# aantoine890/navierstokes

Measured on AMD Instinct MI355X. Metric: fp64 CSR SpMV GFLOP/s & % HBM roofline @ nnz; 1/2/4/8 GPU, higher is better.
Workload: dtype f64

## Files before the change

include/mi355_spmv.h:

```cpp
#ifndef MI355_SPMV_H
#define MI355_SPMV_H

#ifdef __cplusplus
extern "C" {
#endif

#define MI355_SPMV_VERSION 501

enum {
    MI_OK = 0,
    MI_ERR_ARG = 1,
    MI_ERR_NODEVICE = 2,
    MI_ERR_HIP = 3,
    MI_ERR_ALLOC = 4,
    MI_ERR_UNSUPPORTED = 5,
    MI_ERR_STATE = 6
};

#define MI_MAX_POWERS 16

typedef struct mi_csr_s* mi_csr_t;
typedef struct mi_bcsr4_s* mi_bcsr4_t;
typedef struct mi_part_s* mi_part_t;
typedef void* mi_stream_t;

enum {
    MI_KERNEL_AUTO = 0,
    MI_KERNEL_STREAM = 1,
    MI_KERNEL_RING = 2,
    MI_KERNEL_ROWPAR = 3,
    MI_KERNEL_BCSR4 = 4,
    MI_KERNEL_MRING = 6,
    MI_KERNEL_SSTREAM = 7,
    MI_KERNEL_TILE = 5
};

int mi_version(void);
const char* mi_strerror(int status);
const char* mi_last_error(void);
int mi_device_count(int* count);
int mi_set_device(int device);
int mi_device_synchronize(void);
int mi_flush_cache(void);
int mi_flush_cache_async(mi_stream_t s);

int mi_csr_create(int n, int ncols, const int* ptrow, const int* indcol, const double* coef, mi_csr_t* out);
int mi_csr_create_mapped(int n, int ncols, const int* ptrow, const int* indcol, const double* coef,
                         const int* rowmap, mi_csr_t* out);
int mi_csr_destroy(mi_csr_t A);
int mi_csr_update_values(mi_csr_t A, const double* coef);
int mi_csr_update_values_dev(mi_csr_t A, const double* d_coef, mi_stream_t s);
int mi_csr_dims(mi_csr_t A, int* n, int* ncols, long long* nnz);
int mi_csr_reorder_info(mi_csr_t A, int* reordered, int* block, double* spread_before, double* spread_after,
                        double* us_natural, double* us_reordered);
int mi_csr_perm(mi_csr_t A, int* reordered, int* perm );
int mi_vec_to_internal_dev(mi_csr_t A, const double* d_x, double* d_x_int, mi_stream_t s);
int mi_vec_from_internal_dev(mi_csr_t A, const double* d_x_int, double* d_x, mi_stream_t s);
int mi_spmv_internal_dev(mi_csr_t A, const double* d_x_int, double* d_y_int, mi_stream_t s);
int mi_spmk_internal_dev(mi_csr_t A, int k, const double* d_x_int, double* const* d_y_int_out, mi_stream_t s);
int mi_reorder_probe(int n, const int* ptrow, const int* indcol, int* block, int* perm, double* spread_before,
                     double* spread_after);
int mi_csr_set_kernel(mi_csr_t A, int kernel_id);
int mi_csr_ring_info(mi_csr_t A, int* config_id, int* runs, int* runs_not_ringable, double* nnz_fraction_ringable);
int mi_csr_ring_shape_info(mi_csr_t A, int* blocks, int* lean, int* depth, double* us_aligned, double* us_unaligned);
int mi_csr_tune_info(mi_csr_t A, double* us_ring, double* us_stream);
int mi_csr_tune_detail(mi_csr_t A, double us[5], int* ring_nt, int* stream_nt);
int mi_ring_plan_probe(int n, const int* ptrow, const int* indcol, int config_id, int* nblk, int* runs,
                       int* runs_not_ringable, double* nnz_fraction_ringable, int* max_slot);
int mi_csr_tile_info(mi_csr_t A, int* built, int* nblk, double* unique_per_nnz, double us[2], int* nt);
int mi_tile_plan_probe(int n, const int* ptrow, const int* indcol, int threads, int* nblk, long long* distinct_total,
                       int* max_distinct, long long* nnz_listed);
int mi_csr_placement_info(mi_csr_t A, int* n_values, int* n_total, double* us, int cap);
int mi_vec_alloc_placed(mi_csr_t A, int nvec, int draws, double** d_vecs, double* us, int cap, int* n_us);
int mi_vec_free_placed(double* d_vec);
int mi_csr_sstream_info(mi_csr_t A, int* built, int* rounds, long long* steps, double* padding, double us[4], int* form);
int mi_sstream_plan_probe(int n, int ncols, const int* ptrow, const int* indcol, int* eligible, int* rounds, long long* steps, double* padding);
int mi_sstream_plan_probe_ex(int n, int ncols, const int* ptrow, const int* indcol, int shift, int ghost_lo, int ghost_hi, int* eligible, int* rounds,
                             long long* steps, double* padding, int* ghost_workgroups, int* rounds_min_max);
int mi_sstream_mw_plan_probe(int n, int ncols, const int* ptrow, const int* indcol, int shift, int* eligible, int* rounds, long long* steps, double* padding);
int mi_csr_mring_info(mi_csr_t A, int* built, int* runs, int* runs_not_served, double* nnz_fraction_served, double us[2], int* nt);
int mi_mring_plan_probe(int n, const int* ptrow, const int* indcol, int* nblk, int* runs, int* runs_not_served,
                        double* nnz_fraction_served, long long* window_restarts);
int mi_mring_plan_deal_probe(int n, const int* ptrow, const int* indcol, int* table_len, int* run_blocks, int cap);
int mi_ring_plan_lean(int n, const int* ptrow, const int* indcol, int config_id, int* lean);
int mi_csr_block4_structure(int n, const int* ptrow, const int* indcol, int* is_blocked, long long* nblocks);
int mi_csr_set_nontemporal(mi_csr_t A, int ring_nt, int stream_nt);
int mi_stream_read_probe(long long bytes, int launches, double* us_per_launch);
int mi_csr_get_kernel(mi_csr_t A, int* kernel_id);
const char* mi_csr_kernel_name(mi_csr_t A);

int mi_spmv(mi_csr_t A, const double* x, double* y);
int mi_spmv_dev(mi_csr_t A, const double* d_x, double* d_y, mi_stream_t s);

int mi_spmk(mi_csr_t A, int k, const double* x, double* const* y_out);
int mi_spmk_dev(mi_csr_t A, int k, const double* d_x, double* const* d_y_out, mi_stream_t s);

int mi_csr_spmk_info(mi_csr_t A, int k, int* eligible, int* one_launch, double* us_k_launches, double* us_one_launch);

int mi_spmk_plan_probe(int n, const int* ptrow, const int* indcol, int* eligible, int* runs, int* max_deps);

int mi_dot(int n, const double* x, const double* y, double* out);
int mi_dot_dev(int n, const double* d_x, const double* d_y, double* d_out, mi_stream_t s);
int mi_axpy(int n, double a, const double* x, double* y);
int mi_axpy_dev(int n, double a, const double* d_x, double* d_y, mi_stream_t s);
int mi_orthogonalize(int n, const double* b, const double* x1, double* x3, double alpha, double* beta_out);
int mi_orthogonalize_dev(int n, const double* d_b, const double* d_x1, double* d_x3, double alpha,
                         double* d_beta_out, mi_stream_t s);
int mi_spmv_dot_dev(mi_csr_t A, const double* d_x, double* d_y, const double* d_b, double* d_beta_out, mi_stream_t s);
int mi_csr_dot_epilogue_info(mi_csr_t A, int* in_epilogue);
int mi_csr_dot_epilogue_layout(mi_csr_t A, int* threads, int* wgs, int* nblk, int* run_first_block, int* block_row0,
                               int* block_rows, int cap_runs, int cap_blocks);
int mi_spmv_orthogonalize_dev(mi_csr_t A, const double* d_x, double* d_x1, const double* d_b, double* d_x3, double alpha,
                              double* d_beta_out, mi_stream_t s);
int mi_orthonormalize_against_basis(int n, int m, const double* const* basis, double* y, double* dots_out );
int mi_orthonormalize_against_basis_dev(int n, int m, const double* const* d_basis, double* d_y, double* d_dots ,
                                        mi_stream_t s);
int mi_mdot(int n, int m, const double* const* basis, const double* y, double* dots );
int mi_mdot_dev(int n, int m, const double* const* d_basis , const double* d_y,
                double* d_dots , mi_stream_t s);
int mi_maxpy(int n, int m, const double* coef , int negate, const double* const* basis, double* y);
int mi_maxpy_dev(int n, int m, const double* d_coef , int negate, const double* const* d_basis, double* d_y,
                 double* d_norm_out, mi_stream_t s);
int mi_cgs_dev(int n, int m, const double* const* d_basis, double* d_y, int passes, double* d_h ,
               double* d_norm , mi_stream_t s);
int mi_norm2(int n, const double* x, double* out);
int mi_norm2_dev(int n, const double* d_x, double* d_out, mi_stream_t s);
int mi_rel_error(int n, const double* ref, const double* test, double* out);
int mi_rel_error_dev(int n, const double* d_ref, const double* d_test, double* d_out, mi_stream_t s);
int mi_gather_dev(int m, const int* d_idx, const double* d_src, double* d_dst, mi_stream_t s);

int mi_bcsr4_create(int nbrows, int nbcols, const int* ptrow, const int* indcol, const double* coef,
                    mi_bcsr4_t* out);
int mi_bcsr4_destroy(mi_bcsr4_t A);
enum { MI_BLOCK_ROWMAJOR = 0, MI_BLOCK_COLMAJOR = 1 };
int mi_bcsr4_create_layout(int nbrows, int nbcols, const int* ptrow, const int* indcol, const double* coef, int layout, mi_bcsr4_t* out);
int mi_bcsr4_update_values_layout(mi_bcsr4_t A, const double* coef, int layout);
int mi_bcsr4_update_values_layout_dev(mi_bcsr4_t A, const double* d_coef, int layout, mi_stream_t s);
int mi_bcsr4_tile_info(mi_bcsr4_t A, int* built, int* in_use, double* us_plain, double* us_tile);
int mi_bcsr4_sell_info(mi_bcsr4_t A, int* built, int* form_in_use, long long* steps, double* padding, double us[4]);
int mi_bcsr4_sell_plan_probe(int nbrows, const int* ptrow, const int* indcol, int nwaves_max, int* nslices, long long* nsteps, int* nwaves,
                             int* sptr, int* wrng, unsigned* col);
int mi_bcsr4_update_values(mi_bcsr4_t A, const double* coef);
int mi_bcsr4_update_values_dev(mi_bcsr4_t A, const double* d_coef, mi_stream_t s);
int mi_bcsr4_spmv(mi_bcsr4_t A, const double* x, double* y);
int mi_bcsr4_spmv_dev(mi_bcsr4_t A, const double* d_x, double* d_y, mi_stream_t s);
int mi_bcsr4_spmk(mi_bcsr4_t A, int k, const double* x, double* const* y_out);
int mi_bcsr4_spmk_dev(mi_bcsr4_t A, int k, const double* d_x, double* const* d_y_out, mi_stream_t s);

enum { MI_ARITH_CHAIN = 0, MI_ARITH_BLOCKACC = 1 };
int mi_bcsr4_spmm(mi_bcsr4_t A, int s, const double* X, long long ldx, double* Y, long long ldy, int arith);
int mi_bcsr4_spmm_dev(mi_bcsr4_t A, int s, const double* d_X, long long ldx, double* d_Y, long long ldy, int arith,
                      mi_stream_t st);
int mi_bcsr4_spmm_info(mi_bcsr4_t A, int s, int* tile_built, int* form_in_use, int* longest_list, double us[5]);
int mi_spmm_dev(mi_csr_t A, int s, const double* d_X, long long ldx, double* d_Y, long long ldy, mi_stream_t st);
int mi_krylov_basis_dev(mi_csr_t A, int s, const double* d_v0, double* d_V, long long ldv, int orth, double* d_coef,
                        mi_stream_t st);
int mi_krylov_basis_cgs_dev(mi_csr_t A, int s, const double* d_v0, double* d_V, long long ldv, int passes, double* d_coef,
                            mi_stream_t st);

typedef struct mi_bilu4_s* mi_bilu4_t;
int mi_bilu4_create(int nbrows, const int* ptrow, const int* indcol, const double* coef, int layout , int fill,
                    mi_bilu4_t* out);
int mi_bilu4_create_host(int nbrows, const int* ptrow, const int* indcol, const double* coef, int layout, int fill, mi_bilu4_t* out);
int mi_bilu4_destroy(mi_bilu4_t F);
int mi_bilu4_refactor(mi_bilu4_t F, const double* coef, int layout);
int mi_bilu4_solve_dev(mi_bilu4_t F, const double* d_b, double* d_x, mi_stream_t s);
int mi_bilu4_solve(mi_bilu4_t F, const double* b, double* x);
int mi_bilu4_info(mi_bilu4_t F, int* nbrows, long long* nblocks, int* fwd_levels, int* bwd_levels, int* launches, int* form,
                  double us[2], double* factor_seconds, long long* factor_bytes);
int mi_bilu4_factor_host(mi_bilu4_t F, int* ptr, int* col, int* diag, double* val, long long cap_blocks);
int mi_bilu4_plan_probe(int nbrows, const int* ptrow, const int* indcol, int fill, long long* nblocks, int* fwd_levels,
                        int* bwd_levels, int* fwd_launches, int* bwd_launches, int* fwd_sizes, int* bwd_sizes, int cap_levels);

int mi_bilu4dev_plan_probe(int nbrows, const int* ptrow, const int* indcol, int fill, long long* update_pairs, int* launches,
                           long long* plan_bytes);
int mi_bilu4dev_prepare(mi_bilu4_t F);
int mi_bilu4dev_refactor(mi_bilu4_t F, const double* d_coef, int layout, mi_stream_t s);
int mi_bilu4dev_status(mi_bilu4_t F, int* bad_row);
int mi_bilu4dev_fetch(mi_bilu4_t F);
int mi_bilu4dev_info(mi_bilu4_t F, int* prepared, int* launches, long long* plan_bytes);

enum { MI_BILU_FORM_LEVELS = 0, MI_BILU_FORM_ONE = 1, MI_BILU_FORM_AUTO = -1 };
int mi_bilu4one_plan_probe(int nbrows, const int* ptrow, const int* indcol, int fill, int workgroups, int* eligible, int nchunks[2],
                           int max_deps[2], long long* plan_bytes, int* const chunk_pos[2], int* const chunk_lev[2],
                           int* const dep_ptr[2], int* const dep[2]);
int mi_bilu4one_prepare(mi_bilu4_t F);
int (mi_bilu4_set_solve_form)(mi_bilu4_t F, int form);
int mi_bilu4one_status(mi_bilu4_t F);
int mi_bilu4one_info(mi_bilu4_t F, int* prepared, int* eligible, int* workgroups, int nchunks[2], int max_deps[2], long long* plan_bytes);

int mi_bilu4sw_prepare(mi_bilu4_t F);
int mi_bilu4sw_solve_dev(mi_bilu4_t F, const double* d_b, double* d_x, int sweeps_fwd, int sweeps_bwd, mi_stream_t s);
// ... 74 lines not shown
```

navierstokes_amd/csrc/capi_bcsr.hip:

```cpp
#include "capi_internal.hpp"
#include "spmv_bcsr_sell.hpp"

static int sell_fill(mi_bcsr4_t A, hipStream_t s);

template <class Select>
static bool bcsr4_race(mi_bcsr4_t A, int ncand, Select select, double* us)
{
    LaunchTimer tm;
    ScratchPair sp;
    if (sp.alloc(4 * (size_t)std::max(A->nbcols, 1), 4 * (size_t)std::max(A->nbrows, 1)) != MI_OK || tm.init() != MI_OK) return false;
    std::vector<char> failed((size_t)ncand, 0);
    for (int round = 0; round < 2; round++)
        for (int c = 0; c < ncand; c++) {
            if (failed[c]) continue;
            select(c);
            double t = 0.0;
            if (tm.time(3, 8, [&] { return launch_bcsr4(A, sp.x, sp.y, nullptr, false); }, &t) == MI_OK) us[c] = min_measured(us[c], t);
            else failed[c] = 1;
        }
    for (int c = 0; c < ncand; c++)
        if (failed[c]) us[c] = 0.0;
    return true;
}

// ... 42 lines not shown

static int build_bcsr4_sell(mi_bcsr4_t A, const int* ptrow, const int* indcol)
{
    SellPlanHost P, P2;
    build_sell_plan(A->nbrows, ptrow, indcol, 1024, P);
    build_sell_wave_ranges(P, 2048, P2.wrng, P2.nwaves);
    const size_t vbytes = sizeof(double) * (size_t)(P.nsteps + kSellPadSteps) * kSellStepDoubles;
    hipError_t e;
    if ((e = hipMalloc(&A->d_sell_val, vbytes)) != hipSuccess || (e = hipMalloc(&A->d_sell_col, sizeof(unsigned) * P.col.size())) != hipSuccess ||
        (e = hipMalloc(&A->d_sell_sptr, sizeof(int) * P.sptr.size())) != hipSuccess || (e = hipMalloc(&A->d_sell_wrng, sizeof(int) * P.wrng.size())) != hipSuccess ||
        (e = hipMalloc(&A->d_sell_wrng2, sizeof(int) * P2.wrng.size())) != hipSuccess ||
        (e = hipMemcpy(A->d_sell_wrng2, P2.wrng.data(), sizeof(int) * P2.wrng.size(), hipMemcpyHostToDevice)) != hipSuccess ||
        (e = hipMemset(A->d_sell_val + (size_t)P.nsteps * kSellStepDoubles, 0, sizeof(double) * (size_t)kSellPadSteps * kSellStepDoubles)) != hipSuccess ||
        (e = hipMemcpy(A->d_sell_col, P.col.data(), sizeof(unsigned) * P.col.size(), hipMemcpyHostToDevice)) != hipSuccess ||
        (e = hipMemcpy(A->d_sell_sptr, P.sptr.data(), sizeof(int) * P.sptr.size(), hipMemcpyHostToDevice)) != hipSuccess ||
        (e = hipMemcpy(A->d_sell_wrng, P.wrng.data(), sizeof(int) * P.wrng.size(), hipMemcpyHostToDevice)) != hipSuccess) {
        (void)hipGetLastError();
        dfree(A->d_sell_val); dfree(A->d_sell_col); dfree(A->d_sell_sptr); dfree(A->d_sell_wrng); dfree(A->d_sell_wrng2);
        A->d_sell_val = nullptr;
        A->d_sell_col = nullptr;
        A->d_sell_sptr = A->d_sell_wrng = A->d_sell_wrng2 = nullptr;
        return e == hipErrorOutOfMemory ? MI_OK : fail(MI_ERR_HIP, std::string("bcsr4 sliced copy: ") + hipGetErrorString(e));
    }
    A->sell_nslices = P.nslices;
    A->sell_nwaves = P.nwaves;
    A->sell_nwaves2 = P2.nwaves;
    A->sell_nsteps = P.nsteps;
    return sell_fill(A, nullptr);
}

static void choose_bcsr4_sell_form(mi_bcsr4_t A, bool forced)
{
    if (const char* fe = getenv("MI355_BCSR_SELL_FORM")) A->sell_form = std::max(0, std::min(3, atoi(fe)));
    else if (forced) A->sell_form = 0;
    else if (env_is("MI355_SPMV_AUTOTUNE", "0")) A->sell_form = 0;
    else {
        double us[5] = {0, 0, 0, 0, 0};
        if (!bcsr4_race(A, 5, [&](int c) { A->sell_form = c - 1; }, us)) return;
        int best = 0;
        for (int c = 1; c < 5; c++) {
            A->tune_us_sell[c - 1] = us[c];
            if (better(us[c], us[best])) best = c;
        }
        if (A->tune_us_plain <= 0 && A->tune_us_tile <= 0) A->tune_us_plain = us[0];
        A->sell_form = best - 1;
    }
}

extern "C" int mi_bcsr4_create(int nbrows, int nbcols, const int* ptrow, const int* indcol, const double* coef,
                               mi_bcsr4_t* out)
{
    CHECK_ARG(out, "out is null");
    *out = nullptr;
    CHECK_ARG(nbrows >= 0 && nbcols >= 0 && ptrow && ptrow[0] == 0, "bad argument");
    for (int i = 0; i < nbrows; i++) CHECK_ARG(ptrow[i] <= ptrow[i + 1], "ptrow must be non-decreasing");
    const long long nb = ptrow[nbrows];
    CHECK_ARG(nb == 0 || (indcol && coef), "indcol/coef is null");
    for (long long k = 0; k < nb; k++) CHECK_ARG(indcol[k] >= 0 && indcol[k] < nbcols, "block column outside [0, nbcols)");
    int rc = need_device();
    if (rc) return rc;
    std::unique_ptr<mi_bcsr4_s, int (*)(mi_bcsr4_t)> owner(new (std::nothrow) mi_bcsr4_s(), mi_bcsr4_destroy);
    mi_bcsr4_t A = owner.get();
    if (!A) return fail(MI_ERR_ALLOC, "host allocation failed");
    A->nbrows = nbrows;
    A->nbcols = nbcols;
    A->nblocks = nb;
    hipError_t e;
    if ((e = hipGetDevice(&A->device)) != hipSuccess ||
        (e = hipMalloc(&A->d_ptrow, sizeof(int) * ((size_t)nbrows + 1))) != hipSuccess ||
        (e = hipMalloc(&A->d_indcol, sizeof(int) * ((size_t)nb + 1))) != hipSuccess ||
        (e = hipMalloc(&A->d_coef, sizeof(double) * 16 * ((size_t)nb + 1))) != hipSuccess ||
        (e = hipMemcpy(A->d_ptrow, ptrow, sizeof(int) * ((size_t)nbrows + 1), hipMemcpyHostToDevice)) != hipSuccess ||
        (nb && (e = hipMemcpy(A->d_indcol, indcol, sizeof(int) * (size_t)nb, hipMemcpyHostToDevice)) != hipSuccess) ||
        (nb && (e = hipMemcpy(A->d_coef, coef, sizeof(double) * 16 * (size_t)nb, hipMemcpyHostToDevice)) != hipSuccess))
        return fail(e == hipErrorOutOfMemory ? MI_ERR_ALLOC : MI_ERR_HIP, std::string("bcsr4 upload: ") + hipGetErrorString(e));
    for (int s0 = 0; s0 < nbrows; s0 += kSellRows)
        A->max_slice_vals = std::max(A->max_slice_vals, 16 * (ptrow[std::min(nbrows, s0 + kSellRows)] - ptrow[s0]));
    if ((rc = build_bcsr4_tile(A, ptrow, indcol))) return rc;
    const bool forced = env_is("MI355_BCSR_SELL", "1");
    if (!env_is("MI355_BCSR_SELL", "0") && (forced || nb >= 100000) && nbcols > 0 && nbcols < (1 << 30)) {
        if ((rc = build_bcsr4_sell(A, ptrow, indcol))) return rc;
        if (A->d_sell_val) choose_bcsr4_sell_form(A, forced);
    }
    if ((e = hipStreamSynchronize(nullptr)) != hipSuccess) return fail(MI_ERR_HIP, std::string("mi_bcsr4_create: ") + hipGetErrorString(e));
    *out = owner.release();
    return MI_OK;
}

static int sell_fill(mi_bcsr4_t A, hipStream_t s)
{
    const int grid = std::max(1, std::min(A->sell_nslices, 8192));
    hipLaunchKernelGGL(bcsr4_to_sell_kernel, dim3((unsigned)grid), dim3(64), 0, s, A->sell_nslices, A->nbrows, A->d_ptrow, A->d_coef, A->d_sell_sptr, A->d_sell_val);
    HIP_TRY(hipGetLastError());
    return MI_OK;
}

int bcsr4_refresh_from_csr(mi_bcsr4_s* A, const int* d_csr_ptrow, const double* d_src, double* d_csr_out, hipStream_t s)
{
    if (!A || A->nbrows == 0) return MI_OK;
    const int nslices = (A->nbrows + kSellRows - 1) / kSellRows;
    const int grid = std::max(1, std::min(nslices, 2048));
    const int* sptr = A->d_sell_val ? A->d_sell_sptr : nullptr;
    double* sv = A->d_sell_val;
    if (A->max_slice_vals <= 4096)
        hipLaunchKernelGGL((bcsr4_refresh_kernel<4096>), dim3((unsigned)grid), dim3(256), 0, s, nslices, A->nbrows, d_csr_ptrow, d_src, d_csr_out, A->d_ptrow, A->d_coef, sptr, sv);
    else if (A->max_slice_vals <= 16384)
        hipLaunchKernelGGL((bcsr4_refresh_kernel<16384>), dim3((unsigned)std::min(grid, 256)), dim3(256), 0, s, nslices, A->nbrows, d_csr_ptrow, d_src, d_csr_out, A->d_ptrow, A->d_coef, sptr, sv);
    else
        hipLaunchKernelGGL((bcsr4_refresh_kernel<0>), dim3((unsigned)grid), dim3(256), 0, s, nslices, A->nbrows, d_csr_ptrow, d_src, d_csr_out, A->d_ptrow, A->d_coef, sptr, sv);
    HIP_TRY(hipGetLastError());
    return MI_OK;
}

static int bcsr4_refresh_from_blocks(mi_bcsr4_s* A, const double* d_src, bool colmajor, hipStream_t s)
{
    if (!A || A->nbrows == 0 || A->nblocks == 0) return MI_OK;
    const int nslices = (A->nbrows + kSellRows - 1) / kSellRows;
    const int grid = std::max(1, std::min(nslices, 2048));
    const int* sptr = A->d_sell_val ? A->d_sell_sptr : nullptr;
    double* out = d_src == A->d_coef ? nullptr : A->d_coef;
    if (colmajor && !out) return fail(MI_ERR_ARG, "column-major blocks cannot be transposed in place");
    if (!out && !A->d_sell_val) return MI_OK;
#define BR_LAUNCH(CAP_, CM_, G_) hipLaunchKernelGGL((bcsr4_blocks_refresh_kernel<CAP_, CM_>), dim3((unsigned)(G_)), dim3(256), 0, s, nslices, A->nbrows, A->d_ptrow, d_src, out, sptr, A->d_sell_val)
    if (A->max_slice_vals <= 4096) { if (colmajor) BR_LAUNCH(4096, true, grid); else BR_LAUNCH(4096, false, grid); }
    else if (A->max_slice_vals <= 16384) { if (colmajor) BR_LAUNCH(16384, true, std::min(grid, 256)); else BR_LAUNCH(16384, false, std::min(grid, 256)); }
    else { if (colmajor) BR_LAUNCH(0, true, grid); else BR_LAUNCH(0, false, grid); }
#undef BR_LAUNCH
    HIP_TRY(hipGetLastError());
    return MI_OK;
}

int bcsr4_values_changed(mi_bcsr4_s* A, hipStream_t s)
{
    if (A && A->d_sell_val && A->nblocks > 0) return sell_fill(A, s);
    return MI_OK;
}

extern "C" int mi_bcsr4_sell_info(mi_bcsr4_t A, int* built, int* form_in_use, long long* steps, double* padding, double us[4])
{
    CHECK_ARG(A, "null handle");
    if (built) *built = A->d_sell_val != nullptr;
    if (form_in_use) *form_in_use = A->d_sell_val ? A->sell_form : -1;
    if (steps) *steps = A->sell_nsteps;
    if (padding) *padding = A->nblocks > 0 && A->d_sell_val ? (double)A->sell_nsteps * kSellRows / (double)A->nblocks - 1.0 : 0.0;
    if (us)
        for (int i = 0; i < 4; i++) us[i] = A->tune_us_sell[i];
    return MI_OK;
}

extern "C" int mi_bcsr4_sell_plan_probe(int nbrows, const int* ptrow, const int* indcol, int nwaves_max, int* nslices, long long* nsteps,
                                        int* nwaves, int* sptr, int* wrng, unsigned* col)
{
    CHECK_ARG(nbrows >= 0 && ptrow && ptrow[0] == 0 && nwaves_max >= 1, "bad argument");
    for (int i = 0; i < nbrows; i++) CHECK_ARG(ptrow[i] <= ptrow[i + 1], "ptrow must be non-decreasing");
    const long long nb = ptrow[nbrows];
    CHECK_ARG(nb == 0 || indcol, "indcol is null");
    for (long long k = 0; k < nb; k++) CHECK_ARG(indcol[k] >= 0 && indcol[k] < (1 << 30), "block column outside [0, 2^30)");
    SellPlanHost P;
    build_sell_plan(nbrows, ptrow, indcol, nwaves_max, P);
    if (nslices) *nslices = P.nslices;
    if (nsteps) *nsteps = P.nsteps;
    if (nwaves) *nwaves = P.nwaves;
    if (sptr) std::copy(P.sptr.begin(), P.sptr.end(), sptr);
    if (wrng) std::copy(P.wrng.begin(), P.wrng.end(), wrng);
    if (col) std::copy(P.col.begin(), P.col.end(), col);
    return MI_OK;
}

static void transpose_blocks_host(long long nb, const double* src, double* dst)
{
    for (long long k = 0; k < nb; k++)
        for (int r = 0; r < 4; r++)
            for (int c = 0; c < 4; c++) dst[16 * k + 4 * r + c] = src[16 * k + 4 * c + r];
}

extern "C" int mi_bcsr4_create_layout(int nbrows, int nbcols, const int* ptrow, const int* indcol, const double* coef, int layout,
                                      mi_bcsr4_t* out)
{
    CHECK_ARG(layout == MI_BLOCK_ROWMAJOR || layout == MI_BLOCK_COLMAJOR, "unknown block layout");
    if (layout == MI_BLOCK_ROWMAJOR) return mi_bcsr4_create(nbrows, nbcols, ptrow, indcol, coef, out);
    CHECK_ARG(out, "out is null");
    *out = nullptr;
    CHECK_ARG(nbrows >= 0 && ptrow && ptrow[0] == 0 && ptrow[nbrows] >= 0, "bad argument");
    const long long nb = ptrow[nbrows];
    CHECK_ARG(nb == 0 || coef, "coef is null");
    std::vector<double> t((size_t)nb * 16);
    transpose_blocks_host(nb, coef, t.data());
    return mi_bcsr4_create(nbrows, nbcols, ptrow, indcol, t.data(), out);
}

extern "C" int mi_bcsr4_update_values_layout(mi_bcsr4_t A, const double* coef, int layout)
{
    CHECK_ARG(A, "null handle");
    CHECK_ARG(layout == MI_BLOCK_ROWMAJOR || layout == MI_BLOCK_COLMAJOR, "unknown block layout");
    if (layout == MI_BLOCK_ROWMAJOR || A->nblocks == 0) return mi_bcsr4_update_values(A, coef);
    CHECK_ARG(coef, "null coef");
    std::vector<double> t((size_t)A->nblocks * 16);
    transpose_blocks_host(A->nblocks, coef, t.data());
    return mi_bcsr4_update_values(A, t.data());
}

extern "C" int mi_bcsr4_update_values_layout_dev(mi_bcsr4_t A, const double* d_coef, int layout, mi_stream_t s)
{
    CHECK_ARG(A, "null handle");
    CHECK_ARG(layout == MI_BLOCK_ROWMAJOR || layout == MI_BLOCK_COLMAJOR, "unknown block layout");
    if (layout == MI_BLOCK_ROWMAJOR || A->nblocks == 0) return mi_bcsr4_update_values_dev(A, d_coef, s);
    CHECK_ARG(d_coef && d_coef != A->d_coef, "null coef, or the handle's own array");
    return bcsr4_refresh_from_blocks(A, d_coef, true, (hipStream_t)s);
}

extern "C" int mi_bcsr4_tile_info(mi_bcsr4_t A, int* built, int* in_use, double* us_plain, double* us_tile)
{
    CHECK_ARG(A, "null handle");
    if (built) *built = A->d_tl_ptr != nullptr;
    if (in_use) *in_use = A->use_tile && A->d_tl_ptr;
    if (us_plain) *us_plain = A->tune_us_plain;
    if (us_tile) *us_tile = A->tune_us_tile;
    return MI_OK;
}

extern "C" int mi_bcsr4_update_values(mi_bcsr4_t A, const double* coef)
{
    CHECK_ARG(A, "null handle");
    if (A->nblocks == 0) return MI_OK;
    CHECK_ARG(coef, "null coef");
    HIP_TRY(hipMemcpy(A->d_coef, coef, sizeof(double) * 16 * (size_t)A->nblocks, hipMemcpyHostToDevice));
    int rc = bcsr4_values_changed(A, nullptr);
    if (rc) return rc;
    HIP_TRY(hipStreamSynchronize(nullptr));
    return MI_OK;
}

extern "C" int mi_bcsr4_update_values_dev(mi_bcsr4_t A, const double* d_coef, mi_stream_t s)
{
    CHECK_ARG(A, "null handle");
    if (A->nblocks == 0) return MI_OK;
    CHECK_ARG(d_coef, "null coef");
    return bcsr4_refresh_from_blocks(A, d_coef, false, (hipStream_t)s);
}

extern "C" int mi_bcsr4_destroy(mi_bcsr4_t A)
{
    if (!A) return MI_OK;
    dfree(A->d_ptrow);
    dfree(A->d_indcol);
    dfree(A->d_coef);
    dfree(A->d_browmap);
    dfree(A->d_tl_ptr);
    dfree(A->d_tl_nodes);
    dfree(A->d_tl_slots);
    dfree(A->d_sell_val);
    dfree(A->d_sell_col);
    dfree(A->d_sell_sptr);
    dfree(A->d_sell_wrng);
    dfree(A->d_sell_wrng2);
    dfree(A->st.d_ptr);
    dfree(A->st.d_nodes);
    dfree(A->st.d_slots);
    dfree(A->st.d_rows);
    dfree(A->st64.d_ptr);
    dfree(A->st64.d_nodes);
    dfree(A->st64.d_slots);
    dfree(A->st64.d_rows);
    dfree(A->d_x);
    dfree(A->d_y);
    for (double* p : A->d_pow) dfree(p);
    delete A;
    return MI_OK;
}

int launch_bcsr4(mi_bcsr4_t A, const double* d_x, double* d_y, mi_stream_t s, bool use_map)
{
    CHECK_ARG(A, "null handle");
    if (A->nbrows == 0) return MI_OK;
    CHECK_ARG(d_x && d_y, "null vector");
    CHECK_ARG((((uintptr_t)d_x) & 15) == 0, "x must be 16-byte aligned");
    Bcsr4View V{A->nbrows, A->nbcols, A->d_ptrow, A->d_indcol, A->d_coef, use_map ? A->d_browmap : nullptr};
    const long long threads = 4LL * A->nbrows;
    const int nwg = (int)((threads + kWG - 1) / kWG);
    static const int chunk = getenv("MI355_BCSR_XCD_CHUNK") ? atoi(getenv("MI355_BCSR_XCD_CHUNK")) : 0;
    const int grid = nwg;
    if (A->sell_form >= 0 && A->d_sell_val) {
        const bool two = A->sell_form == 2;
        SellView S{A->d_sell_val, A->d_sell_col, A->d_sell_sptr, two ? A->d_sell_wrng2 : A->d_sell_wrng, A->sell_nslices, A->nbrows, V.browmap};
        const int swg = two ? A->sell_nwaves2 / 8 : A->sell_nwaves / 4;
        switch (A->sell_form) {
        case 0: hipLaunchKernelGGL((spmv_bcsr4_sell<8, true, 0, 2, 4>), dim3((unsigned)swg), dim3(256), 0, (hipStream_t)s, S, d_x, d_y, swg); break;
        case 1: hipLaunchKernelGGL((spmv_bcsr4_sell<8, false, 0, 2, 4>), dim3((unsigned)swg), dim3(256), 0, (hipStream_t)s, S, d_x, d_y, swg); break;
        case 2: hipLaunchKernelGGL((spmv_bcsr4_sell<4, true, 0, 2, 8>), dim3((unsigned)swg), dim3(512), 0, (hipStream_t)s, S, d_x, d_y, swg); break;
        default: hipLaunchKernelGGL((spmv_bcsr4_sell<12, true, 0, 2, 4>), dim3((unsigned)swg), dim3(256), 0, (hipStream_t)s, S, d_x, d_y, swg); break;
        }
        HIP_TRY(hipGetLastError());
        return MI_OK;
    }
    if (A->use_tile && A->d_tl_ptr) {
        Bcsr4Tile Tl{A->d_tl_ptr, A->d_tl_nodes, A->d_tl_slots};
        hipLaunchKernelGGL(spmv_bcsr4_tile<kBcsrDepth>, dim3((unsigned)grid), dim3(kWG), 0, (hipStream_t)s, V, Tl, d_x, d_y, nwg);
        HIP_TRY(hipGetLastError());
        return MI_OK;
    }
    hipLaunchKernelGGL(spmv_bcsr4<kBcsrDepth>, dim3((unsigned)grid), dim3(kWG), 0, (hipStream_t)s, V, d_x, d_y, chunk, nwg);
    HIP_TRY(hipGetLastError());
    return MI_OK;
}

void bcsr4_drop_sliced(mi_bcsr4_s* A)
{
    if (!A || !A->d_sell_val) return;
    (void)hipDeviceSynchronize();
    dfree(A->d_sell_val);
    dfree(A->d_sell_col);
    dfree(A->d_sell_sptr);
    dfree(A->d_sell_wrng);
    dfree(A->d_sell_wrng2);
    A->d_sell_val = nullptr;
    A->d_sell_col = nullptr;
    A->d_sell_sptr = A->d_sell_wrng = A->d_sell_wrng2 = nullptr;
    A->sell_form = -1;
}

extern "C" int mi_bcsr4_spmv_dev(mi_bcsr4_t A, const double* d_x, double* d_y, mi_stream_t s)
{
    return launch_bcsr4(A, d_x, d_y, s, true);
}

extern "C" int mi_bcsr4_spmv(mi_bcsr4_t A, const double* x, double* y)
{
    CHECK_ARG(A, "null handle");
    if (A->nbrows == 0) return MI_OK;
    CHECK_ARG(x && y, "null vector");
    if (!A->d_x) HIP_TRY(hipMalloc(&A->d_x, sizeof(double) * 4 * (size_t)(A->nbcols > 0 ? A->nbcols : 1)));
    if (!A->d_y) HIP_TRY(hipMalloc(&A->d_y, sizeof(double) * 4 * (size_t)A->nbrows));
    HIP_TRY(hipMemcpy(A->d_x, x, sizeof(double) * 4 * (size_t)A->nbcols, hipMemcpyHostToDevice));
    int rc = mi_bcsr4_spmv_dev(A, A->d_x, A->d_y, nullptr);
    if (rc) return rc;
    HIP_TRY(hipMemcpy(y, A->d_y, sizeof(double) * 4 * (size_t)A->nbrows, hipMemcpyDeviceToHost));
    return MI_OK;
}

extern "C" int mi_bcsr4_spmk_dev(mi_bcsr4_t A, int k, const double* d_x, double* const* d_y_out, mi_stream_t s)
{
    CHECK_ARG(A, "null handle");
    if (k < 1 || k > MI_MAX_POWERS) return fail(MI_ERR_UNSUPPORTED, "k must be in 1..MI_MAX_POWERS");
    CHECK_ARG(A->nbrows == A->nbcols, "matrix powers need a square matrix");
    CHECK_ARG(d_y_out, "null output array");
    const double* src = d_x;
    for (int p = 0; p < k; p++) {
        CHECK_ARG(A->nbrows == 0 || d_y_out[p], "null output vector");
        int rc = mi_bcsr4_spmv_dev(A, src, d_y_out[p], s);
        if (rc) return rc;
        src = d_y_out[p];
    }
    return MI_OK;
}

extern "C" int mi_bcsr4_spmk(mi_bcsr4_t A, int k, const double* x, double* const* y_out)
{
    CHECK_ARG(A, "null handle");
    if (k < 1 || k > MI_MAX_POWERS) return fail(MI_ERR_UNSUPPORTED, "k must be in 1..MI_MAX_POWERS");
    CHECK_ARG(A->nbrows == A->nbcols, "matrix powers need a square matrix");
    if (A->nbrows == 0) return MI_OK;
// ... 156 lines not shown
    if (A->st_state) return A->st_state;
    A->st_state = -1;
    if (env_is("MI355_SPMM_TILE", "0") || A->nblocks < 4096) return -1;
    std::vector<int> ptrow((size_t)A->nbrows + 1), indcol((size_t)A->nblocks);
    if (hipMemcpy(ptrow.data(), A->d_ptrow, sizeof(int) * ptrow.size(), hipMemcpyDeviceToHost) != hipSuccess ||
        hipMemcpy(indcol.data(), A->d_indcol, sizeof(int) * indcol.size(), hipMemcpyDeviceToHost) != hipSuccess) {
        (void)hipGetLastError();
        return -1;
    }
    int cap128 = 368, cap64 = 256;
    if (const char* ce = getenv("MI355_SPMM_TILE_UCAP")) (void)sscanf(ce, "%d,%d", &cap128, &cap64);
    A->st_state = build_spmm_tile_plan(A, 128, cap128, ptrow, indcol, A->st);
    (void)build_spmm_tile_plan(A, 64, cap64, ptrow, indcol, A->st64);
    return A->st_state;
}

static const SpmmTilePlan* spmm_plan_of(const mi_bcsr4_s* A, int s)
{
    if (s < 1 || s > 4) return nullptr;
    const SpmmTilePlan* Pl = A->st.d_ptr ? &A->st : nullptr;
    if (!Pl || spmm_tile_lds(Pl, s) > kLdsBytesPerCU) return nullptr;
    return Pl;
}

enum { kSpmmGather = 0, kSpmmTile = 1, kSpmmOct = 2, kSpmmOctNt = 3, kSpmmSell = 4, kSpmmForms = 5 };

static int sell_fill(mi_bcsr4_t A, hipStream_t s);

static bool spmm_form_possible(const mi_bcsr4_s* A, int s, int form, bool mapped = false)
{
    if (form == kSpmmGather) return true;
    if (form == kSpmmSell) return (s == 4 || s == 8) && A->d_sell_val;
    if (form == kSpmmTile) return spmm_plan_of(A, s) != nullptr;
    return s % 2 == 0 && A->st64.d_ptr && spmm_tile_lds(&A->st64, s) <= kLdsBytesPerCU;
}

static void launch_spmm_gather(const Bcsr4View& V, int m, int arith, const double* Xj, long long ldx, double* Yj, long long ldy, hipStream_t st)
{
    switch (m) {
    case 1: launch_spmm_s<1>(V, arith, Xj, ldx, Yj, ldy, st); break;
    case 2: launch_spmm_s<2>(V, arith, Xj, ldx, Yj, ldy, st); break;
    case 3: launch_spmm_s<3>(V, arith, Xj, ldx, Yj, ldy, st); break;
    case 4: launch_spmm_s<4>(V, arith, Xj, ldx, Yj, ldy, st); break;
    case 5: launch_spmm_s<5>(V, arith, Xj, ldx, Yj, ldy, st); break;
    case 6: launch_spmm_s<6>(V, arith, Xj, ldx, Yj, ldy, st); break;
    case 7: launch_spmm_s<7>(V, arith, Xj, ldx, Yj, ldy, st); break;
    default: launch_spmm_s<8>(V, arith, Xj, ldx, Yj, ldy, st); break;
    }
}

static int launch_spmm(mi_bcsr4_t A, int s, int arith, const double* X, long long ldx, double* Y, long long ldy, hipStream_t st,
                       bool use_map)
{
    Bcsr4View V{A->nbrows, A->nbcols, A->d_ptrow, A->d_indcol, A->d_coef, use_map ? A->d_browmap : nullptr};
    for (int j0 = 0; j0 < s; j0 += 8) {
        const int m = std::min(8, s - j0);
        const double* Xj = X + (size_t)j0 * ldx;
        double* Yj = Y + (size_t)j0 * ldy;
        const bool mapped = V.browmap != nullptr;
        auto run = [&](int form) -> hipError_t {
            if (form == kSpmmSell) {
                SellView Sv{A->d_sell_val, A->d_sell_col, A->d_sell_sptr, A->d_sell_wrng, A->sell_nslices, A->nbrows, V.browmap};
                const int swg = A->sell_nwaves / 4;
                if (m == 4) {
                    if (arith == MI_ARITH_CHAIN) hipLaunchKernelGGL((spmm_bcsr4_sell<4, 0, 6, true>), dim3((unsigned)swg), dim3(256), 0, st, Sv, Xj, ldx, Yj, ldy, swg);
                    else hipLaunchKernelGGL((spmm_bcsr4_sell<4, 1, 6, true>), dim3((unsigned)swg), dim3(256), 0, st, Sv, Xj, ldx, Yj, ldy, swg);
                } else {
                    if (arith == MI_ARITH_CHAIN) hipLaunchKernelGGL((spmm_bcsr4_sell<8, 0, 6, true>), dim3((unsigned)swg), dim3(256), 0, st, Sv, Xj, ldx, Yj, ldy, swg);
                    else hipLaunchKernelGGL((spmm_bcsr4_sell<8, 1, 6, true>), dim3((unsigned)swg), dim3(256), 0, st, Sv, Xj, ldx, Yj, ldy, swg);
                }
                return hipGetLastError();
            }
            if (form == kSpmmTile) return spmm_tile_launch(A, spmm_plan_of(A, m), V, m, arith, Xj, ldx, Yj, ldy, st);
            if (form == kSpmmOct || form == kSpmmOctNt) return spmm_otile_launch(A, &A->st64, V, m, arith, form == kSpmmOctNt, Xj, ldx, Yj, ldy, st);
            launch_spmm_gather(V, m, arith, Xj, ldx, Yj, ldy, st);
            return hipGetLastError();
        };
        int form = kSpmmGather;
        const bool capturing = stream_is_capturing(st);
        if (capturing && A->spmm_choice[m] > 0 && (A->st_state == 1 || A->spmm_choice[m] - 1 == kSpmmSell) &&
            !(A->spmm_choice[m] - 1 == kSpmmSell && mapped))
            form = A->spmm_choice[m] - 1;
        const bool tiles = !capturing && build_spmm_tile(A) == 1;
        if (!capturing && (tiles || spmm_form_possible(A, m, kSpmmSell, mapped))) {
            const char* e = getenv("MI355_SPMM_TILE");
            const int forced = e ? atoi(e) : -1;
            auto possible = [&](int f) { return (f == kSpmmGather || f == kSpmmSell || tiles) && spmm_form_possible(A, m, f, mapped); };
            if (forced >= 0 && forced < kSpmmForms) form = possible(forced) ? forced : kSpmmGather;
            else {
                if (A->spmm_choice[m] == 0) {
                    int best = kSpmmGather;
                    LaunchTimer tm(st);
                    if (tm.init() == MI_OK) {
                        double us[kSpmmForms] = {0, 0, 0, 0, 0};
                        bool ok = true;
                        for (int round = 0; round < 2 && ok; round++)
                            for (int f = 0; f < kSpmmForms && ok; f++) {
                                if (!possible(f)) continue;
                                double t = 0.0;
                                ok = tm.time(2, 5, [&] { return run(f) == hipSuccess ? MI_OK : MI_ERR_HIP; }, &t) == MI_OK;
                                if (ok) us[f] = min_measured(us[f], t);
                            }
                        for (int f = 0; f < kSpmmForms; f++) {
                            A->spmm_us[m][f] = us[f];
                            if (ok && us[f] > 0 && us[f] < us[best]) best = f;
                        }
                        if (!ok) { (void)hipGetLastError(); best = kSpmmGather; }
                    }
                    A->spmm_choice[m] = 1 + best;
                }
                form = A->spmm_choice[m] - 1;
                if (!possible(form)) form = kSpmmGather;
            }
        }
        hipError_t er = run(form);
        if (er != hipSuccess) return fail(MI_ERR_HIP, std::string("multi-vector product: ") + hipGetErrorString(er));
    }
    HIP_TRY(hipGetLastError());
    return MI_OK;
}

extern "C" int mi_bcsr4_spmm_info(mi_bcsr4_t A, int s, int* tile_built, int* form_in_use, int* longest_list, double us[5])
{
    CHECK_ARG(A && s >= 1 && s <= 8, "bad argument");
    if (tile_built) *tile_built = A->st_state == 1;
// ... 155 lines not shown
```

navierstokes_amd/csrc/capi_csr.hip:

```cpp
#include "capi_internal.hpp"
#include "reorder.hpp"
#include "mring_plan.hpp"
#include "tile_plan.hpp"

int get_table(mi_csr_t A, int nnzb, BlockTable** out)
{
    BlockTable& T = A->tables[nnzb];
    if (!T.d_blk) {
        std::vector<int> rows, ptrs;
        int row_align = A->nnz < 20000000 ? 64 : 1;
        if (const char* e = getenv("MI355_STREAM_ROW_ALIGN")) row_align = std::max(1, atoi(e));
        build_row_blocks(A->n, A->h_ptrow.data(), nnzb, 4 * kWG, rows, ptrs, row_align, 7);
        T.nnzb = nnzb;
        T.nblk = (int)rows.size() - 1;
        std::vector<int2> h(rows.size());
        for (size_t i = 0; i < rows.size(); i++) h[i] = make_int2(rows[i], ptrs[i]);
        HIP_TRY(hipMalloc(&T.d_blk, sizeof(int2) * h.size()));
        HIP_TRY(hipMemcpy(T.d_blk, h.data(), sizeof(int2) * h.size(), hipMemcpyHostToDevice));
    }
    *out = &T;
    return MI_OK;
}

static void free_tile(mi_csr_t A)
{
    dfree(A->tile.d_desc);
    dfree(A->tile.d_ulist);
    dfree(A->tile.d_slots);
    A->tile = TileTable();
}

static void free_mring(mi_csr_t A)
{
    dfree(A->mring.d_plan);
    dfree(A->mring.d_first);
    dfree(A->mring.d_ok);
    dfree(A->mring.d_rng);
    dfree(A->mring.d_slots);
    A->mring = MringTable();
}

static void free_sstream(mi_csr_t A)
{
    ss_free(A->ss.dev);
    A->ss = SstreamTable();
}

static inline bool beyond_infinity_cache(double bytes_per_nnz, long long nnz, int n) { return bytes_per_nnz * (double)nnz + 16.0 * (double)n > 0.75 * 256e6; }

constexpr double kSsMaxPadding = 0.12;
static double ss_max_padding()
{
    if (const char* e = getenv("MI355_SSTREAM_MAX_PADDING")) return std::max(0.0, atof(e));
    return kSsMaxPadding;
}

static int build_sstream(mi_csr_t A, const int* ptrow, const int* indcol, int ghost_lo = 0, int ghost_hi = 0)
{
    if (A->ss.dev.val) return MI_OK;
    SsPlanHost P;
    SsMwPlanHost M;
    const int shift = (A->y_offset & 1) && !A->d_rowmap ? 1 : 0;
    build_sstream_plan(A->n, A->ncols, ptrow, indcol, ss_max_padding(), P, true, shift, ghost_lo, ghost_hi);
    SstreamTable& T = A->ss;
    hipError_t e;
    if (!P.eligible) {
        if (ghost_lo < ghost_hi || env_is("MI355_SSTREAM_MW", "0")) return MI_OK;
        build_sstream_mw_plan(A->n, A->ncols, ptrow, indcol, ss_max_padding(), M, shift);
        if (!M.eligible) return MI_OK;
        e = ss_mw_upload(M, T.dev);
        T.mw = e == hipSuccess;
    } else e = ss_upload(P, T.dev, ghost_lo < ghost_hi);
    const SsPlanHost& Q = P.eligible ? P : M;
    if (e != hipSuccess) {
        free_sstream(A);
        if (e == hipErrorOutOfMemory) { (void)hipGetLastError(); return MI_OK; }
        return fail(MI_ERR_HIP, std::string("sliced copy: ") + hipGetErrorString(e));
    }
    T.nwg = Q.nwg;
    T.rounds = Q.rounds;
    T.shift = Q.shift;
    T.steps = Q.steps;
    T.padding = (double)Q.pad_places / (double)A->nnz;
    T.max_slice_nnz = Q.max_slice_nnz;
    if (ghost_lo < ghost_hi) {
        T.h_wg_halo = P.wg_halo;
        T.h_wg = P.wg;
        T.fusable = P.fusable;
    }
    sstream_fill_values(T.rounds, A->n, T.shift, A->d_ptrow, A->d_coef, nullptr, T.dev.slice_step, T.dev.slice_len, T.dev.val, T.max_slice_nnz, nullptr, T.mw ? 1 : 0);
    if ((e = hipGetLastError()) != hipSuccess) {
        free_sstream(A);
        return fail(MI_ERR_HIP, std::string("sliced copy fill: ") + hipGetErrorString(e));
    }
    T.nt = beyond_infinity_cache(10.0, A->nnz, A->n);
    T.deep = T.nt;
    if (const char* fe = getenv("MI355_SSTREAM_FORM")) {
        const int f = atoi(fe);
        T.nt = (f & 1) == 0;
        T.deep = f >= 2;
    }
    return MI_OK;
}

int launch_sstream(mi_csr_t A, const double* d_x, double* d_y, const int* rowmap, hipStream_t s, const RingComm* comm)
{
    SstreamTable& T = A->ss;
    SsView S{T.dev.val, T.dev.slot, T.dev.wg, T.dev.win, T.nwg, A->n + T.shift, A->ncols, rowmap, T.shift};
    double* yy = rowmap ? d_y : d_y - T.shift;
    if (T.mw) {
        if (comm) return fail(MI_ERR_STATE, "the cut-ring sliced stream has no fused multi-GPU form");
        SsMwView V{S, T.dev.winK};
        if (T.deep) {
            if (T.nt) hipLaunchKernelGGL((spmv_sstream_mw<12, true>), dim3((unsigned)T.nwg), dim3(256), 0, s, V, d_x, yy);
            else hipLaunchKernelGGL((spmv_sstream_mw<12, false>), dim3((unsigned)T.nwg), dim3(256), 0, s, V, d_x, yy);
        } else {
            if (T.nt) hipLaunchKernelGGL((spmv_sstream_mw<8, true>), dim3((unsigned)T.nwg), dim3(256), 0, s, V, d_x, yy);
            else hipLaunchKernelGGL((spmv_sstream_mw<8, false>), dim3((unsigned)T.nwg), dim3(256), 0, s, V, d_x, yy);
        }
        HIP_TRY(hipGetLastError());
        return MI_OK;
    }
    if (comm) {
        const unsigned grid = (unsigned)(T.nwg + comm->push_wgs);
        if (T.deep) {
            if (T.nt) hipLaunchKernelGGL((spmv_sstream_fused<12, true>), dim3(grid), dim3(256), 0, s, S, d_x, yy, *comm);
            else hipLaunchKernelGGL((spmv_sstream_fused<12, false>), dim3(grid), dim3(256), 0, s, S, d_x, yy, *comm);
        } else {
            if (T.nt) hipLaunchKernelGGL((spmv_sstream_fused<8, true>), dim3(grid), dim3(256), 0, s, S, d_x, yy, *comm);
            else hipLaunchKernelGGL((spmv_sstream_fused<8, false>), dim3(grid), dim3(256), 0, s, S, d_x, yy, *comm);
        }
    } else if (T.deep) {
        if (T.nt) hipLaunchKernelGGL((spmv_sstream<12, true>), dim3((unsigned)T.nwg), dim3(256), 0, s, S, d_x, yy);
        else hipLaunchKernelGGL((spmv_sstream<12, false>), dim3((unsigned)T.nwg), dim3(256), 0, s, S, d_x, yy);
    } else {
        if (T.nt) hipLaunchKernelGGL((spmv_sstream<8, true>), dim3((unsigned)T.nwg), dim3(256), 0, s, S, d_x, yy);
        else hipLaunchKernelGGL((spmv_sstream<8, false>), dim3((unsigned)T.nwg), dim3(256), 0, s, S, d_x, yy);
    }
    HIP_TRY(hipGetLastError());
    return MI_OK;
}

static bool ring_wants_skew(int n, const int* ptrow)
// ... 504 lines not shown
            T2.nt = A->ring.nt;
            A->kernel = MI_KERNEL_RING;
            int rct = time_now(&us1);
            std::swap(A->ring, T2);
            if (rct == MI_OK) rct = time_now(&us64);
            A->kernel = MI_KERNEL_AUTO;
            A->tune_us_ring_aligned = us64;
            A->tune_us_ring_unaligned = us1;
            if (rct != MI_OK || !(us64 < 0.98 * us1)) std::swap(A->ring, T2);
            free_ring_table(T2);
        }
    } else if (A->auto_kernel == MI_KERNEL_MRING) {
        MringTable keep = A->mring;
        A->mring = MringTable();
        if (build_mring(A, in.indcol, 64) == MI_OK && A->mring.d_plan && A->mring.ok_fraction >= 0.90) {
            A->mring.nt = keep.nt;
            A->kernel = MI_KERNEL_MRING;
            int rct = time_now(&us64);
            std::swap(A->mring, keep);
            if (rct == MI_OK) rct = time_now(&us1);
            A->kernel = MI_KERNEL_AUTO;
            A->tune_us_ring_aligned = us64;
            A->tune_us_ring_unaligned = us1;
            if (rct == MI_OK && us64 < 0.98 * us1) std::swap(A->mring, keep);
        } else {
            std::swap(A->mring, keep);
        }
        std::swap(A->mring, keep);
        free_mring(A);
        A->mring = keep;
    }
}

static int measure_at_create(mi_csr_t A, const CsrInput& in, bool defer_placement)
{
    const size_t scratch_len = placed_vector_len(in.n, in.ncols);
    LaunchTimer tm;
    ScratchPair sp;
    int rc = sp.alloc(std::max(scratch_len, (size_t)(in.ncols > 0 ? in.ncols : 1)), std::max(scratch_len, (size_t)(A->n_out > 0 ? A->n_out : 1)));
    if (rc || (rc = tm.init())) return rc;
    tune(A, tm, sp);
    compare_ring_shapes(A, in, tm, sp);
    if (!defer_placement && placement_draws(A, sp.x, sp.y, !in.rowmap && in.n == in.ncols && in.n == A->n_out && !in.ghosts()) == MI_OK &&
        A->kept_x == sp.x)
        sp.hand_over();
    return MI_OK;
}

int csr_create_impl(int n, int ncols, const int* ptrow, const int* indcol, const double* coef,
                    const int* rowmap, mi_csr_t* out, int ghost_lo, int ghost_hi, bool defer_placement)
{
    CHECK_ARG(out, "out is null");
    *out = nullptr;
    CsrInput in{n, ncols, ptrow, indcol, coef, rowmap, ghost_lo, ghost_hi};
    int rc = check_input(in);
    if (rc || (rc = need_device())) return rc;
    std::unique_ptr<mi_csr_s, int (*)(mi_csr_t)> owner(new (std::nothrow) mi_csr_s(), mi_csr_destroy);
    mi_csr_t A = owner.get();
    if (!A) return fail(MI_ERR_ALLOC, "host allocation failed");
    A->n = n;
    A->ncols = ncols;
    A->nnz = in.nnz;
    A->ghost_lo = ghost_lo;
    A->ghost_hi = ghost_hi;
    A->h_ptrow.assign(ptrow, ptrow + n + 1);
    if ((rc = upload(A, in)) || (rc = plan_ring(A, in)) || (rc = plan_optional(A, in)) || (rc = attach_blocked(A, in))) return rc;
    load_defaults(A, in);
    const bool forced_kernel = apply_forced_kernel(A);
    if (!forced_kernel && in.nnz < kMeasureNnz && A->auto_kernel == MI_KERNEL_RING && !in.ghosts()) A->auto_kernel = MI_KERNEL_STREAM;
    if (!forced_kernel && !env_is("MI355_SPMV_AUTOTUNE", "0") && in.nnz >= kMeasureNnz && (rc = measure_at_create(A, in, defer_placement))) return rc;
    HIP_TRY(hipStreamSynchronize(nullptr));
    *out = owner.release();
    return MI_OK;
}

static int time_handle(mi_csr_t A, int warm, int timed, double* us)
{
    LaunchTimer tm;
    ScratchPair sp;
    int rc = sp.alloc((size_t)(A->ncols > 0 ? A->ncols : 1), (size_t)(A->n_out > 0 ? A->n_out : 1));
    if (rc || (rc = tm.init())) return rc;
    return time_on(tm, A, sp.x, sp.y, warm, timed, us);
}

static void release_natural_arrays(mi_csr_t A)
{
    dfree(A->d_ptrow);
    dfree(A->d_indcol);
    dfree(A->d_coef);
    A->d_ptrow = A->d_indcol = nullptr;
    A->d_coef = nullptr;
    for (auto& kv : A->tables) dfree(kv.second.d_blk);
    A->tables.clear();
    free_ring_table(A->ring);
    free_tile(A);
    free_mring(A);
    free_sstream(A);
    mi_bcsr4_destroy(A->blocked);
    A->blocked = nullptr;
}

static int maybe_reorder(mi_csr_t A, const int* ptrow, const int* indcol, const double* coef)
{
    const bool force = env_is("MI355_REORDER", "1");
    if (env_is("MI355_REORDER", "0")) return MI_OK;
    const int n = A->n;
// ... 1 lines not shown
    if (!force && (n < 100000 || resolve_kernel(A) == MI_KERNEL_RING || resolve_kernel(A) == MI_KERNEL_SSTREAM)) return MI_OK;
    const int block = csr_has_block4_pattern(n, ptrow, indcol) ? 4 : 1;
    const double nn = (double)n / block;
    const double spread = mean_column_distance(n, ptrow, indcol, block);
    A->spread_before = spread;
    if (!force && spread < 2.0 * std::pow(nn, 2.0 / 3.0)) return MI_OK;
    Reorder R;
    rcm_reorder(n, ptrow, indcol, block, R);
    A->reorder_block = block;
    A->spread_after = R.spread_after;
    if (!force && R.spread_after > 0.5 * spread) return MI_OK;
    std::vector<int> p2, c2, src_start;
    std::vector<double> v2;
    permute_csr(n, ptrow, indcol, coef, R, p2, c2, v2, src_start);
    mi_csr_t inner = nullptr;
    int rc = csr_create_impl(n, n, p2.data(), c2.data(), v2.data(), R.iperm.data(), &inner);
    if (rc) return rc;
    A->inner = inner;
    hipError_t e;
    if ((e = hipMalloc(&A->d_iperm, sizeof(int) * (size_t)n)) != hipSuccess ||
        (e = hipMalloc(&A->d_src_start, sizeof(int) * (size_t)n)) != hipSuccess ||
        (e = hipMalloc(&A->d_xp, sizeof(double) * (size_t)n)) != hipSuccess ||
        (e = hipMemcpy(A->d_iperm, R.iperm.data(), sizeof(int) * (size_t)n, hipMemcpyHostToDevice)) != hipSuccess ||
        (e = hipMemcpy(A->d_src_start, src_start.data(), sizeof(int) * (size_t)n, hipMemcpyHostToDevice)) != hipSuccess)
        return fail(e == hipErrorOutOfMemory ? MI_ERR_ALLOC : MI_ERR_HIP, std::string("reorder upload: ") + hipGetErrorString(e));
    bool keep = true;
    if (!force && !env_is("MI355_SPMV_AUTOTUNE", "0")) {
        const int timed = A->nnz < 40000000 ? 12 : 6;
        A->inner = nullptr;
        rc = time_handle(A, 3, timed, &A->us_natural);
        A->inner = inner;
        if (rc) return rc;
        if ((rc = time_handle(A, 3, timed, &A->us_reordered))) return rc;
        keep = A->us_reordered < 0.97 * A->us_natural;
    }
    if (!keep) {
        mi_csr_destroy(A->inner);
        A->inner = nullptr;
        dfree(A->d_iperm);
        dfree(A->d_src_start);
        dfree(A->d_xp);
        A->d_iperm = A->d_src_start = nullptr;
        A->d_xp = nullptr;
        return MI_OK;
    }
    A->h_iperm = R.iperm;
    A->xp_claimed = false;
    release_natural_arrays(A);
    return MI_OK;
}

extern "C" int mi_csr_create(int n, int ncols, const int* ptrow, const int* indcol, const double* coef, mi_csr_t* out)
{
    int rc = csr_create_impl(n, ncols, ptrow, indcol, coef, nullptr, out, 0, 0, true);
    if (rc) return rc;
    if ((rc = maybe_reorder(*out, ptrow, indcol, coef)) || (!(*out)->inner && (rc = placement_draws(*out, nullptr, nullptr, n == ncols))) ||
        (hipStreamSynchronize(nullptr) != hipSuccess && (rc = fail(MI_ERR_HIP, "mi_csr_create: synchronize")))) {
        mi_csr_destroy(*out);
        *out = nullptr;
    }
    return rc;
}

extern "C" int mi_reorder_probe(int n, const int* ptrow, const int* indcol, int* block, int* perm, double* spread_before,
                                double* spread_after)
{
    CHECK_ARG(n >= 0 && ptrow && (ptrow[n] == 0 || indcol), "bad argument");
    for (int i = 0; i < n; i++) {
        CHECK_ARG(ptrow[i] <= ptrow[i + 1], "ptrow must be non-decreasing");
        for (int k = ptrow[i]; k < ptrow[i + 1]; k++) CHECK_ARG(indcol[k] >= 0 && indcol[k] < n, "column index outside [0, n)");
    }
    const int b = csr_has_block4_pattern(n, ptrow, indcol) ? 4 : 1;
    Reorder R;
    rcm_reorder(n, ptrow, indcol, b, R);
    if (block) *block = b;
    if (perm)
        for (int i = 0; i < n; i++) perm[i] = R.perm[i];
    if (spread_before) *spread_before = R.spread_before;
    if (spread_after) *spread_after = R.spread_after;
    return MI_OK;
}

extern "C" int mi_csr_reorder_info(mi_csr_t A, int* reordered, int* block, double* spread_before, double* spread_after,
                                   double* us_natural, double* us_reordered)
{
    CHECK_ARG(A, "null handle");
    if (reordered) *reordered = A->inner ? 1 : 0;
    if (block) *block = A->reorder_block;
    if (spread_before) *spread_before = A->spread_before;
    if (spread_after) *spread_after = A->spread_after;
    if (us_natural) *us_natural = A->us_natural;
    if (us_reordered) *us_reordered = A->us_reordered;
    return MI_OK;
}

extern "C" int mi_csr_perm(mi_csr_t A, int* reordered, int* perm)
{
    CHECK_ARG(A, "null handle");
    if (reordered) *reordered = A->inner ? 1 : 0;
    if (perm) {
        if (A->inner) {
            CHECK_ARG((int)A->h_iperm.size() == A->n, "permutation not kept on this handle");
            for (int r = 0; r < A->n; r++) perm[A->h_iperm[r]] = r;
        } else {
            for (int i = 0; i < A->n; i++) perm[i] = i;
        }
// ... 30 lines not shown
    return launch_spmv(A, d_x_int, d_y_int, (hipStream_t)s);
}

extern "C" int mi_spmk_internal_dev(mi_csr_t A, int k, const double* d_x_int, double* const* d_y_int_out, mi_stream_t s)
{
    CHECK_ARG(A, "null handle");
    if (k < 1 || k > MI_MAX_POWERS) return fail(MI_ERR_UNSUPPORTED, "k must be in 1..MI_MAX_POWERS");
    CHECK_ARG(d_y_int_out, "null output array");
    CHECK_ARG(A->n == A->ncols && !A->mapped, "the internal numbering is defined for square, unmapped matrices");
    if (A->n == 0) return MI_OK;
    CHECK_ARG(d_x_int, "null vector");
    for (int p = 0; p < k; p++) CHECK_ARG(d_y_int_out[p], "null output vector");
    return spmk_unmapped(A->inner ? A->inner : A, k, d_x_int, d_y_int_out, (hipStream_t)s);
}

extern "C" int mi_csr_create_mapped(int n, int ncols, const int* ptrow, const int* indcol, const double* coef,
                                    const int* rowmap, mi_csr_t* out)
{
    return csr_create_impl(n, ncols, ptrow, indcol, coef, rowmap, out);
}

extern "C" int mi_csr_destroy(mi_csr_t A)
{
    if (!A) return MI_OK;
    dfree(A->d_ptrow);
    dfree(A->d_indcol);
    dfree(A->d_coef);
    dfree(A->d_rowmap);
    dfree(A->d_x);
    dfree(A->d_y);
    dfree(A->kept_x);
    dfree(A->kept_y);
    for (double* p : A->d_pow) dfree(p);
    for (auto& kv : A->tables) {
        dfree(kv.second.d_blk);
    }
    free_ring_table(A->ring);
    free_tile(A);
    free_mring(A);
    free_sstream(A);
    mi_bcsr4_destroy(A->blocked);
    mi_csr_destroy(A->inner);
    dfree(A->d_iperm);
    dfree(A->d_src_start);
    dfree(A->d_xp);
    for (auto& kv : A->xp_more) dfree(kv.second);
    dfree(A->d_vtmp);
    for (double* p : A->d_pp) dfree(p);
    spmk_release(A);
    delete A;
    return MI_OK;
}

static int refresh_blocked_values(mi_csr_t A, hipStream_t s, bool sliced_done = false)
{
    if (A->ss.dev.val && !sliced_done) {
        SstreamTable& T = A->ss;
        sstream_fill_values(T.rounds, A->n, T.shift, A->d_ptrow, A->d_coef, nullptr, T.dev.slice_step, T.dev.slice_len, T.dev.val, T.max_slice_nnz, s, T.mw ? 1 : 0);
        HIP_TRY(hipGetLastError());
    }
    if (!A->blocked || A->blocked->nbrows == 0) return MI_OK;
    return bcsr4_refresh_from_csr(A->blocked, A->d_ptrow, A->d_coef, nullptr, s);
}

__global__ __launch_bounds__(256) void permute_values_kernel(int n, const int* __restrict__ new_ptrow, const int* __restrict__ src_start,
                                                             const double* __restrict__ src, double* __restrict__ dst)
{
    __shared__ int s_p[65], s_a[64];
    const int tid = threadIdx.x;
    for (int r0 = blockIdx.x * 64; r0 < n; r0 += gridDim.x * 64) {
        const int nr = min(64, n - r0);
        if (tid <= nr) s_p[tid] = new_ptrow[r0 + tid];
        if (tid < nr) s_a[tid] = src_start[r0 + tid];
        __syncthreads();
        const int b0 = s_p[0], seg = s_p[nr] - b0;
        for (int k = tid; k < seg; k += 256) {
            const int p = b0 + k;
            int lo = 0, hi = nr;
            while (hi - lo > 1) {
                const int mid = (lo + hi) >> 1;
                if (s_p[mid] <= p) lo = mid;
                else hi = mid;
            }
            dst[p] = src[s_a[lo] + (p - s_p[lo])];
        }
        __syncthreads();
    }
}

extern "C" int mi_csr_update_values_dev(mi_csr_t A, const double* d_coef, mi_stream_t s_)
{
    CHECK_ARG(A, "null handle");
    if (A->nnz == 0) return MI_OK;
    CHECK_ARG(d_coef, "null coef");
    hipStream_t s = (hipStream_t)s_;
    if (A->inner) {
        mi_csr_t I = A->inner;
        hipLaunchKernelGGL(permute_values_kernel, dim3((unsigned)std::max(1, std::min((A->n + 63) / 64, 4096))), dim3(256), 0, s, A->n, I->d_ptrow, A->d_src_start, d_coef, I->d_coef);
        HIP_TRY(hipGetLastError());
        return refresh_blocked_values(I, s);
    }
    if (A->ss.dev.val && d_coef != A->d_coef) {
        SstreamTable& T = A->ss;
        sstream_fill_values(T.rounds, A->n, T.shift, A->d_ptrow, d_coef, A->d_coef, T.dev.slice_step, T.dev.slice_len, T.dev.val, T.max_slice_nnz, s, T.mw ? 1 : 0);
        HIP_TRY(hipGetLastError());
        return refresh_blocked_values(A, s, true);
    }
    if (A->blocked && A->blocked->nbrows > 0 && d_coef != A->d_coef)
        return bcsr4_refresh_from_csr(A->blocked, A->d_ptrow, d_coef, A->d_coef, s);
    if (d_coef != A->d_coef) HIP_TRY(hipMemcpyAsync(A->d_coef, d_coef, sizeof(double) * (size_t)A->nnz, hipMemcpyDeviceToDevice, s));
    return refresh_blocked_values(A, s);
}

extern "C" int mi_csr_update_values(mi_csr_t A, const double* coef)
{
    CHECK_ARG(A, "null handle");
    if (A->nnz == 0) return MI_OK;
    CHECK_ARG(coef, "null coef");
    if (A->inner) {
        if (!A->d_vtmp) HIP_TRY(hipMalloc(&A->d_vtmp, sizeof(double) * (size_t)A->nnz));
        HIP_TRY(hipMemcpy(A->d_vtmp, coef, sizeof(double) * (size_t)A->nnz, hipMemcpyHostToDevice));
        int rc = mi_csr_update_values_dev(A, A->d_vtmp, nullptr);
        if (rc) return rc;
        HIP_TRY(hipStreamSynchronize(nullptr));
        return MI_OK;
    }
    HIP_TRY(hipMemcpy(A->d_coef, coef, sizeof(double) * (size_t)A->nnz, hipMemcpyHostToDevice));
    int rc = refresh_blocked_values(A, nullptr);
    if (rc) return rc;
    HIP_TRY(hipStreamSynchronize(nullptr));
    return MI_OK;
}

extern "C" int mi_csr_dims(mi_csr_t A, int* n, int* ncols, long long* nnz)
{
    CHECK_ARG(A, "null handle");
    if (n) *n = A->n;
    if (ncols) *ncols = A->ncols;
    if (nnz) *nnz = A->nnz;
    return MI_OK;
}

int resolve_kernel(const mi_csr_s* A)
{
    int k = A->kernel != MI_KERNEL_AUTO ? A->kernel : A->auto_kernel;
    if (k == MI_KERNEL_RING && !A->ring.d_plan) k = MI_KERNEL_STREAM;
    if (k == MI_KERNEL_BCSR4 && !A->blocked) k = MI_KERNEL_STREAM;
    if (k == MI_KERNEL_TILE && !A->tile.d_desc) k = MI_KERNEL_STREAM;
    if (k == MI_KERNEL_MRING && !A->mring.d_plan) k = MI_KERNEL_STREAM;
    if (k == MI_KERNEL_SSTREAM && !A->ss.dev.val) k = A->ring.d_plan && A->ring.ok_fraction >= 0.90 ? MI_KERNEL_RING : MI_KERNEL_STREAM;
    return k;
}

extern "C" int mi_csr_tune_info(mi_csr_t A, double* us_ring, double* us_stream)
{
    CHECK_ARG(A, "null handle");
    if (A->inner) A = A->inner;
    if (us_ring) *us_ring = A->tune_us[MI_KERNEL_RING][A->ring.nt];
    if (us_stream) *us_stream = A->tune_us[MI_KERNEL_STREAM][A->stream_nt];
    return MI_OK;
}

extern "C" int mi_csr_tune_detail(mi_csr_t A, double us[5], int* ring_nt, int* stream_nt)
{
    CHECK_ARG(A, "null handle");
    if (A->inner) A = A->inner;
    if (us) {
        us[0] = A->tune_us[MI_KERNEL_RING][0];
        us[1] = A->tune_us[MI_KERNEL_RING][1];
        us[2] = A->tune_us[MI_KERNEL_STREAM][0];
        us[3] = A->tune_us[MI_KERNEL_STREAM][1];
        us[4] = A->tune_us[MI_KERNEL_BCSR4][0];
    }
    if (ring_nt) *ring_nt = A->ring.nt ? 1 : 0;
    if (stream_nt) *stream_nt = A->stream_nt ? 1 : 0;
// ... 607 lines not shown
```

navierstokes_amd/csrc/capi_internal.hpp:

```cpp
#pragma once
#include "mi355_spmv.h"

#include <hip/hip_runtime.h>

#include <cstdio>
#include <cstdlib>
#include <cmath>
#include <chrono>
#include <cstring>
#include <map>
#include <memory>
#include <mutex>
#include <new>
#include <string>
#include <vector>

#include "partition.hpp"
#include "push_exchange.hpp"
#include "ring_plan.hpp"
#include "spmv_kernels.hpp"
#include "spmv_ring.hpp"
#include "spmv_sstream_mw.hpp"

using namespace mi355;
// ... 53 lines not shown
        HIP_TRY(hipEventCreate(&e1));
        return MI_OK;
    }
    template <class F>
    int time(int warm, int timed, F&& launch, double* us)
    {
        int rc;
        for (int w = 0; w < warm; w++)
            if ((rc = launch())) return rc;
        HIP_TRY(hipEventRecord(e0, s));
        for (int w = 0; w < timed; w++)
            if ((rc = launch())) return rc;
        HIP_TRY(hipEventRecord(e1, s));
        HIP_TRY(hipEventSynchronize(e1));
        float ms = 0.f;
        HIP_TRY(hipEventElapsedTime(&ms, e0, e1));
        *us = ms * 1e3 / timed;
        return MI_OK;
    }
};

struct ScratchPair {
    double *x = nullptr, *y = nullptr;
    ScratchPair() = default;
    ScratchPair(const ScratchPair&) = delete;
    ScratchPair& operator=(const ScratchPair&) = delete;
    ~ScratchPair()
    {
        dfree(x);
        dfree(y);
    }
    int alloc(size_t nx, size_t ny)
    {
        HIP_TRY(hipMalloc(&x, sizeof(double) * nx));
        HIP_TRY(hipMalloc(&y, sizeof(double) * ny));
        HIP_TRY(hipMemset(x, 0, sizeof(double) * nx));
        return MI_OK;
    }
    void hand_over() { x = y = nullptr; }
};

static inline double min_measured(double a, double b) { return a > 0 ? std::min(a, b) : b; }
static inline bool better(double a, double b) { return a > 0 && (b <= 0 || a < b); }

static inline bool stream_is_capturing(hipStream_t s)
{
    hipStreamCaptureStatus st = hipStreamCaptureStatusNone;
    if (hipStreamIsCapturing(s, &st) != hipSuccess) {
        (void)hipGetLastError();
        return false;
    }
    return st != hipStreamCaptureStatusNone;
}

struct BlockTable {
    int nnzb = 0;
    int nblk = 0;
    int2* d_blk = nullptr;
};

struct RingTable {
    RingConfig cfg{};
    int nblk = 0, wgs = 0, bpw = 0, bad_runs = 0;
    double ok_fraction = 0.0;
    int* d_plan = nullptr;
    int* d_ok = nullptr;
    int* d_rng = nullptr;
    int* d_run_halo = nullptr;
    std::vector<int> h_run_halo;
    bool uniform = true;
    bool lean = false;
    bool all_in_loop = false;
    std::vector<int> h_dep_ptr, h_dep_run;
    unsigned short* d_slots = nullptr;
    bool nt = false;
    bool skew = false;
};

struct MringTable {
    int nblk = 0, wgs = 0, nruns = 0, bpw = 0, bad_runs = 0, depth = 2;
    double ok_fraction = 0.0;
    long long restarts = 0;
    int* d_plan = nullptr;
    int* d_first = nullptr;
    int* d_ok = nullptr;
    int* d_rng = nullptr;
    unsigned short* d_slots = nullptr;
    bool nt = false, skew = false;
};

struct TileTable {
    int nblk = 0;
    int* d_desc = nullptr;
    unsigned* d_ulist = nullptr;
    unsigned short* d_slots = nullptr;
    double unique_per_nnz = 0.0;
    bool nt = false;
    bool skew = false;
};

struct SstreamTable {
    bool mw = false;
    SsDevice dev;
    int nwg = 0, rounds = 0;
    int shift = 0;
    long long steps = 0;
    double padding = 0.0;
    int max_slice_nnz = 0;
    bool nt = true;
    bool deep = true;
    bool fusable = false;
    bool asked = false;
    std::vector<int> h_wg_halo;
    std::vector<SsWg> h_wg;
    double tune_us[4] = {0, 0, 0, 0};
};

struct mi_csr_s {
    int device = 0;
    int n = 0, ncols = 0;
    long long nnz = 0;
    int* d_ptrow = nullptr;
    int* d_indcol = nullptr;
    double* d_coef = nullptr;
    int* d_rowmap = nullptr;
    bool mapped = false;
    int y_offset = 0;
    int ghost_lo = 0, ghost_hi = 0;
    std::vector<int> h_ptrow;
    std::map<int, BlockTable> tables;
    RingTable ring;
    TileTable tile;
    SstreamTable ss;
    MringTable mring;
    int kernel = MI_KERNEL_AUTO;
    int auto_kernel = MI_KERNEL_STREAM;
    std::vector<double> place_us;
    int place_draws_coef = 0;
    double *kept_x = nullptr, *kept_y = nullptr;
    double tune_us[MI_KERNEL_SSTREAM + 1][2] = {};
    double tune_us_ring_aligned = 0.0, tune_us_ring_unaligned = 0.0;
    bool stream_nt = false;
    mi_bcsr4_t blocked = nullptr;
    int n_out = 0;
    mi_csr_t inner = nullptr;
    int* d_iperm = nullptr;
    std::vector<int> h_iperm;
    int* d_src_start = nullptr;
    double* d_xp = nullptr;
    hipStream_t xp_stream = nullptr;
    bool xp_claimed = false;
    std::map<hipStream_t, double*> xp_more;
    std::vector<double*> d_pp;
    double* d_vtmp = nullptr;
    double spread_before = 0.0, spread_after = 0.0, us_natural = 0.0, us_reordered = 0.0;
    int reorder_block = 0;
    double* d_x = nullptr;
    double* d_y = nullptr;
    std::vector<double*> d_pow;
    unsigned* d_kflags = nullptr;
    int* d_kdep_ptr = nullptr;
    int* d_kdep_run = nullptr;
    unsigned kstep_epoch = 0;
    unsigned* h_ktimeouts = nullptr;
    unsigned* d_ktimeouts = nullptr;
    int kstep_setup = 0;
    int kstep_choice[9] = {0, 0, 0, 0, 0, 0, 0, 0, 0};
    double kstep_us[9][2] = {};
};

struct SpmmTilePlan {
    int rows = 0, umax = 0, ntiles = 0;
    double mean_list = 0.0;
    int* d_ptr = nullptr;
    unsigned* d_nodes = nullptr;
    unsigned short* d_slots = nullptr;
    int* d_rows = nullptr;
};

struct mi_bcsr4_s {
    int device = 0;
    int nbrows = 0, nbcols = 0;
    long long nblocks = 0;
    int* d_ptrow = nullptr;
    int* d_indcol = nullptr;
    double* d_coef = nullptr;
    int* d_browmap = nullptr;
    int* d_tl_ptr = nullptr;
    unsigned* d_tl_nodes = nullptr;
    unsigned short* d_tl_slots = nullptr;
    bool use_tile = false;
    double tune_us_plain = 0.0, tune_us_tile = 0.0;
    double* d_sell_val = nullptr;
    unsigned* d_sell_col = nullptr;
    int* d_sell_sptr = nullptr;
    int* d_sell_wrng = nullptr;
    int* d_sell_wrng2 = nullptr;
    int sell_nslices = 0, sell_nwaves = 0, sell_nwaves2 = 0;
    long long sell_nsteps = 0;
    int max_slice_vals = 0;
    int sell_form = -1;
    double tune_us_sell[4] = {0, 0, 0, 0};
    SpmmTilePlan st, st64;
    int st_state = 0;
    int spmm_choice[9] = {0, 0, 0, 0, 0, 0, 0, 0, 0};
    double spmm_us[9][5] = {};
    double* d_x = nullptr;
    double* d_y = nullptr;
    std::vector<double*> d_pow;
};

struct mi_part_s {
    PartPlan plan;
    mi_csr_t piece[2] = {nullptr, nullptr};
    int* d_send_idx = nullptr;
    bool finalized = false;
    int kernel = MI_KERNEL_AUTO;
    void* comm = nullptr;
    hipStream_t comm_stream = nullptr;
    hipEvent_t ev_pack = nullptr, ev_comm = nullptr;
    double* d_sendbuf = nullptr;
    unsigned* d_flags = nullptr;
    unsigned* h_timeouts = nullptr;
    unsigned* d_timeouts = nullptr;
    unsigned step_no = 0;
    bool flag_handoff = false;
    std::vector<int> ag_union;
    int ag_slice = 0;
    int* d_ag_idx = nullptr;
    int* d_ag_src = nullptr;
    double* d_ag_send = nullptr;
    double* d_ag_recv = nullptr;
    bool ag_ready = false, ag_use = false;
    void* win = nullptr;
    bool win_uncached = false, win_registered = false;
    std::string win_key;
    unsigned* win_flags = nullptr;
    double* win_data = nullptr;
    std::vector<void*> ipc_opened;
// ... 27 lines not shown
    int ext_debug = 0;
};

static inline size_t win_data_offset(int nranks) { return ((size_t)nranks * kWinFlagStride * sizeof(unsigned) + 255) / 256 * 256; }

extern std::mutex g_mu;
int get_ws(hipStream_t s, double** out);

struct Scratch {
    std::vector<double*> bufs;
    ~Scratch()
    {
        for (double* p : bufs) dfree(p);
    }
    int up(const double* h, size_t n, double** d)
    {
        *d = nullptr;
        HIP_TRY(hipMalloc(d, sizeof(double) * (n ? n : 1)));
        bufs.push_back(*d);
        if (h && n) HIP_TRY(hipMemcpy(*d, h, sizeof(double) * n, hipMemcpyHostToDevice));
        return MI_OK;
    }
};

int csr_create_impl(int n, int ncols, const int* ptrow, const int* indcol, const double* coef, const int* rowmap, mi_csr_t* out,
                    int ghost_lo = 0, int ghost_hi = 0, bool defer_placement = false);
int resolve_kernel(const mi_csr_s* A);
int get_table(mi_csr_t A, int nnzb, BlockTable** out);
int launch_spmv(mi_csr_t A, const double* d_x, double* d_y, hipStream_t s, bool use_map = true, const RingComm* comm = nullptr,
                const RingDot* dot = nullptr);
bool ring_dot_eligible(const mi_csr_s* A);
int reorder_scratch(mi_csr_t A, hipStream_t s, double** buf);
void launch_ring_cfg(const mi_csr_s* A, const CsrView& V, const double* d_x, double* d_y, hipStream_t s, const RingComm* comm, const RingDot* dot);
int spmk_unmapped(mi_csr_t H, int k, const double* d_x, double* const* d_y, hipStream_t s);
void spmk_release(mi_csr_t H);
int gather_perm(mi_csr_t A, const double* d_x, double* d_xp, hipStream_t s);
int ortho_update_from_parts(int n, int nparts, const double* parts, double alpha, const double* d_b, const double* d_x1, double* d_x3, double* d_beta_out,
                            hipStream_t s);
int scatter_perm(mi_csr_t A, const double* d_src, double* d_dst, hipStream_t s);
constexpr size_t kLdsBytesPerCU = 160 * 1024;
static inline size_t spmm_tile_lds(const SpmmTilePlan* T, int s) { return T ? (size_t)T->umax * (4 * s + 2) * sizeof(double) : (size_t)-1; }
hipError_t spmm_tile_launch(const mi_bcsr4_s* A, const SpmmTilePlan* Pl, const Bcsr4View& V, int s, int arith, const double* X, long long ldx,
                            double* Y, long long ldy, hipStream_t st);
hipError_t spmm_otile_launch(const mi_bcsr4_s* A, const SpmmTilePlan* Pl, const Bcsr4View& V, int s, int arith, bool nt, const double* X, long long ldx,
                             double* Y, long long ldy, hipStream_t st);
int part_push_window(mi_part_s* P);
void part_push_layout(const mi_part_s* P, long long* layout );
int part_push_connect_bases(mi_part_s* P, void* const* bases , const long long* layouts);
int part_ext_launch(mi_part_s* P, const double* d_x_ext, double* d_y_local, unsigned step, unsigned spin_max, hipStream_t s, unsigned long long* trace, int* grid_out);
int launch_sstream(mi_csr_t A, const double* d_x, double* d_y, const int* rowmap, hipStream_t s, const RingComm* comm = nullptr);
static inline bool sstream_y_ok(const mi_csr_s* A, const double* yy, const int* map) { return map || A->ss.mw || (((uintptr_t)(yy - A->ss.shift)) & 15) == 0; }
int bcsr4_values_changed(mi_bcsr4_s* A, hipStream_t s);
void bcsr4_drop_sliced(mi_bcsr4_s* A);
int bcsr4_refresh_from_csr(mi_bcsr4_s* A, const int* d_csr_ptrow, const double* d_src, double* d_csr_out, hipStream_t s);
int launch_bcsr4(mi_bcsr4_t A, const double* d_x, double* d_y, mi_stream_t s, bool use_map);
```

navierstokes_amd/csrc/capi_lib.hip:

```cpp
#include "capi_internal.hpp"

thread_local std::string g_err;
std::mutex g_mu;

int need_device()
{
    int cnt = 0;
    hipError_t e = hipGetDeviceCount(&cnt);
    if (e != hipSuccess || cnt <= 0)
        return fail(MI_ERR_NODEVICE, std::string("no HIP device: ") + (e != hipSuccess ? hipGetErrorString(e) : "count is 0") +
                                         " (libmi355spmv has no CPU fallback)");
    return MI_OK;
}

extern "C" int mi_version(void) { return MI355_SPMV_VERSION; }

extern "C" const char* mi_strerror(int status)
{
    switch (status) {
    case MI_OK: return "ok";
    case MI_ERR_ARG: return "invalid argument";
    case MI_ERR_NODEVICE: return "no HIP device (no CPU fallback)";
    case MI_ERR_HIP: return "HIP runtime error";
    case MI_ERR_ALLOC: return "allocation failed";
    case MI_ERR_UNSUPPORTED: return "unsupported";
    case MI_ERR_STATE: return "bad handle state";
    default: return "unknown status";
    }
}

extern "C" const char* mi_last_error(void) { return g_err.c_str(); }

extern "C" int mi_device_count(int* count)
{
    CHECK_ARG(count, "count is null");
    int c = 0;
    hipError_t e = hipGetDeviceCount(&c);
    *count = (e == hipSuccess) ? c : 0;
    return MI_OK;
}

extern "C" int mi_set_device(int device)
{
    int rc = need_device();
    if (rc) return rc;
    HIP_TRY(hipSetDevice(device));
    return MI_OK;
}

extern "C" int mi_device_synchronize(void)
{
    int rc = need_device();
    if (rc) return rc;
    HIP_TRY(hipDeviceSynchronize());
    return MI_OK;
// ... 81 lines not shown
```

navierstokes_amd/csrc/capi_part.hip:

```cpp
#include "capi_internal.hpp"
#include "handoff_kernels.hpp"
#include "push_kernels.hpp"
#include "spmv_bcsr4_ext.hpp"
#include "rccl_loader.hpp"

static std::map<std::string, void*> g_win_registry;
static void part_comm_release(mi_part_s* P);
static int part_need_timeouts(mi_part_s* P);

static Rccl& g_rccl = rccl_state();
static_assert(MI_COMM_ID_BYTES == kCommIdBytes, "id size");

#define NCCL_TRY(expr)                                                                                  \
    do {                                                                                                \
        int r_ = (expr);                                                                                \
        if (r_ != 0) return fail(MI_ERR_HIP, std::string(#expr) + ": " + g_rccl.GetErrorString(r_));    \
    } while (0)

static void part_comm_release(mi_part_s* P)
{
    if (P->comm && g_rccl.ok) g_rccl.CommDestroy(P->comm);
    P->comm = nullptr;
    if (P->comm_stream) (void)hipStreamDestroy(P->comm_stream);
    if (P->ev_pack) (void)hipEventDestroy(P->ev_pack);
// ... 789 lines not shown
    if (P->fused_ext && P->ext_csr) return P->ext_split ? "spmv_csr_fused_ext x2 (ranks share a device: two launches)" : "spmv_csr_fused_ext";
    if (P->fused_ext) return P->ext_split ? "spmv_bcsr4_fused_ext x2 (ranks share a device: two launches)" : "spmv_bcsr4_fused_ext";
    static thread_local char nm[160];
    const char* base = mi_csr_kernel_name(P->piece_all);
    if (resolve_kernel(P->piece_all) == MI_KERNEL_SSTREAM) snprintf(nm, sizeof nm, "spmv_sstream_fused<%d, %s>", P->piece_all->ss.deep ? 12 : 8, P->piece_all->ss.nt ? "true" : "false");
    else snprintf(nm, sizeof nm, "%s [FUSED]", base);
    return nm;
}

extern "C" int mi_part_push_info(mi_part_t P, int* ready, int* fused, int* neighbours)
{
    CHECK_ARG(P, "null handle");
    if (ready) *ready = P->push_ready ? 1 : 0;
    if (fused) *fused = P->fused ? 1 : 0;
    if (neighbours) *neighbours = P->n_nb;
    return MI_OK;
}
int part_ext_launch(mi_part_s* P, const double* d_x_ext, double* d_y_local, unsigned step, unsigned spin_max, hipStream_t s, unsigned long long* trace, int* grid_out)
{
    const PartPlan& pl = P->plan;
    if (!P->ext_csr && (((uintptr_t)d_x_ext) & 15) != 0) return fail(MI_ERR_ARG, "the fused blocked step needs a 16-byte aligned x");
    ExtComm C;
    C.links = P->d_links;
    C.work = P->d_push_work;
    C.link_chunks = P->d_link_chunks;
    C.tickets = P->d_tickets;
    C.send_idx = P->d_send_idx;
    C.flags = P->win_flags;
    C.nb = P->d_nb;
    C.halo = P->win_data + (size_t)(step & 1u) * (size_t)pl.n_halo;
    C.stage = P->d_stage;
    C.ready = P->d_ready;
    C.timeouts = P->d_timeouts;
    C.n_work = P->n_push_work;
    C.n_nb = P->n_nb;
    C.n_local = pl.n_local;
    C.n_halo = pl.n_halo;
    C.xwgs = P->n_push_work + P->ext_wgs;
    C.step = step;
    C.spin_max = spin_max;
    C.trace = trace;
    C.nowait = 0;
    if (P->ext_debug & 2) C.links = nullptr;
    if (P->ext_debug & 4) C.n_halo = 0;
    if (P->ext_debug & 8) C.n_nb = 0;
    const bool split = P->ext_split && !trace && P->n_ext_units > P->n_ext_plain;
    const dim3 grid((split ? P->n_ext_plain : P->n_ext_units) + C.xwgs);
    if (grid_out) *grid_out = (int)grid.x;
    if (P->ext_csr) {
        mi_csr_t A = P->piece_all;
        BlockTable* T = nullptr;
        int rc = get_table(A, 1024, &T);
        if (rc) return rc;
        CsrView V{A->n, A->ncols, A->d_ptrow, A->d_indcol, A->d_coef, nullptr, T->d_blk, nullptr, T->nblk};
        if (trace) hipLaunchKernelGGL((spmv_csr_fused_ext<1024, false, true>), grid, dim3(kWG), 0, s, V, d_x_ext, d_y_local, C, P->d_ext_order);
        else if (A->stream_nt) hipLaunchKernelGGL((spmv_csr_fused_ext<1024, true>), grid, dim3(kWG), 0, s, V, d_x_ext, d_y_local, C, P->d_ext_order);
        else hipLaunchKernelGGL((spmv_csr_fused_ext<1024, false>), grid, dim3(kWG), 0, s, V, d_x_ext, d_y_local, C, P->d_ext_order);
        if (split) {
            ExtComm C2 = C;
            C2.xwgs = C2.n_work = 0;
            C2.nowait = 1;
            const dim3 g2(P->n_ext_units - P->n_ext_plain);
            if (A->stream_nt) hipLaunchKernelGGL((spmv_csr_fused_ext<1024, true>), g2, dim3(kWG), 0, s, V, d_x_ext, d_y_local, C2, P->d_ext_order + P->n_ext_plain);
            else hipLaunchKernelGGL((spmv_csr_fused_ext<1024, false>), g2, dim3(kWG), 0, s, V, d_x_ext, d_y_local, C2, P->d_ext_order + P->n_ext_plain);
        }
        HIP_TRY(hipGetLastError());
        return MI_OK;
    }
    mi_bcsr4_t B = P->piece_all->blocked;
    Bcsr4View V{B->nbrows, B->nbcols, B->d_ptrow, B->d_indcol, B->d_coef, nullptr};
    if (trace) {
        hipLaunchKernelGGL((spmv_bcsr4_fused_ext<kBcsrDepth, 4, kWG, true>), grid, dim3(kWG), 0, s, V, d_x_ext, d_y_local, C, P->d_ext_units);
        HIP_TRY(hipGetLastError());
        return MI_OK;
    }
    static const int depth = getenv("MI355_PUSH_EXT_DEPTH") ? atoi(getenv("MI355_PUSH_EXT_DEPTH")) : 24;
#define EXT_LAUNCH(P_, U_) hipLaunchKernelGGL((spmv_bcsr4_fused_ext<P_, U_, kWG>), grid, dim3(kWG), 0, s, V, d_x_ext, d_y_local, C, P->d_ext_units)
    switch (depth) {
    case 22: EXT_LAUNCH(2, 2); break;
    case 23: EXT_LAUNCH(2, 3); break;
    case 27: EXT_LAUNCH(2, 7); break;
    default: EXT_LAUNCH(2, 4); break;
    }
#undef EXT_LAUNCH
    if (split) {
        ExtComm C2 = C;
        C2.xwgs = C2.n_work = 0;
        C2.nowait = 1;
        hipLaunchKernelGGL((spmv_bcsr4_fused_ext<kBcsrDepth, 4, kWG>), dim3(P->n_ext_units - P->n_ext_plain), dim3(kWG), 0, s, V, d_x_ext, d_y_local, C2,
                           P->d_ext_units + P->n_ext_plain);
    }
    HIP_TRY(hipGetLastError());
    return MI_OK;
}

extern "C" int mi_part_spmv_push_dev(mi_part_t P, double* d_x_ext, double* d_y_local, mi_stream_t s_)
{
    CHECK_ARG(P, "null handle");
    if (!P->finalized) return fail(MI_ERR_STATE, "partition not finalized");
    hipStream_t s = (hipStream_t)s_;
    const PartPlan& pl = P->plan;
    int rc;
    if (pl.nranks == 1) {
        if ((rc = mi_spmv_dev(P->piece[0], d_x_ext, d_y_local, s))) return rc;
        return mi_spmv_dev(P->piece[1], d_x_ext, d_y_local, s);
    }
    if (!P->push_ready) return fail(MI_ERR_STATE, "mi_part_push_connect was not called");
    if ((rc = part_handoff_status(P))) return rc;
    if (stream_is_capturing(s))
        return fail(MI_ERR_UNSUPPORTED, "the push step cannot be captured into a HIP graph: its step number is a kernel argument (a replay would "
                                        "present an old step and every wait would pass at once); capture mi_part_spmv_dev (RCCL, events) instead");
    const unsigned step = ++P->push_step;
    static const unsigned spin_max = 1u << (getenv("MI355_PUSH_SPIN_LOG2") ? std::max(8, std::min(30, atoi(getenv("MI355_PUSH_SPIN_LOG2")))) : kPushSpinLog2Default);
    if (P->fused_ext) return part_ext_launch(P, d_x_ext, d_y_local, step, spin_max, s, nullptr, nullptr);
    if (P->fused) {
        RingComm C;
        C.links = P->d_links;
        C.send_idx = P->d_send_idx;
        C.flags = P->win_flags;
        C.nb = P->d_nb;
        C.halo = P->win_data + (size_t)(step & 1u) * (size_t)(pl.n_halo > 0 ? pl.n_halo : 1);
        C.run_halo = P->d_run_halo;
        C.timeouts = P->d_timeouts;
// ... 85 lines not shown
```

navierstokes_amd/csrc/devtools.hip:

```cpp
#include "capi_internal.hpp"
#include "mi355_devtools.h"

__global__ __launch_bounds__(256) void xcc_probe_kernel(int* out)
{
    __shared__ double hog[9000];
    hog[threadIdx.x] = 0.0;
    if (threadIdx.x == 0) out[blockIdx.x] = __builtin_amdgcn_s_getreg((3 << 11) | 20) & 15;
    if (hog[threadIdx.x] != 0.0) out[blockIdx.x] = -1;
}

extern "C" int mi_debug_xcc_map(int wgs, int* host_out)
{
    CHECK_ARG(wgs > 0 && host_out, "bad argument");
    int rc = need_device();
    if (rc) return rc;
    int* d = nullptr;
    HIP_TRY(hipMalloc(&d, sizeof(int) * wgs));
    hipLaunchKernelGGL(xcc_probe_kernel, dim3(wgs), dim3(256), 0, nullptr, d);
    HIP_TRY(hipMemcpy(host_out, d, sizeof(int) * wgs, hipMemcpyDeviceToHost));
    dfree(d);
    return MI_OK;
}
__global__ __launch_bounds__(256) void touch_pages_kernel(const char* __restrict__ p, size_t bytes, size_t stride, int* __restrict__ sink)
{
    int acc = 0;
    const size_t step = (size_t)gridDim.x * blockDim.x;
    for (size_t i = (size_t)blockIdx.x * blockDim.x + threadIdx.x; i * stride < bytes; i += step)
        acc += *reinterpret_cast<const int*>(p + i * stride);
    if (acc == 0x7fffffff) sink[0] = acc;
}

extern "C" int mi_debug_touch_pages(mi_csr_t A, int stride_bytes, const void* d_extra0, long long bytes0, const void* d_extra1, long long bytes1)
{
    CHECK_ARG(A && stride_bytes >= 64 && stride_bytes % 4 == 0, "bad argument");
    if (A->inner) A = A->inner;
    int* sink = nullptr;
    HIP_TRY(hipMalloc(&sink, 64));
    auto touch = [&](const void* p, size_t bytes) {
        if (!p || bytes < 4) return;
        hipLaunchKernelGGL(touch_pages_kernel, dim3(256), dim3(256), 0, nullptr, (const char*)p, bytes - 3, (size_t)stride_bytes, sink);
    };
    const size_t nnz = (size_t)A->nnz, n = (size_t)A->n;
    touch(A->d_coef, 8 * nnz);
    touch(A->d_indcol, 4 * nnz);
    touch(A->d_ptrow, 4 * (n + 1));
    touch(A->d_rowmap, 4 * n);
    if (A->ring.d_plan) {
        touch(A->ring.d_plan, 32 * (size_t)A->ring.nblk);
        touch(A->ring.d_slots, 2 * (size_t)A->ring.nblk * A->ring.cfg.nnzb);
    }
    if (A->tile.d_desc) {
        touch(A->tile.d_desc, 16 * (size_t)A->tile.nblk);
        touch(A->tile.d_ulist, (size_t)(A->tile.unique_per_nnz * 4.0 * (double)nnz));
        touch(A->tile.d_slots, 2 * nnz);
    }
    if (A->blocked) {
        touch(A->blocked->d_coef, 128 * (size_t)A->blocked->nblocks);
        touch(A->blocked->d_indcol, 4 * (size_t)A->blocked->nblocks);
        touch(A->blocked->d_ptrow, 4 * ((size_t)A->blocked->nbrows + 1));
    }
    touch(d_extra0, (size_t)bytes0);
    touch(d_extra1, (size_t)bytes1);
    HIP_TRY(hipGetLastError());
    HIP_TRY(hipDeviceSynchronize());
    dfree(sink);
    return MI_OK;
}
extern "C" int mi_part_push_debug_preset(mi_part_t P, unsigned value)
{
    CHECK_ARG(P && P->win, "no window");
    std::vector<unsigned> f((size_t)P->plan.nranks * kWinFlagStride, value);
    HIP_TRY(hipMemcpy(P->win_flags, f.data(), sizeof(unsigned) * f.size(), hipMemcpyHostToDevice));
    return MI_OK;
}

#include "spmv_mring.hpp"
extern "C" int mi_debug_mring_trace(mi_csr_t A, const double* d_x, double* d_y, int max_wgs, long long* host_out, int* wgs_out)
{
    CHECK_ARG(A && d_x && d_y && host_out && wgs_out, "null argument");
    if (A->inner) A = A->inner;
    const MringTable& M = A->mring;
    if (!M.d_plan) return fail(MI_ERR_STATE, "no multi-window ring plan on this handle");
    CHECK_ARG(M.wgs <= max_wgs, "output array too small");
    CsrView V{};
    V.n = A->n;
    V.ncols = A->ncols;
    V.ptrow = A->d_ptrow;
    V.indcol = A->d_indcol;
    V.coef = A->d_coef;
    V.rowmap = nullptr;
    V.nblk = M.nblk;
    long long* d = nullptr;
    HIP_TRY(hipMalloc(&d, sizeof(long long) * 4 * (size_t)M.wgs));
    HIP_TRY(hipMemset(d, 0, sizeof(long long) * 4 * (size_t)M.wgs));
    hipLaunchKernelGGL((spmv_csr_mring<kMringThreads, kMringNnzb, 4, kMringMaxB, false, true, false, true>), dim3(M.wgs), dim3(kMringThreads), 0, nullptr,
                       V, reinterpret_cast<const int4*>(M.d_plan), reinterpret_cast<const int4*>(M.d_first), M.d_ok, M.d_slots, d_x, d_y,
                       reinterpret_cast<const int2*>(M.d_rng), M.wgs, d);
    HIP_TRY(hipDeviceSynchronize());
    HIP_TRY(hipMemcpy(host_out, d, sizeof(long long) * 4 * (size_t)M.wgs, hipMemcpyDeviceToHost));
    dfree(d);
    *wgs_out = M.wgs;
    return MI_OK;
}

extern "C" int mi_debug_move_array(mi_csr_t A, int which, int how, unsigned long long* old_ptr, unsigned long long* new_ptr)
{
    CHECK_ARG(A && which >= 0 && which <= 3 && (how == 0 || how == 2 || how == 3), "bad argument (how = 1, hipDeviceMallocContiguous, is refused: see the comment in devtools.hip)");
    if (A->inner) A = A->inner;
    void** slot = nullptr;
    size_t bytes = 0, pad_bytes = 0;
    if (which == 0) { slot = (void**)&A->d_coef; bytes = sizeof(double) * (size_t)A->nnz; pad_bytes = sizeof(double) * (size_t)kRingPadNnz; }
    if (which == 1) { slot = (void**)&A->ring.d_slots; bytes = sizeof(unsigned short) * (size_t)A->ring.nblk * A->ring.cfg.nnzb; }
    if (which == 2) { slot = (void**)&A->d_ptrow; bytes = sizeof(int) * ((size_t)A->n + 1); pad_bytes = sizeof(int) * (size_t)kRingPadRows; }
    if (which == 3) { slot = (void**)&A->ring.d_plan; bytes = sizeof(int) * 8 * (size_t)A->ring.nblk; }
    if (!*slot || bytes == 0) return fail(MI_ERR_STATE, "the handle has no such array");
    void* fresh = nullptr;
    if (how == 0) HIP_TRY(hipMalloc(&fresh, bytes + pad_bytes));
    else HIP_TRY(hipExtMallocWithFlags(&fresh, bytes + pad_bytes, how == 2 ? hipDeviceMallocUncached : hipDeviceMallocFinegrained));
    if (pad_bytes) HIP_TRY(hipMemset((char*)fresh + bytes, 0, pad_bytes));
    HIP_TRY(hipMemcpy(fresh, *slot, bytes, hipMemcpyDeviceToDevice));
    HIP_TRY(hipDeviceSynchronize());
    if (old_ptr) *old_ptr = (unsigned long long)(uintptr_t)*slot;
    if (new_ptr) *new_ptr = (unsigned long long)(uintptr_t)fresh;
    void* old = *slot;
    *slot = fresh;
    HIP_TRY(hipFree(old));
    return MI_OK;
}

#include "mring_plan.hpp"
extern "C" int mi_debug_mring_replan(mi_csr_t A, int skew_pct, int* table_len, int* longest_run)
{
    CHECK_ARG(A, "null handle");
    if (A->inner) A = A->inner;
    MringTable& M = A->mring;
    if (!M.d_plan || !A->d_indcol) return fail(MI_ERR_STATE, "no multi-window ring plan (or no column indices) on this handle");
    std::vector<int> ind((size_t)A->nnz);
    HIP_TRY(hipMemcpy(ind.data(), A->d_indcol, sizeof(int) * (size_t)A->nnz, hipMemcpyDeviceToHost));
    MringPlanHost P;
    build_mring_plan(A->n, A->h_ptrow.data(), ind.data(), P, 0, skew_pct);
    if (P.nblk != M.nblk) return fail(MI_ERR_STATE, "the new plan has other row blocks");
    if (const char* bad = check_mring_plan(P, A->n, A->h_ptrow.data(), ind.data())) return fail(MI_ERR_STATE, std::string("mring plan: ") + bad);
    HIP_TRY(hipDeviceSynchronize());
    HIP_TRY(hipMemcpy(M.d_plan, P.plan.data(), sizeof(int) * P.plan.size(), hipMemcpyHostToDevice));
    HIP_TRY(hipMemcpy(M.d_slots, P.slots.data(), sizeof(unsigned short) * P.slots.size(), hipMemcpyHostToDevice));
    dfree(M.d_first); dfree(M.d_ok); dfree(M.d_rng);
    M.d_first = M.d_ok = M.d_rng = nullptr;
    HIP_TRY(hipMalloc(&M.d_first, sizeof(int) * P.first.size()));
    HIP_TRY(hipMalloc(&M.d_ok, sizeof(int) * P.run_ok.size()));
    HIP_TRY(hipMalloc(&M.d_rng, sizeof(int) * P.run_rng.size()));
    HIP_TRY(hipMemcpy(M.d_first, P.first.data(), sizeof(int) * P.first.size(), hipMemcpyHostToDevice));
    HIP_TRY(hipMemcpy(M.d_ok, P.run_ok.data(), sizeof(int) * P.run_ok.size(), hipMemcpyHostToDevice));
    HIP_TRY(hipMemcpy(M.d_rng, P.run_rng.data(), sizeof(int) * P.run_rng.size(), hipMemcpyHostToDevice));
    M.wgs = P.wgs;
    M.nruns = P.nruns;
    M.bpw = P.bpw;
    M.bad_runs = P.bad_runs;
    if (table_len) *table_len = P.wgs;
    if (longest_run) {
        *longest_run = 0;
        for (int g = 0; g < P.wgs; g++) *longest_run = std::max(*longest_run, P.run_rng[2 * g + 1] - P.run_rng[2 * g]);
    }
    return MI_OK;
// ... 96 lines not shown
```

navierstokes_amd/csrc/launch_csr.hip:

```cpp
#include "capi_internal.hpp"
#include "spmv_rowpar.hpp"
#include "spmv_tile.hpp"
#include "spmv_mring.hpp"

int reorder_scratch(mi_csr_t A, hipStream_t s, double** buf)
{
    std::lock_guard<std::mutex> lock(g_mu);
    if (!A->xp_claimed || A->xp_stream == s) {
        A->xp_claimed = true;
        A->xp_stream = s;
        *buf = A->d_xp;
        return MI_OK;
    }
    double*& b = A->xp_more[s];
    if (!b) {
        if (stream_is_capturing(s)) return fail(MI_ERR_STATE, "first product of a relabelled handle on this stream: run one outside stream capture first (it allocates a gather buffer)");
        HIP_TRY(hipMalloc(&b, sizeof(double) * (size_t)A->n));
    }
    *buf = b;
    return MI_OK;
}

bool ring_dot_eligible(const mi_csr_s* A)
{
    if (A->inner || A->n == 0 || A->d_rowmap || A->y_offset) return false;
    if (resolve_kernel(A) != MI_KERNEL_RING) return false;
    const RingTable& R = A->ring;
    int depth = R.cfg.depth;
    if (const char* e = getenv("MI355_RING_DEPTH")) depth = atoi(e);
    return R.cfg.id == 4 && R.lean && depth != 3 && R.all_in_loop && R.wgs >= 1 && R.wgs <= 1024  &&
           !env_is("MI355_SPMV_DOT_EPILOGUE", "0");
}

int launch_spmv(mi_csr_t A, const double* d_x, double* d_y, hipStream_t s, bool use_map, const RingComm* comm, const RingDot* dot)
{
    if (dot && !ring_dot_eligible(A)) return fail(MI_ERR_STATE, "dot epilogue requested on a handle whose launch cannot carry it");
    if (A->n == 0) return MI_OK;
    const bool ss_fused = comm && resolve_kernel(A) == MI_KERNEL_SSTREAM && A->ss.fusable;
    if (comm && (A->inner || A->d_rowmap || (resolve_kernel(A) != MI_KERNEL_RING && !ss_fused)))
        return fail(MI_ERR_STATE, "fused multi-GPU step: the combined piece must be an unmapped, unreordered handle served by the ring or the sliced-stream kernel");
    if (A->inner) {
        double* xp = nullptr;
        int rc = reorder_scratch(A, s, &xp);
        if (rc) return rc;
        if ((rc = gather_perm(A, d_x, xp, s))) return rc;
        return launch_spmv(A->inner, xp, d_y, s, true);
    }
    int kid = resolve_kernel(A);
    if (kid == MI_KERNEL_SSTREAM && !dot && (!comm || ss_fused)) {
        const int* map = use_map ? A->d_rowmap : nullptr;
        double* yy = d_y + (use_map ? A->y_offset : 0);
        if (sstream_y_ok(A, yy, map)) return launch_sstream(A, d_x, yy, map, s, comm);
        if (comm) return fail(MI_ERR_ARG, "fused multi-GPU step: y must be 16-byte aligned");
        kid = A->ring.d_plan && A->ring.ok_fraction >= 0.90 ? MI_KERNEL_RING : MI_KERNEL_STREAM;
    } else if (kid == MI_KERNEL_SSTREAM) {
        kid = A->ring.d_plan && A->ring.ok_fraction >= 0.90 ? MI_KERNEL_RING : MI_KERNEL_STREAM;
    }
    if (use_map) d_y += A->y_offset;
    CsrView V{};
    V.n = A->n;
    V.ncols = A->ncols;
    V.ptrow = A->d_ptrow;
    V.indcol = A->d_indcol;
    V.coef = A->d_coef;
    V.rowmap = use_map ? A->d_rowmap : nullptr;
    V.blk = nullptr;
    V.blk_span = nullptr;
    V.nblk = 0;
    if (kid == MI_KERNEL_BCSR4 && (((uintptr_t)d_x) & 15) == 0) return launch_bcsr4(A->blocked, d_x, d_y, (mi_stream_t)s, use_map);
    if (kid == MI_KERNEL_BCSR4) {
        BlockTable* T = nullptr;
        int rc = get_table(A, 1024, &T);
        if (rc) return rc;
        V.blk = T->d_blk;
        V.nblk = T->nblk;
        const int grid = kNXCD * ((T->nblk + kNXCD - 1) / kNXCD);
        hipLaunchKernelGGL((spmv_csr_stream<1024, false>), dim3(grid), dim3(kWG), 0, s, V, d_x, d_y);
        HIP_TRY(hipGetLastError());
        return MI_OK;
    }
    if (kid == MI_KERNEL_MRING) {
        const MringTable& M = A->mring;
        V.nblk = M.nblk;
        const int4* plan = reinterpret_cast<const int4*>(M.d_plan);
        const int2* rng = reinterpret_cast<const int2*>(M.d_rng);
#define MRING_L(D_, MP_, NT_, SK_) hipLaunchKernelGGL((spmv_csr_mring<kMringThreads, kMringNnzb, D_, kMringMaxB, MP_, NT_, SK_>), dim3(M.wgs), dim3(kMringThreads), 0, s, V, plan, reinterpret_cast<const int4*>(M.d_first), M.d_ok, M.d_slots, d_x, d_y, rng, M.wgs)
#define MRING_L3(D_, MP_) do { if (M.nt) { if (M.skew) MRING_L(D_, MP_, true, true); else MRING_L(D_, MP_, true, false); } \
                               else { if (M.skew) MRING_L(D_, MP_, false, true); else MRING_L(D_, MP_, false, false); } } while (0)
#define MRING_L2(D_) do { if (V.rowmap) MRING_L3(D_, true); else MRING_L3(D_, false); } while (0)
        int depth = M.depth;
        if (const char* e = getenv("MI355_RING_DEPTH")) depth = atoi(e);
        if (depth == 4) MRING_L2(4);
        else MRING_L2(2);
#undef MRING_L2
#undef MRING_L3
#undef MRING_L
    } else if (kid == MI_KERNEL_TILE) {
        const TileTable& T = A->tile;
        const int grid = kNXCD * ((T.nblk + kNXCD - 1) / kNXCD);
        const int4* desc = reinterpret_cast<const int4*>(T.d_desc);
#define TILE_LAUNCH(NT_, SK_) hipLaunchKernelGGL((spmv_csr_tile<kTileNnzb, NT_, SK_>), dim3(grid), dim3(kTileThreads), 0, s, V, desc, T.nblk, T.d_ulist, T.d_slots, d_x, d_y)
        if (T.nt) { if (T.skew) TILE_LAUNCH(true, true); else TILE_LAUNCH(true, false); }
        else { if (T.skew) TILE_LAUNCH(false, true); else TILE_LAUNCH(false, false); }
#undef TILE_LAUNCH
    } else if (kid == MI_KERNEL_ROWPAR) {
        hipLaunchKernelGGL(spmv_csr_rowpar, dim3((A->n + kWG - 1) / kWG), dim3(kWG), 0, s, V, d_x, d_y);
    } else if (kid == MI_KERNEL_RING) {
        V.nblk = A->ring.nblk;
        launch_ring_cfg(A, V, d_x, d_y, s, comm, dot);
    } else {
        BlockTable* T = nullptr;
        int rc = get_table(A, 1024, &T);
        if (rc) return rc;
        V.blk = T->d_blk;
        V.nblk = T->nblk;
        const int grid = kNXCD * ((T->nblk + kNXCD - 1) / kNXCD);
        if (A->stream_nt) hipLaunchKernelGGL((spmv_csr_stream<1024, true>), dim3(grid), dim3(kWG), 0, s, V, d_x, d_y);
        else hipLaunchKernelGGL((spmv_csr_stream<1024, false>), dim3(grid), dim3(kWG), 0, s, V, d_x, d_y);
    }
    HIP_TRY(hipGetLastError());
    return MI_OK;
}
// ... 1 lines not shown
```

navierstokes_amd/csrc/launch_spmk.hip:

```cpp
#include "capi_internal.hpp"
#include "spmk_ring.hpp"

template <int D, bool NT, bool SKEW>
static hipError_t launch_fused_t(const mi_csr_s* H, const CsrView& V, const SpmkArgs& K, hipStream_t s, bool query, int* max_blocks)
{
    auto kern = spmk_csr_ring<256, 2048, 5120, D, kRingMaxB, NT, SKEW>;
    if (query) return hipOccupancyMaxActiveBlocksPerMultiprocessor(max_blocks, kern, 256, 0);
    hipLaunchKernelGGL(kern, dim3(H->ring.wgs), dim3(256), 0, s, V, reinterpret_cast<const int4*>(H->ring.d_plan), H->ring.d_slots,
                       reinterpret_cast<const int2*>(H->ring.d_rng), H->ring.uniform ? H->ring.bpw : 0, K);
    return hipGetLastError();
}

static hipError_t launch_fused(const mi_csr_s* H, const CsrView& V, const SpmkArgs& K, hipStream_t s, bool query = false, int* max_blocks = nullptr)
{
    const bool nt = H->ring.nt, sk = H->ring.skew;
    if (H->ring.cfg.depth == 4) {
        if (nt) return sk ? launch_fused_t<4, true, true>(H, V, K, s, query, max_blocks) : launch_fused_t<4, true, false>(H, V, K, s, query, max_blocks);
        return sk ? launch_fused_t<4, false, true>(H, V, K, s, query, max_blocks) : launch_fused_t<4, false, false>(H, V, K, s, query, max_blocks);
    }
    if (nt) return sk ? launch_fused_t<2, true, true>(H, V, K, s, query, max_blocks) : launch_fused_t<2, true, false>(H, V, K, s, query, max_blocks);
    return sk ? launch_fused_t<2, false, true>(H, V, K, s, query, max_blocks) : launch_fused_t<2, false, false>(H, V, K, s, query, max_blocks);
}

void spmk_release(mi_csr_t H)
{
    dfree(H->d_kflags);
    dfree(H->d_kdep_ptr);
    dfree(H->d_kdep_run);
    if (H->h_ktimeouts) (void)hipHostFree(H->h_ktimeouts);
    H->d_kflags = nullptr;
    H->d_kdep_ptr = H->d_kdep_run = nullptr;
    H->h_ktimeouts = H->d_ktimeouts = nullptr;
    H->kstep_setup = 0;
}

static CsrView unmapped_view(const mi_csr_s* H)
{
    CsrView V{};
    V.n = H->n;
    V.ncols = H->ncols;
    V.ptrow = H->d_ptrow;
    V.indcol = H->d_indcol;
    V.coef = H->d_coef;
    V.rowmap = nullptr;
    V.blk = nullptr;
    V.blk_span = nullptr;
    V.nblk = H->ring.nblk;
    return V;
}

static int spmk_setup(mi_csr_t H)
{
    if (H->kstep_setup) return H->kstep_setup;
    H->kstep_setup = -1;
    const RingTable& R = H->ring;
    const int kid = resolve_kernel(H);
    if (H->inner || H->n != H->ncols || (kid != MI_KERNEL_RING && kid != MI_KERNEL_SSTREAM) || !R.d_plan || R.ok_fraction < 0.90 || R.cfg.id != 4 || !R.lean || !R.all_in_loop ||
        R.cfg.depth == 3 || R.h_dep_ptr.empty() || R.wgs < kNXCD || R.wgs % kNXCD)
        return -1;
    int maxdep = 0;
    for (int g = 0; g < R.wgs; g++) maxdep = std::max(maxdep, R.h_dep_ptr[g + 1] - R.h_dep_ptr[g]);
    if (maxdep > 64) return -1;
    int per_cu = 0, dev = 0, cus = 0;
    SpmkArgs dummy{};
    if (launch_fused(H, unmapped_view(H), dummy, nullptr, true, &per_cu) != hipSuccess || hipGetDevice(&dev) != hipSuccess ||
        hipDeviceGetAttribute(&cus, hipDeviceAttributeMultiprocessorCount, dev) != hipSuccess) {
        (void)hipGetLastError();
        return -1;
    }
    if ((long long)per_cu * cus < R.wgs) return -1;
    hipError_t e;
    const size_t nflag = (size_t)R.wgs * kSpmkFlagStride;
    if ((e = hipMalloc(&H->d_kflags, sizeof(unsigned) * nflag)) != hipSuccess || (e = hipMemset(H->d_kflags, 0, sizeof(unsigned) * nflag)) != hipSuccess ||
        (e = hipStreamSynchronize(nullptr)) != hipSuccess ||
        (e = hipMalloc(&H->d_kdep_ptr, sizeof(int) * R.h_dep_ptr.size())) != hipSuccess ||
        (e = hipMalloc(&H->d_kdep_run, sizeof(int) * std::max<size_t>(1, R.h_dep_run.size()))) != hipSuccess ||
        (e = hipMemcpy(H->d_kdep_ptr, R.h_dep_ptr.data(), sizeof(int) * R.h_dep_ptr.size(), hipMemcpyHostToDevice)) != hipSuccess ||
        (R.h_dep_run.size() && (e = hipMemcpy(H->d_kdep_run, R.h_dep_run.data(), sizeof(int) * R.h_dep_run.size(), hipMemcpyHostToDevice)) != hipSuccess) ||
        (e = hipHostMalloc((void**)&H->h_ktimeouts, sizeof(unsigned), hipHostMallocMapped)) != hipSuccess) {
        (void)hipGetLastError();
        spmk_release(H);
        H->kstep_setup = -1;
        return -1;
    }
    *H->h_ktimeouts = 0;
    if (hipHostGetDevicePointer((void**)&H->d_ktimeouts, H->h_ktimeouts, 0) != hipSuccess) {
        spmk_release(H);
        H->kstep_setup = -1;
        return -1;
    }
    H->kstep_epoch = 0;
    H->kstep_setup = 1;
    return 1;
}

static int spmk_chain(mi_csr_t H, int k, const double* d_x, double* const* d_y, hipStream_t s)
{
    const double* src = d_x;
    for (int p = 0; p < k; p++) {
        int rc = launch_spmv(H, src, d_y[p], s, false);
        if (rc) return rc;
        src = d_y[p];
    }
    return MI_OK;
}

static int spmk_fused(mi_csr_t H, int k, const double* d_x, double* const* d_y, hipStream_t s)
{
    SpmkArgs K{};
    K.x = d_x;
    for (int p = 0; p < k; p++) K.y[p] = d_y[p];
    for (int p = k; p < kSpmkFusedMaxK; p++) K.y[p] = d_y[k - 1];
    K.k = k;
    K.epoch = H->kstep_epoch;
    H->kstep_epoch += (unsigned)k;
    K.flags = H->d_kflags;
    K.dep_ptr = H->d_kdep_ptr;
    K.dep_run = H->d_kdep_run;
    K.timeouts = H->d_ktimeouts;
    static const unsigned spin_max = 1u << (getenv("MI355_SPMK_SPIN_LOG2") ? std::max(8, std::min(30, atoi(getenv("MI355_SPMK_SPIN_LOG2")))) : 21);
    K.spin_max = spin_max;
    K.acquire = env_is("MI355_SPMK_ACQUIRE", "1") ? 1 : 0;
    hipError_t e = launch_fused(H, unmapped_view(H), K, s);
    if (e != hipSuccess) return fail(MI_ERR_HIP, std::string("one-launch powers step: ") + hipGetErrorString(e));
    return MI_OK;
}

int spmk_unmapped(mi_csr_t H, int k, const double* d_x, double* const* d_y, hipStream_t s)
{
    if (H->h_ktimeouts && __atomic_load_n(H->h_ktimeouts, __ATOMIC_ACQUIRE) != 0)
        return fail(MI_ERR_HIP, "mi_spmk: a hand-off wait of the one-launch powers step gave up (workgroups of the grid were not all resident); "
                                "results since then are invalid — set MI355_SPMK_FUSED=0 when other kernels share the GPU");
    if (k < 2 || k > kSpmkFusedMaxK || env_is("MI355_SPMK_FUSED", "0") || stream_is_capturing(s) || spmk_setup(H) != 1) return spmk_chain(H, k, d_x, d_y, s);
    if (env_is("MI355_SPMK_FUSED", "1")) return spmk_fused(H, k, d_x, d_y, s);
    if (H->kstep_choice[k] == 0) {
        LaunchTimer tm(s);
        if (tm.init() != MI_OK) {
            (void)hipGetLastError();
            return spmk_chain(H, k, d_x, d_y, s);
        }
        double us[2] = {0, 0};
        int rc = MI_OK;
        for (int round = 0; round < 2 && !rc; round++)
            for (int form = 0; form < 2 && !rc; form++) {
                double t = 0.0;
                rc = tm.time(2, 5, [&] { return form ? spmk_fused(H, k, d_x, d_y, s) : spmk_chain(H, k, d_x, d_y, s); }, &t);
                if (!rc) us[form] = min_measured(us[form], t);
                if (form == 1 && H->h_ktimeouts && __atomic_load_n(H->h_ktimeouts, __ATOMIC_ACQUIRE) != 0) round = 2;
            }
        if (rc) return rc;
        H->kstep_us[k][0] = us[0];
        H->kstep_us[k][1] = us[1];
        const bool gave_up = H->h_ktimeouts && __atomic_load_n(H->h_ktimeouts, __ATOMIC_ACQUIRE) != 0;
        if (gave_up) *H->h_ktimeouts = 0;
        H->kstep_choice[k] = (!gave_up && us[1] > 0 && us[1] < 0.98 * us[0]) ? 1 : -1;
    }
    return H->kstep_choice[k] == 1 ? spmk_fused(H, k, d_x, d_y, s) : spmk_chain(H, k, d_x, d_y, s);
}

extern "C" int mi_csr_spmk_info(mi_csr_t A, int k, int* eligible, int* one_launch, double* us_k_launches, double* us_one_launch)
{
    CHECK_ARG(A && k >= 1 && k <= MI_MAX_POWERS, "bad argument");
    mi_csr_t H = A->inner ? A->inner : A;
    const bool small = k <= kSpmkFusedMaxK;
    if (eligible) *eligible = small && k >= 2 && H->kstep_setup == 1;
    if (one_launch) *one_launch = small && (env_is("MI355_SPMK_FUSED", "1") ? H->kstep_setup == 1 : H->kstep_choice[k] == 1);
    if (us_k_launches) *us_k_launches = small ? H->kstep_us[k][0] : 0.0;
    if (us_one_launch) *us_one_launch = small ? H->kstep_us[k][1] : 0.0;
    return MI_OK;
}
```

navierstokes_amd/csrc/spmv_bcsr_sell.hpp:

```cpp
#pragma once
#include <hip/hip_runtime.h>

#include <algorithm>
#include <vector>

#include "spmv_kernels.hpp"

namespace mi355 {

constexpr int kSellRows = 16;
constexpr int kSellStepDoubles = 256;
constexpr int kSellPadSteps = 48;
constexpr unsigned kSellPadCol = 0x80000000u;
constexpr unsigned kSellFirstCol = 0x40000000u;
constexpr unsigned kSellColMask = 0x3fffffffu;

struct SellView {
    const double* val;
    const unsigned* col;
    const int* sptr;
    const int* wrng;
    int nslices, nbrows;
    const int* browmap = nullptr;
};
// ... 28 lines not shown
        for (int r = 0; r < kSellRows; r++) P.col[(size_t)P.sptr[s] * kSellRows + r] |= kSellFirstCol;
    for (int r = 0; r < kSellRows; r++) P.col[(size_t)t * kSellRows + r] |= kSellFirstCol;
    P.nsteps = t;
    P.sptr[P.nslices] = P.sptr[P.nslices + 1] = P.sptr[P.nslices + 2] = (int)t;
    build_sell_wave_ranges(P, nwaves_max, P.wrng, P.nwaves);
}

inline void build_sell_wave_ranges(const SellPlanHost& P, int nwaves_max, std::vector<int>& wrng, int& nwaves, int nslices_static)
{
    const int NS = nslices_static >= 0 ? std::min(nslices_static, P.nslices) : P.nslices;
    const int W = std::min(nwaves_max, std::max(32, (P.nslices / 2 + 31) / 32 * 32));
    nwaves = W;
    wrng.assign((size_t)W + 1, NS);
    wrng[0] = 0;
    const long long steps = P.sptr[NS];
    int s = 0;
    for (int w = 1; w < W; w++) {
        const long long target = steps * w / W;
        while (s < NS && P.sptr[s] < target) s++;
        wrng[w] = s;
    }
}

typedef double sell_v2d __attribute__((ext_vector_type(2)));

template <bool NT>
__device__ __forceinline__ sell_v2d sell_ld(const sell_v2d* p)
{
    return NT ? __builtin_nontemporal_load(p) : *p;
}

__global__ __launch_bounds__(64) void bcsr4_to_sell_kernel(int nslices, int nbrows, const int* __restrict__ ptrow, const double* __restrict__ coef,
                                                           const int* __restrict__ sptr, double* __restrict__ val)
{
    const int lane = threadIdx.x, r = lane >> 2, q = lane & 3;
    for (int s = blockIdx.x; s < nslices; s += gridDim.x) {
        const int bi = kSellRows * s + r;
        const int b0 = bi < nbrows ? ptrow[bi] : 0, n = bi < nbrows ? ptrow[bi + 1] - b0 : 0;
        const int t0 = sptr[s], L = sptr[s + 1] - t0;
        for (int j = 0; j < L; j++) {
            sell_v2d lo = {0.0, 0.0}, hi = {0.0, 0.0};
            if (j < n) {
                const sell_v2d* src = reinterpret_cast<const sell_v2d*>(coef + 16 * (size_t)(b0 + j) + 4 * q);
                lo = src[0];
                hi = src[1];
            }
            sell_v2d* dst = reinterpret_cast<sell_v2d*>(val + (size_t)(t0 + j) * kSellStepDoubles);
            dst[lane] = lo;
            dst[64 + lane] = hi;
        }
    }
}

template <int CAP>
__global__ __launch_bounds__(256) void bcsr4_refresh_kernel(int nslices, int nbrows, const int* __restrict__ csr_ptrow, const double* __restrict__ src,
                                                            double* __restrict__ csr_out, const int* __restrict__ bptr, double* __restrict__ bval,
                                                            const int* __restrict__ sptr, double* __restrict__ sell_val)
{
    __shared__ double buf[CAP > 0 ? CAP : 1];
    __shared__ int rp[4 * kSellRows + 1];
    __shared__ int bp[kSellRows + 1];
    const int tid = threadIdx.x;
    for (int s = blockIdx.x; s < nslices; s += gridDim.x) {
        if (tid <= 4 * kSellRows) rp[tid] = csr_ptrow[min(4 * kSellRows * s + tid, 4 * nbrows)];
        if (tid <= kSellRows) bp[tid] = bptr[min(kSellRows * s + tid, nbrows)];
        __syncthreads();
        const int base = rp[0], seg = rp[4 * kSellRows] - base;
        const bool staged = CAP > 0 && seg <= CAP;
        if (staged) {
            for (int k0 = tid; k0 < seg; k0 += 4 * 256) {
                double v[4];
#pragma unroll
                for (int u = 0; u < 4; u++) v[u] = src[base + min(k0 + 256 * u, seg - 1)];
#pragma unroll
                for (int u = 0; u < 4; u++)
                    if (k0 + 256 * u < seg) {
                        buf[k0 + 256 * u] = v[u];
                        if (csr_out) csr_out[base + k0 + 256 * u] = v[u];
                    }
            }
            __syncthreads();
        } else if (csr_out) {
            for (int k = tid; k < seg; k += 256) csr_out[base + k] = src[base + k];
        }
        auto at = [&](int row, int pos) -> double { return staged ? buf[rp[row] - base + pos] : src[rp[row] + pos]; };
        for (int r = 0; r < kSellRows; r++) {
            const int nb = bp[r + 1] - bp[r];
            for (int k = tid; k < 16 * nb; k += 256) bval[16 * (size_t)bp[r] + k] = at(4 * r + ((k >> 2) & 3), 4 * (k >> 4) + (k & 3));
        }
        if (sell_val) {
            const int t0 = sptr[s], L = sptr[s + 1] - t0;
            for (int k = tid; k < L * 128; k += 256) {
                const int j = k >> 7, h = (k >> 6) & 1, lane = k & 63, r = lane >> 2, q = lane & 3;
                sell_v2d v = {0.0, 0.0};
                if (j < bp[r + 1] - bp[r]) {
                    v.x = at(4 * r + q, 4 * j + 2 * h);
                    v.y = at(4 * r + q, 4 * j + 2 * h + 1);
                }
                reinterpret_cast<sell_v2d*>(sell_val + (size_t)(t0 + j) * kSellStepDoubles)[h * 64 + lane] = v;
            }
        }
        __syncthreads();
    }
}

template <int CAP, bool COLMAJOR>
__global__ __launch_bounds__(256) void bcsr4_blocks_refresh_kernel(int nslices, int nbrows, const int* __restrict__ bptr, const double* __restrict__ src,
                                                                   double* __restrict__ bval_out, const int* __restrict__ sptr, double* __restrict__ sell_val)
{
    __shared__ double buf[CAP > 0 ? CAP : 1];
    __shared__ int bp[kSellRows + 1];
    const int tid = threadIdx.x;
    for (int s = blockIdx.x; s < nslices; s += gridDim.x) {
        if (tid <= kSellRows) bp[tid] = bptr[min(kSellRows * s + tid, nbrows)];
        __syncthreads();
        const size_t base = 16 * (size_t)bp[0];
        const int seg = 16 * (bp[kSellRows] - bp[0]);
        const bool staged = CAP > 0 && seg <= CAP;
        const bool copy_in_stage = staged && !COLMAJOR && bval_out != nullptr;
        if (staged) {
            for (int k0 = tid; k0 < seg; k0 += 4 * 256) {
                double v[4];
#pragma unroll
                for (int u = 0; u < 4; u++) v[u] = src[base + min(k0 + 256 * u, seg - 1)];
#pragma unroll
                for (int u = 0; u < 4; u++)
                    if (k0 + 256 * u < seg) {
                        buf[k0 + 256 * u] = v[u];
                        if (copy_in_stage) bval_out[base + k0 + 256 * u] = v[u];
                    }
            }
            __syncthreads();
        }
        auto el = [&](int blk, int q, int c) -> double {
            const int o = 16 * blk + (COLMAJOR ? 4 * c + q : 4 * q + c);
            return staged ? buf[o] : src[base + o];
        };
        if (bval_out && !copy_in_stage)
            for (int k = tid; k < seg; k += 256) bval_out[base + k] = el(k >> 4, (k >> 2) & 3, k & 3);
        if (sell_val) {
            const int t0 = sptr[s], L = sptr[s + 1] - t0;
            for (int k = tid; k < L * 128; k += 256) {
// ... 250 lines not shown
```

navierstokes_amd/csrc/spmv_sstream.hpp:

```cpp
#pragma once
#include <hip/hip_runtime.h>

#include <algorithm>
#include <thread>
#include <vector>

#include "spmv_ring.hpp"

namespace mi355 {

typedef double ss_v2d __attribute__((ext_vector_type(2)));
constexpr int kSsRing = 8192;
constexpr int kSsSliceRows = 128;
constexpr int kSsRound = 512;
constexpr int kSsNewMax = 1024;
constexpr int kSsPark = 20;
#ifndef MI355_SS_TAIL
#define MI355_SS_TAIL 2
#endif
constexpr int kSsTail = MI355_SS_TAIL;
constexpr unsigned kSsPad = 0x8000u;
constexpr unsigned kSsFirst = 0x4000u;
constexpr int kSsPadSteps = 64;
constexpr int kSsMaxWgs = 256;
// ... 229 lines not shown
        if (W.r_begin < W.r_end) {
            const int2 w0 = P.win[W.r_begin], w1 = P.win[std::min(W.r_begin + 1, W.r_end - 1)];
            if (W.w0_lo != w0.x || W.w0_n != w0.y || W.w1_lo != w1.x || W.w1_n != w1.y) return "a workgroup record disagrees with the window table";
        }
        bool names_ghost = false;
        for (int r = P.rptr[g]; r < P.rptr[g + 1]; r++) {
            const int2 w = P.win[r];
            if (r == P.rptr[g]) { wlo = w.x; whi = w.x + w.y; }
            else {
                if (w.x != whi) return "a round's new columns do not continue the window";
                whi += w.y;
                if (w.y > kSsNewMax) return "too many new columns";
            }
            wlo = std::max(wlo, whi - kSsRing);
            for (int wv = 0; wv < 4; wv++) {
                const int row0 = r * kSsRound + wv * kSsSliceRows;
                const size_t base = (size_t)P.slice_step[(size_t)r * 4 + wv] * 64;
                int L = 1;
                for (int v = row0; v < std::min(nv, row0 + kSsSliceRows); v++) L = std::max(L, PT(v + 1) - PT(v));
                if (L != P.slice_len[(size_t)r * 4 + wv]) return "slice length disagrees with the rows";
                for (int j = 0; j < L; j++)
                    for (int l = 0; l < 64; l++) {
                        const unsigned s = P.slot[base + (size_t)j * 64 + l];
                        if (l == 0 && ((s & kSsFirst) != 0) != (j == 0)) return "slice-begin flag misplaced";
                        for (int h = 0; h < 2; h++) {
                            const int v = row0 + 2 * l + h;
                            const unsigned sh = (s >> (16 * h)) & 0xffffu;
                            const bool real = v < nv && j < PT(v + 1) - PT(v);
                            if (!real) {
                                if (!(sh & kSsPad)) return "a padding place is not flagged";
                                continue;
                            }
                            const int c = indcol[PT(v) + j];
                            if (sh & kSsPad) return "a nonzero is flagged as padding";
                            if ((sh & (kSsRing - 1)) != (unsigned)(c & (kSsRing - 1))) return "slot is not the column's ring slot";
                            if (c < wlo || c >= whi) return "a column lies outside the window when its round runs";
                            names_ghost = names_ghost || (ghost_lo < ghost_hi && (c < ghost_lo || c >= ghost_hi));
                        }
                    }
            }
        }
        if (names_ghost && !P.wg_halo[g]) return "a workgroup names a ghost column and is not marked";
        if (P.fusable && P.wg_halo[g])
            for (int r = P.rptr[g] + 1; r < P.rptr[g + 1]; r++)
                if (P.win[r].y != 0) return "a ghost-reading workgroup takes columns in after its first fill";
        if (W.halo != P.wg_halo[g]) return "a workgroup record's ghost mark disagrees with the plan's";
    }
    return nullptr;
}

template <int CAP>
__global__ __launch_bounds__(256) void sstream_fill_kernel(int nslices, int n, int shift, const int* __restrict__ ptrow, const double* __restrict__ src,
                                                           double* __restrict__ csr_out, const int* __restrict__ slice_step, const int* __restrict__ slice_len,
                                                           ss_v2d* __restrict__ val, int pair64)
{
    __shared__ double buf[CAP > 0 ? CAP : 1];
    __shared__ int rp[kSsSliceRows + 1];
    const int tid = threadIdx.x;
    for (int sidx = blockIdx.x; sidx < nslices; sidx += gridDim.x) {
        const int row0 = kSsSliceRows * sidx - shift;
        if (tid <= kSsSliceRows) rp[tid] = ptrow[max(0, min(row0 + tid, n))];
        __syncthreads();
        const int base = rp[0], seg = rp[kSsSliceRows] - base;
        const bool staged = CAP > 0 && seg <= CAP;
        if (staged) {
            for (int k = tid; k < seg; k += 256) {
                const double v = src[base + k];
                buf[k] = v;
                if (csr_out) csr_out[base + k] = v;
            }
            __syncthreads();
        } else if (csr_out) {
            for (int k = tid; k < seg; k += 256) csr_out[base + k] = src[base + k];
        }
        const int t0 = slice_step[sidx], L = slice_len[sidx];
        for (int q = tid; q < L * 64; q += 256) {
            const int j = q >> 6, lane = q & 63;
            const int ra = pair64 ? lane : 2 * lane, rb = pair64 ? lane + 64 : 2 * lane + 1;
            const int a0 = rp[ra], a1 = rp[ra + 1], b0 = rp[rb], b1 = rp[rb + 1];
            ss_v2d v = {0.0, 0.0};
            if (j < a1 - a0) v.x = staged ? buf[a0 - base + j] : src[a0 + j];
            if (j < b1 - b0) v.y = staged ? buf[b0 - base + j] : src[b0 + j];
            val[(size_t)(t0 + j) * 64 + lane] = v;
        }
        __syncthreads();
    }
}

inline void sstream_fill_values(int rounds, int n, int shift, const int* d_ptrow, const double* d_src, double* d_csr_out, const int* d_slice_step,
                                const int* d_slice_len, ss_v2d* d_val, int max_slice_nnz, hipStream_t s, int pair64 = 0)
{
    const int nslices = 4 * rounds;
    if (nslices <= 0) return;
    if (max_slice_nnz <= 2048)
        hipLaunchKernelGGL((sstream_fill_kernel<2048>), dim3((unsigned)std::min(nslices, 2048)), dim3(256), 0, s, nslices, n, shift, d_ptrow, d_src, d_csr_out, d_slice_step, d_slice_len, d_val, pair64);
    else if (max_slice_nnz <= 8192)
        hipLaunchKernelGGL((sstream_fill_kernel<8192>), dim3((unsigned)std::min(nslices, 1024)), dim3(256), 0, s, nslices, n, shift, d_ptrow, d_src, d_csr_out, d_slice_step, d_slice_len, d_val, pair64);
    else
        hipLaunchKernelGGL((sstream_fill_kernel<0>), dim3((unsigned)std::min(nslices, 2048)), dim3(256), 0, s, nslices, n, shift, d_ptrow, d_src, d_csr_out, d_slice_step, d_slice_len, d_val, pair64);
}

struct SsDevice {
    ss_v2d* val = nullptr;
    unsigned* slot = nullptr;
    SsWg* wg = nullptr;
    int2* win = nullptr;
    int* slice_step = nullptr;
    int* slice_len = nullptr;
    int* wg_halo = nullptr;
    int2* winK = nullptr;
};
inline void ss_free(SsDevice& Dv)
{
    (void)hipFree(Dv.winK);
    (void)hipFree(Dv.val); (void)hipFree(Dv.slot); (void)hipFree(Dv.wg); (void)hipFree(Dv.win); (void)hipFree(Dv.slice_step); (void)hipFree(Dv.slice_len); (void)hipFree(Dv.wg_halo);
    Dv = SsDevice();
}
inline hipError_t ss_upload(const SsPlanHost& P, SsDevice& Dv, bool ghosts)
{
    hipError_t e;
    const size_t vbytes = sizeof(ss_v2d) * (size_t)(P.steps + kSsPadSteps) * 64;
    if ((e = hipMalloc(&Dv.val, vbytes)) != hipSuccess || (e = hipMalloc(&Dv.slot, sizeof(unsigned) * P.slot.size())) != hipSuccess ||
        (e = hipMalloc(&Dv.wg, sizeof(SsWg) * P.wg.size())) != hipSuccess || (e = hipMalloc(&Dv.win, sizeof(int2) * P.win.size())) != hipSuccess ||
        (e = hipMalloc(&Dv.slice_step, sizeof(int) * P.slice_step.size())) != hipSuccess || (e = hipMalloc(&Dv.slice_len, sizeof(int) * P.slice_len.size())) != hipSuccess ||
        (ghosts && (e = hipMalloc(&Dv.wg_halo, sizeof(int) * P.wg_halo.size())) != hipSuccess) ||
        (e = hipMemset((char*)Dv.val + sizeof(ss_v2d) * (size_t)P.steps * 64, 0, sizeof(ss_v2d) * (size_t)kSsPadSteps * 64)) != hipSuccess ||
        (e = hipMemcpy(Dv.slot, P.slot.data(), sizeof(unsigned) * P.slot.size(), hipMemcpyHostToDevice)) != hipSuccess ||
        (e = hipMemcpy(Dv.wg, P.wg.data(), sizeof(SsWg) * P.wg.size(), hipMemcpyHostToDevice)) != hipSuccess ||
        (e = hipMemcpy(Dv.win, P.win.data(), sizeof(int2) * P.win.size(), hipMemcpyHostToDevice)) != hipSuccess ||
        (e = hipMemcpy(Dv.slice_step, P.slice_step.data(), sizeof(int) * P.slice_step.size(), hipMemcpyHostToDevice)) != hipSuccess ||
        (e = hipMemcpy(Dv.slice_len, P.slice_len.data(), sizeof(int) * P.slice_len.size(), hipMemcpyHostToDevice)) != hipSuccess ||
        (ghosts && (e = hipMemcpy(Dv.wg_halo, P.wg_halo.data(), sizeof(int) * P.wg_halo.size(), hipMemcpyHostToDevice)) != hipSuccess)) {
        ss_free(Dv);
        return e;
    }
    return hipSuccess;
}

template <int D, bool NT, int ABL, int MODE>
__device__ __forceinline__ void ss_body(const SsView& S, const SsWg& W, int g, const double* __restrict__ x_in, double* __restrict__ y, const RingComm& C,
                                        double* ring , ss_v2d* s_park )
{
    constexpr bool GHOSTS = MODE == 2;
    const int tid = threadIdx.x, lane = tid & 63;
    const int wv = __builtin_amdgcn_readfirstlane(tid >> 6);
    const double* __restrict__ x = MODE != 0 ? x_in - C.n_left : x_in;
    const int r_begin = W.r_begin, r_end = W.r_end;
    if ((ABL & 8) && tid == 0) S.trace[4 * g] = __builtin_amdgcn_s_memrealtime();
    if (GHOSTS && W.link >= 0 && C.npush_runs > 0)
        for (int l = W.link; l < C.n_links; l += C.npush_runs) ring_push_link<256>(C, x_in, l);
    ss_v2d* park = s_park + wv * kSsPark * 64 + lane;
    int parked = 0, park_first = 0;
// ... 151 lines not shown
```

navierstokes_amd/mpk.py:

```python
from __future__ import annotations

import ctypes
import os

import numpy as np

_HERE = os.path.dirname(os.path.abspath(__file__))
LIB_PATH = os.environ.get("MI355_SPMV_LIBRARY") or os.path.join(_HERE, "csrc", "libmi355spmv.so")

MI_OK = 0
KERNEL_AUTO, KERNEL_STREAM, KERNEL_RING, KERNEL_ROWPAR = 0, 1, 2, 3
KERNELS = {"auto": 0, "stream": 1, "ring": 2, "rowpar": 3, "bcsr4": 4, "tile": 5, "mring": 6, "sstream": 7}

_c = ctypes
_vp = ctypes.c_void_p
_LIB = None


class MiError(RuntimeError):
    def __init__(self, status, detail):
        super().__init__(f"libmi355spmv status {status}: {detail}")
        self.status = status


# ... 25 lines not shown
        "mi_device_synchronize": [],
        "mi_flush_cache": [],
        "mi_flush_cache_async": [_vp],
        "mi_csr_create": [i, i, _vp, _vp, _vp, P(_vp)],
        "mi_csr_create_mapped": [i, i, _vp, _vp, _vp, _vp, P(_vp)],
        "mi_csr_destroy": [_vp],
        "mi_csr_update_values": [_vp, _vp],
        "mi_csr_update_values_dev": [_vp, _vp, _vp],
        "mi_bcsr4_update_values": [_vp, _vp],
        "mi_bcsr4_update_values_dev": [_vp, _vp, _vp],
        "mi_orthonormalize_against_basis": [i, i, _vp, _vp, _vp],
        "mi_orthonormalize_against_basis_dev": [i, i, _vp, _vp, _vp, _vp],
        "mi_mdot": [i, i, _vp, _vp, _vp],
        "mi_mdot_dev": [i, i, _vp, _vp, _vp, _vp],
        "mi_maxpy": [i, i, _vp, i, _vp, _vp],
        "mi_maxpy_dev": [i, i, _vp, i, _vp, _vp, _vp, _vp],
        "mi_cgs_dev": [i, i, _vp, _vp, i, _vp, _vp, _vp],
        "mi_part_status": [_vp],
        "mi_part_push_export": [_vp, _vp, _vp],
        "mi_part_push_connect": [_vp, _vp, _vp],
        "mi_part_spmv_push_dev": [_vp, _vp, _vp, _vp],
        "mi_part_push_info": [_vp, P(i), P(i), P(i)],
        "mi_part_sends_contiguous": [_vp, P(i)],
        "mi_part_combined_info": [_vp, P(i)],
        "mi_part_push_disable": [_vp],
        "mi_part_push_unfuse": [_vp],
        "mi_bcsr4_spmm": [_vp, i, _vp, ll, _vp, ll, i],
        "mi_bcsr4_spmm_info": [_vp, i, P(i), P(i), P(i), P(d)],
        "mi_bcsr4_spmm_dev": [_vp, i, _vp, ll, _vp, ll, i, _vp],
        "mi_spmm_dev": [_vp, i, _vp, ll, _vp, ll, _vp],
        "mi_krylov_basis_dev": [_vp, i, _vp, _vp, ll, i, _vp, _vp],
        "mi_krylov_basis_cgs_dev": [_vp, i, _vp, _vp, ll, i, _vp, _vp],
        "mi_csr_reorder_info": [_vp, P(i), P(i), P(d), P(d), P(d), P(d)],
        "mi_reorder_probe": [i, _vp, _vp, P(i), _vp, P(d), P(d)],
        "mi_csr_perm": [_vp, P(i), _vp],
        "mi_vec_to_internal_dev": [_vp, _vp, _vp, _vp],
        "mi_vec_from_internal_dev": [_vp, _vp, _vp, _vp],
        "mi_spmv_internal_dev": [_vp, _vp, _vp, _vp],
        "mi_spmk_internal_dev": [_vp, i, _vp, _vp, _vp],
        "mi_csr_dims": [_vp, P(i), P(i), P(ll)],
        "mi_csr_set_kernel": [_vp, i],
        "mi_csr_get_kernel": [_vp, P(i)],
        "mi_csr_ring_info": [_vp, P(i), P(i), P(i), P(d)],
        "mi_csr_ring_shape_info": [_vp, P(i), P(i), P(i), P(d), P(d)],
        "mi_csr_tune_info": [_vp, P(d), P(d)],
        "mi_csr_tune_detail": [_vp, P(d), P(_c.c_int), P(_c.c_int)],
        "mi_csr_set_nontemporal": [_vp, i, i],
        "mi_csr_block4_structure": [i, _vp, _vp, P(i), P(_c.c_longlong)],
        "mi_ring_plan_probe": [i, _vp, _vp, i, P(i), P(i), P(i), P(d), P(i)],
        "mi_ring_plan_lean": [i, _vp, _vp, i, P(i)],
        "mi_csr_tile_info": [_vp, P(i), P(i), P(d), P(d), P(i)],
        "mi_bcsr4_tile_info": [_vp, P(i), P(i), P(d), P(d)],
        "mi_bcsr4_sell_info": [_vp, P(i), P(i), P(ll), P(d), P(d)],
        "mi_bcsr4_sell_plan_probe": [i, _vp, _vp, i, P(i), P(ll), P(i), _vp, _vp, _vp],
        "mi_csr_mring_info": [_vp, P(i), P(i), P(i), P(d), P(d), P(i)],
        "mi_csr_sstream_info": [_vp, P(i), P(i), P(ll), P(d), P(d), P(i)],
        "mi_sstream_plan_probe": [i, i, _vp, _vp, P(i), P(i), P(ll), P(d)],
        "mi_sstream_plan_probe_ex": [i, i, _vp, _vp, i, i, i, P(i), P(i), P(ll), P(d), P(i), P(i)],
        "mi_sstream_mw_plan_probe": [i, i, _vp, _vp, i, P(i), P(i), P(ll), P(d)],
        "mi_csr_placement_info": [_vp, P(i), P(i), P(d), i],
        "mi_vec_alloc_placed": [_vp, i, i, P(_vp), P(d), i, P(i)],
        "mi_vec_free_placed": [_vp],
        "mi_mring_plan_deal_probe": [i, _vp, _vp, P(i), _vp, i],
        "mi_mring_plan_probe": [i, _vp, _vp, P(i), P(i), P(i), P(d), P(ll)],
        "mi_tile_plan_probe": [i, _vp, _vp, i, P(i), P(ll), P(i), P(ll)],
        "mi_stream_read_probe": [ll, i, P(d)],
        "mi_spmv": [_vp, _vp, _vp],
        "mi_spmv_dev": [_vp, _vp, _vp, _vp],
        "mi_spmk": [_vp, i, _vp, _vp],
        "mi_spmk_dev": [_vp, i, _vp, _vp, _vp],
        "mi_csr_spmk_info": [_vp, i, P(i), P(i), P(d), P(d)],
        "mi_spmk_plan_probe": [i, _vp, _vp, P(i), P(i), P(i)],
        "mi_dot": [i, _vp, _vp, P(d)],
        "mi_dot_dev": [i, _vp, _vp, _vp, _vp],
        "mi_axpy": [i, d, _vp, _vp],
        "mi_axpy_dev": [i, d, _vp, _vp, _vp],
        "mi_orthogonalize": [i, _vp, _vp, _vp, d, P(d)],
        "mi_orthogonalize_dev": [i, _vp, _vp, _vp, d, _vp, _vp],
        "mi_spmv_dot_dev": [_vp, _vp, _vp, _vp, _vp, _vp],
        "mi_csr_dot_epilogue_info": [_vp, P(i)],
        "mi_csr_dot_epilogue_layout": [_vp, P(i), P(i), P(i), _vp, _vp, _vp, i, i],
        "mi_spmv_orthogonalize_dev": [_vp, _vp, _vp, _vp, _vp, d, _vp, _vp],
        "mi_norm2": [i, _vp, P(d)],
        "mi_norm2_dev": [i, _vp, _vp, _vp],
        "mi_rel_error": [i, _vp, _vp, P(d)],
        "mi_rel_error_dev": [i, _vp, _vp, _vp, _vp],
        "mi_gather_dev": [i, _vp, _vp, _vp, _vp],
        "mi_bcsr4_create": [i, i, _vp, _vp, _vp, P(_vp)],
        "mi_bcsr4_destroy": [_vp],
        "mi_bcsr4_create_layout": [i, i, _vp, _vp, _vp, i, P(_vp)],
        "mi_bcsr4_update_values_layout": [_vp, _vp, i],
        "mi_bcsr4_update_values_layout_dev": [_vp, _vp, i, _vp],
        "mi_bcsr4_spmv": [_vp, _vp, _vp],
        "mi_bcsr4_spmv_dev": [_vp, _vp, _vp, _vp],
        "mi_bcsr4_spmk": [_vp, i, _vp, _vp],
        "mi_bcsr4_spmk_dev": [_vp, i, _vp, _vp, _vp],
        "mi_bilu4_create": [i, _vp, _vp, _vp, i, i, P(_vp)],
        "mi_bilu4_create_host": [i, _vp, _vp, _vp, i, i, P(_vp)],
        "mi_bilu4_destroy": [_vp],
        "mi_bilu4_refactor": [_vp, _vp, i],
        "mi_bilu4_solve_dev": [_vp, _vp, _vp, _vp],
        "mi_bilu4_solve": [_vp, _vp, _vp],
        "mi_bilu4_info": [_vp, P(i), P(ll), P(i), P(i), P(i), P(i), P(d), P(d), P(ll)],
        "mi_bilu4_factor_host": [_vp, _vp, _vp, _vp, _vp, ll],
        "mi_bilu4_plan_probe": [i, _vp, _vp, i, P(ll), P(i), P(i), P(i), P(i), _vp, _vp, i],
        "mi_bilu4dev_plan_probe": [i, _vp, _vp, i, P(ll), P(i), P(ll)],
# ... 228 lines not shown
    def tile_info(self):
        b, nb, nt = _c.c_int(), _c.c_int(), _c.c_int()
        u = _c.c_double()
        us = (_c.c_double * 2)()
        check(lib().mi_csr_tile_info(self.handle, _c.byref(b), _c.byref(nb), _c.byref(u), us, _c.byref(nt)))
        return dict(built=bool(b.value), nblk=nb.value, unique_per_nnz=u.value, us=us[0], us_nt=us[1], nt=bool(nt.value))

    def reorder_info(self):
        r, b = _c.c_int(), _c.c_int()
        v = [_c.c_double() for _ in range(4)]
        check(lib().mi_csr_reorder_info(self.handle, _c.byref(r), _c.byref(b), *[_c.byref(t) for t in v]))
        return dict(reordered=bool(r.value), block=b.value, spread_before=v[0].value, spread_after=v[1].value,
                    us_natural=v[2].value, us_reordered=v[3].value)

    def spmk_info(self, k):
        e, o = _c.c_int(), _c.c_int()
        a, b = _c.c_double(), _c.c_double()
        check(lib().mi_csr_spmk_info(self.handle, int(k), _c.byref(e), _c.byref(o), _c.byref(a), _c.byref(b)))
        return dict(eligible=bool(e.value), one_launch=bool(o.value), us_k_launches=a.value, us_one_launch=b.value)

    def dot_in_epilogue(self):
        r = _c.c_int()
        check(lib().mi_csr_dot_epilogue_info(self.handle, _c.byref(r)))
        return bool(r.value)

    def dot_epilogue_layout(self):
        t, w, nb = _c.c_int(), _c.c_int(), _c.c_int()
        check(lib().mi_csr_dot_epilogue_layout(self.handle, _c.byref(t), _c.byref(w), _c.byref(nb), None, None, None, 0, 0))
        first = np.zeros(w.value + 1, np.int32)
        row0 = np.zeros(max(nb.value, 1), np.int32)
        rows = np.zeros(max(nb.value, 1), np.int32)
        check(lib().mi_csr_dot_epilogue_layout(self.handle, _c.byref(t), _c.byref(w), _c.byref(nb), first.ctypes.data,
                                               row0.ctypes.data, rows.ctypes.data, first.size, row0.size))
        return dict(threads=t.value, run_first_block=first, block_row0=row0[: nb.value], block_rows=rows[: nb.value])

    def perm(self):
        r = _c.c_int()
        p = np.empty(self.n, np.int32)
        check(lib().mi_csr_perm(self.handle, _c.byref(r), p.ctypes.data))
        return bool(r.value), p

    def to_internal(self, x, out=None):
        import torch
        out = torch.empty_like(x) if out is None else out
        check(lib().mi_vec_to_internal_dev(self.handle, _dev_ptr(x, self.n, "x"), _dev_ptr(out, self.n, "x_int"), _stream_ptr()))
        return out

    def from_internal(self, x_int, out=None):
        import torch
        out = torch.empty_like(x_int) if out is None else out
        check(lib().mi_vec_from_internal_dev(self.handle, _dev_ptr(x_int, self.n, "x_int"), _dev_ptr(out, self.n, "x"), _stream_ptr()))
        return out

    def update_values(self, coef):
        if _is_torch(coef):
            check(lib().mi_csr_update_values_dev(self.handle, _dev_ptr(coef, self.nnz, "coef"), _stream_ptr()))
        else:
            self.coef = _host_f64(coef, self.nnz, "coef")
            check(lib().mi_csr_update_values(self.handle, self.coef.ctypes.data))
        return self

    def drop_host_arrays(self):
        _ = self.handle
        self.indcol = self.indcol[:0]
        self.coef = self.coef[:0]

    def close(self):
        if self._h is not None:
            lib().mi_csr_destroy(self._h)
            self._h = None

    def __del__(self):
        try:
            self.close()
        except Exception:
            pass


class bcsr4x4_matrix:

    def __init__(self, nrows, ptrow, indcol, coef, nbcols=None, layout="row"):
        self.layout = {"row": 0, "col": 1}[layout]
        self.nrows = int(nrows)
        self.ptrow = np.ascontiguousarray(ptrow, dtype=np.int32)
        self.indcol = np.ascontiguousarray(indcol, dtype=np.int32)
        self.coef = np.ascontiguousarray(coef, dtype=np.float64)
        self.nblocks = len(self.indcol)
        self.nbcols = (int(self.indcol.max()) + 1 if self.nblocks else 0) if nbcols is None else int(nbcols)
        self.nbcols = max(self.nbcols, self.nrows)
        self._h = None

    @property
    def handle(self):
        if self._h is None:
            h = _vp()
            check(lib().mi_bcsr4_create_layout(self.nrows, self.nbcols, self.ptrow.ctypes.data, self.indcol.ctypes.data,
                                               self.coef.ctypes.data, self.layout, _c.byref(h)))
            self._h = h
        return self._h

    def update_values(self, coef):
        if _is_torch(coef):
            check(lib().mi_bcsr4_update_values_layout_dev(self.handle, _dev_ptr(coef, 16 * self.nblocks, "coef"), self.layout, _stream_ptr()))
        else:
            self.coef = _host_f64(coef, 16 * self.nblocks, "coef")
            check(lib().mi_bcsr4_update_values_layout(self.handle, self.coef.ctypes.data, self.layout))
        return self

    def close(self):
        if self._h is not None:
            lib().mi_bcsr4_destroy(self._h)
            self._h = None

    def __del__(self):
        try:
            self.close()
        except Exception:
            pass


class bilu4:

    def __init__(self, A, ptrow=None, indcol=None, coef=None, fill=0, layout="row", host_only=False):
        if isinstance(A, bcsr4x4_matrix):
            nbrows, ptrow, indcol, coef, lay = A.nrows, A.ptrow, A.indcol, A.coef, A.layout
        else:
            nbrows, lay = int(A), {"row": 0, "col": 1}[layout]
        self.nbrows = int(nbrows)
        self.layout = lay
        self.fill = int(fill)
        ptrow = np.ascontiguousarray(ptrow, dtype=np.int32)
        indcol = np.ascontiguousarray(indcol, dtype=np.int32)
        coef = _host_f64(coef, None, "coef")
        if len(ptrow) != self.nbrows + 1:
            raise ValueError("ptrow must have nbrows+1 entries")
        if coef.size < 16 * len(indcol):
            raise ValueError("coef: 16 values per block")
        self._nblocks_in = len(indcol)
        self._h = None
        h = _vp()
        make = lib().mi_bilu4_create_host if host_only else lib().mi_bilu4_create
        check(make(self.nbrows, ptrow.ctypes.data, indcol.ctypes.data, coef.ctypes.data, lay, self.fill, _c.byref(h)))
        self._h = h

    @property
    def handle(self):
        if self._h is None:
            raise ValueError("bilu4: closed")
        return self._h

    def solve(self, x, b):
        n = 4 * self.nbrows
# ... 699 lines not shown
```

Measured before the change: 1237.

## Lazily materialize CSR and block value copies when a sliced copy carries values

```diff
diff --git a/include/mi355_spmv.h b/include/mi355_spmv.h
--- a/include/mi355_spmv.h
+++ b/include/mi355_spmv.h
@@ -74,6 +74,7 @@
 int mi_vec_alloc_placed(mi_csr_t A, int nvec, int draws, double** d_vecs, double* us, int cap, int* n_us);
 int mi_vec_free_placed(double* d_vec);
 int mi_csr_sstream_info(mi_csr_t A, int* built, int* rounds, long long* steps, double* padding, double us[4], int* form);
+int mi_csr_values_state(mi_csr_t A, int* csr_stale, int* csr_live, int* blocks_stale, int* blocks_live);
 int mi_sstream_plan_probe(int n, int ncols, const int* ptrow, const int* indcol, int* eligible, int* rounds, long long* steps, double* padding);
 int mi_sstream_plan_probe_ex(int n, int ncols, const int* ptrow, const int* indcol, int shift, int ghost_lo, int ghost_hi, int* eligible, int* rounds,
                              long long* steps, double* padding, int* ghost_workgroups, int* rounds_min_max);
@@ -138,6 +139,7 @@
 int mi_bcsr4_update_values_layout_dev(mi_bcsr4_t A, const double* d_coef, int layout, mi_stream_t s);
 int mi_bcsr4_tile_info(mi_bcsr4_t A, int* built, int* in_use, double* us_plain, double* us_tile);
 int mi_bcsr4_sell_info(mi_bcsr4_t A, int* built, int* form_in_use, long long* steps, double* padding, double us[4]);
+int mi_bcsr4_values_state(mi_bcsr4_t A, int* stale, int* live);
 int mi_bcsr4_sell_plan_probe(int nbrows, const int* ptrow, const int* indcol, int nwaves_max, int* nslices, long long* nsteps, int* nwaves,
                              int* sptr, int* wrng, unsigned* col);
 int mi_bcsr4_update_values(mi_bcsr4_t A, const double* coef);
diff --git a/navierstokes_amd/csrc/capi_bcsr.hip b/navierstokes_amd/csrc/capi_bcsr.hip
--- a/navierstokes_amd/csrc/capi_bcsr.hip
+++ b/navierstokes_amd/csrc/capi_bcsr.hip
@@ -118,6 +118,7 @@
 {
     CHECK_ARG(out, "out is null");
     *out = nullptr;
+    InternalLaunches own_launches;
     CHECK_ARG(nbrows >= 0 && nbcols >= 0 && ptrow && ptrow[0] == 0, "bad argument");
     for (int i = 0; i < nbrows; i++) CHECK_ARG(ptrow[i] <= ptrow[i + 1], "ptrow must be non-decreasing");
     const long long nb = ptrow[nbrows];
@@ -161,20 +162,66 @@
     return MI_OK;
 }
 
-int bcsr4_refresh_from_csr(mi_bcsr4_s* A, const int* d_csr_ptrow, const double* d_src, double* d_csr_out, hipStream_t s)
+int bcsr4_refresh_from_csr(mi_bcsr4_s* A, const int* d_csr_ptrow, const double* d_src, double* d_csr_out, hipStream_t s, bool write_blocks, const int* d_src_start)
 {
     if (!A || A->nbrows == 0) return MI_OK;
+    if (!write_blocks && !A->d_sell_val) return fail(MI_ERR_STATE, "blocked copy: the blocks can only be skipped where a sliced copy carries the values");
+    double* const bval = write_blocks ? A->d_coef : nullptr;
     const int nslices = (A->nbrows + kSellRows - 1) / kSellRows;
     const int grid = std::max(1, std::min(nslices, 2048));
     const int* sptr = A->d_sell_val ? A->d_sell_sptr : nullptr;
     double* sv = A->d_sell_val;
     if (A->max_slice_vals <= 4096)
-        hipLaunchKernelGGL((bcsr4_refresh_kernel<4096>), dim3((unsigned)grid), dim3(256), 0, s, nslices, A->nbrows, d_csr_ptrow, d_src, d_csr_out, A->d_ptrow, A->d_coef, sptr, sv);
+        hipLaunchKernelGGL((bcsr4_refresh_kernel<4096>), dim3((unsigned)grid), dim3(256), 0, s, nslices, A->nbrows, d_csr_ptrow, d_src, d_csr_out, A->d_ptrow, bval, sptr, sv, d_src_start);
     else if (A->max_slice_vals <= 16384)
-        hipLaunchKernelGGL((bcsr4_refresh_kernel<16384>), dim3((unsigned)std::min(grid, 256)), dim3(256), 0, s, nslices, A->nbrows, d_csr_ptrow, d_src, d_csr_out, A->d_ptrow, A->d_coef, sptr, sv);
+        hipLaunchKernelGGL((bcsr4_refresh_kernel<16384>), dim3((unsigned)std::min(grid, 256)), dim3(256), 0, s, nslices, A->nbrows, d_csr_ptrow, d_src, d_csr_out, A->d_ptrow, bval, sptr, sv, d_src_start);
     else
-        hipLaunchKernelGGL((bcsr4_refresh_kernel<0>), dim3((unsigned)grid), dim3(256), 0, s, nslices, A->nbrows, d_csr_ptrow, d_src, d_csr_out, A->d_ptrow, A->d_coef, sptr, sv);
+        hipLaunchKernelGGL((bcsr4_refresh_kernel<0>), dim3((unsigned)grid), dim3(256), 0, s, nslices, A->nbrows, d_csr_ptrow, d_src, d_csr_out, A->d_ptrow, bval, sptr, sv, d_src_start);
     HIP_TRY(hipGetLastError());
+    A->coef_state.stale = !write_blocks;
+    return MI_OK;
+}
+
+int bcsr4_sliced_to_csr(mi_bcsr4_s* A, const int* d_csr_ptrow, double* d_csr_out, hipStream_t s)
+{
+    if (!bcsr4_sliced_carries(A)) return fail(MI_ERR_STATE, "CSR values are stale and no sliced copy holds them");
+    const int nslices = (A->nbrows + kSellRows - 1) / kSellRows;
+    const int grid = std::max(1, std::min(nslices, 2048));
+    if (A->max_slice_vals <= 4096)
+        hipLaunchKernelGGL((bcsr4_sell_to_csr_kernel<4096>), dim3((unsigned)grid), dim3(256), 0, s, nslices, A->nbrows, d_csr_ptrow, A->d_ptrow, A->d_sell_sptr, A->d_sell_val, d_csr_out);
+    else if (A->max_slice_vals <= 16384)
+        hipLaunchKernelGGL((bcsr4_sell_to_csr_kernel<16384>), dim3((unsigned)std::min(grid, 256)), dim3(256), 0, s, nslices, A->nbrows, d_csr_ptrow, A->d_ptrow, A->d_sell_sptr, A->d_sell_val, d_csr_out);
+    else
+        hipLaunchKernelGGL((bcsr4_sell_to_csr_kernel<0>), dim3((unsigned)grid), dim3(256), 0, s, nslices, A->nbrows, d_csr_ptrow, A->d_ptrow, A->d_sell_sptr, A->d_sell_val, d_csr_out);
+    HIP_TRY(hipGetLastError());
+    return MI_OK;
+}
+
+const double* block_values(mi_bcsr4_s* B, hipStream_t s)
+{
+    ValuesState& st = B->coef_state;
+    if (st.stale) {
+        if (!bcsr4_sliced_carries(B)) {
+            fail(MI_ERR_STATE, "block values are stale and no sliced copy holds them");
+            return nullptr;
+        }
+        const int grid = std::max(1, std::min(B->sell_nslices, 8192));
+        hipLaunchKernelGGL(sell_to_bcsr4_kernel, dim3((unsigned)grid), dim3(64), 0, s, B->sell_nslices, B->nbrows, B->d_ptrow, B->d_sell_sptr, B->d_sell_val, B->d_coef);
+        if (hipError_t e = hipGetLastError(); e != hipSuccess) {
+            fail(MI_ERR_HIP, std::string("blocks from the sliced copy: ") + hipGetErrorString(e));
+            return nullptr;
+        }
+        st.stale = false;
+    }
+    if (!g_internal_launches) st.live = true;
+    return B->d_coef;
+}
+
+extern "C" int mi_bcsr4_values_state(mi_bcsr4_t A, int* stale, int* live)
+{
+    CHECK_ARG(A, "null handle");
+    if (stale) *stale = A->coef_state.stale;
+    if (live) *live = A->coef_state.live;
     return MI_OK;
 }
 
@@ -184,8 +231,11 @@
     const int nslices = (A->nbrows + kSellRows - 1) / kSellRows;
     const int grid = std::max(1, std::min(nslices, 2048));
     const int* sptr = A->d_sell_val ? A->d_sell_sptr : nullptr;
-    double* out = d_src == A->d_coef ? nullptr : A->d_coef;
-    if (colmajor && !out) return fail(MI_ERR_ARG, "column-major blocks cannot be transposed in place");
+    const bool in_place = d_src == A->d_coef;
+    if (colmajor && in_place) return fail(MI_ERR_ARG, "column-major blocks cannot be transposed in place");
+    const bool lazy = !in_place && bcsr4_sliced_carries(A) && !A->coef_state.live;
+    double* out = in_place || lazy ? nullptr : A->d_coef;
+    A->coef_state.stale = lazy;
     if (!out && !A->d_sell_val) return MI_OK;
 #define BR_LAUNCH(CAP_, CM_, G_) hipLaunchKernelGGL((bcsr4_blocks_refresh_kernel<CAP_, CM_>), dim3((unsigned)(G_)), dim3(256), 0, s, nslices, A->nbrows, A->d_ptrow, d_src, out, sptr, A->d_sell_val)
     if (A->max_slice_vals <= 4096) { if (colmajor) BR_LAUNCH(4096, true, grid); else BR_LAUNCH(4096, false, grid); }
@@ -291,6 +341,7 @@
     if (A->nblocks == 0) return MI_OK;
     CHECK_ARG(coef, "null coef");
     HIP_TRY(hipMemcpy(A->d_coef, coef, sizeof(double) * 16 * (size_t)A->nblocks, hipMemcpyHostToDevice));
+    A->coef_state.stale = false;
     int rc = bcsr4_values_changed(A, nullptr);
     if (rc) return rc;
     HIP_TRY(hipStreamSynchronize(nullptr));
@@ -341,7 +392,7 @@
     if (A->nbrows == 0) return MI_OK;
     CHECK_ARG(d_x && d_y, "null vector");
     CHECK_ARG((((uintptr_t)d_x) & 15) == 0, "x must be 16-byte aligned");
-    Bcsr4View V{A->nbrows, A->nbcols, A->d_ptrow, A->d_indcol, A->d_coef, use_map ? A->d_browmap : nullptr};
+    Bcsr4View V{A->nbrows, A->nbcols, A->d_ptrow, A->d_indcol, nullptr, use_map ? A->d_browmap : nullptr};
     const long long threads = 4LL * A->nbrows;
     const int nwg = (int)((threads + kWG - 1) / kWG);
     static const int chunk = getenv("MI355_BCSR_XCD_CHUNK") ? atoi(getenv("MI355_BCSR_XCD_CHUNK")) : 0;
@@ -359,6 +410,7 @@
         HIP_TRY(hipGetLastError());
         return MI_OK;
     }
+    if (!(V.coef = block_values(A, (hipStream_t)s))) return MI_ERR_HIP;
     if (A->use_tile && A->d_tl_ptr) {
         Bcsr4Tile Tl{A->d_tl_ptr, A->d_tl_nodes, A->d_tl_slots};
         hipLaunchKernelGGL(spmv_bcsr4_tile<kBcsrDepth>, dim3((unsigned)grid), dim3(kWG), 0, (hipStream_t)s, V, Tl, d_x, d_y, nwg);
@@ -373,6 +425,10 @@
 void bcsr4_drop_sliced(mi_bcsr4_s* A)
 {
     if (!A || !A->d_sell_val) return;
+    {
+        InternalLaunches own_launches;
+        (void)block_values(A, nullptr);
+    }
     (void)hipDeviceSynchronize();
     dfree(A->d_sell_val);
     dfree(A->d_sell_col);
@@ -635,7 +691,7 @@
 static int launch_spmm(mi_bcsr4_t A, int s, int arith, const double* X, long long ldx, double* Y, long long ldy, hipStream_t st,
                        bool use_map)
 {
-    Bcsr4View V{A->nbrows, A->nbcols, A->d_ptrow, A->d_indcol, A->d_coef, use_map ? A->d_browmap : nullptr};
+    Bcsr4View V{A->nbrows, A->nbcols, A->d_ptrow, A->d_indcol, nullptr, use_map ? A->d_browmap : nullptr};
     for (int j0 = 0; j0 < s; j0 += 8) {
         const int m = std::min(8, s - j0);
         const double* Xj = X + (size_t)j0 * ldx;
@@ -654,6 +710,7 @@
                 }
                 return hipGetLastError();
             }
+            if (!(V.coef = block_values(A, st))) return hipErrorUnknown;
             if (form == kSpmmTile) return spmm_tile_launch(A, spmm_plan_of(A, m), V, m, arith, Xj, ldx, Yj, ldy, st);
             if (form == kSpmmOct || form == kSpmmOctNt) return spmm_otile_launch(A, &A->st64, V, m, arith, form == kSpmmOctNt, Xj, ldx, Yj, ldy, st);
             launch_spmm_gather(V, m, arith, Xj, ldx, Yj, ldy, st);
diff --git a/navierstokes_amd/csrc/capi_csr.hip b/navierstokes_amd/csrc/capi_csr.hip
--- a/navierstokes_amd/csrc/capi_csr.hip
+++ b/navierstokes_amd/csrc/capi_csr.hip
@@ -58,6 +58,9 @@
 static int build_sstream(mi_csr_t A, const int* ptrow, const int* indcol, int ghost_lo = 0, int ghost_hi = 0)
 {
     if (A->ss.dev.val) return MI_OK;
+    InternalLaunches own_launches;
+    const double* coef = csr_values(A, nullptr);
+    if (!coef) return MI_ERR_HIP;
     SsPlanHost P;
     SsMwPlanHost M;
     const int shift = (A->y_offset & 1) && !A->d_rowmap ? 1 : 0;
@@ -88,7 +91,7 @@
         T.h_wg = P.wg;
         T.fusable = P.fusable;
     }
-    sstream_fill_values(T.rounds, A->n, T.shift, A->d_ptrow, A->d_coef, nullptr, T.dev.slice_step, T.dev.slice_len, T.dev.val, T.max_slice_nnz, nullptr, T.mw ? 1 : 0);
+    sstream_fill_values(T.rounds, A->n, T.shift, A->d_ptrow, coef, nullptr, T.dev.slice_step, T.dev.slice_len, T.dev.val, T.max_slice_nnz, nullptr, T.mw ? 1 : 0);
     if ((e = hipGetLastError()) != hipSuccess) {
         free_sstream(A);
         return fail(MI_ERR_HIP, std::string("sliced copy fill: ") + hipGetErrorString(e));
@@ -699,6 +702,7 @@
 {
     CHECK_ARG(out, "out is null");
     *out = nullptr;
+    InternalLaunches own_launches;
     CsrInput in{n, ncols, ptrow, indcol, coef, rowmap, ghost_lo, ghost_hi};
     int rc = check_input(in);
     if (rc || (rc = need_device())) return rc;
@@ -806,6 +810,7 @@
 
 extern "C" int mi_csr_create(int n, int ncols, const int* ptrow, const int* indcol, const double* coef, mi_csr_t* out)
 {
+    InternalLaunches own_launches;
     int rc = csr_create_impl(n, ncols, ptrow, indcol, coef, nullptr, out, 0, 0, true);
     if (rc) return rc;
     if ((rc = maybe_reorder(*out, ptrow, indcol, coef)) || (!(*out)->inner && (rc = placement_draws(*out, nullptr, nullptr, n == ncols))) ||
@@ -942,8 +947,38 @@
     return MI_OK;
 }
 
+const double* csr_values(mi_csr_s* A, hipStream_t s)
+{
+    ValuesState& st = A->coef_state;
+    if (st.stale) {
+        if (A->ss.dev.val) {
+            const SstreamTable& T = A->ss;
+            sstream_unfill_values(T.rounds, A->n, T.shift, A->d_ptrow, T.dev.val, T.dev.slice_step, T.dev.slice_len, A->d_coef, T.max_slice_nnz, s, T.mw ? 1 : 0);
+            if (hipError_t e = hipGetLastError(); e != hipSuccess) {
+                fail(MI_ERR_HIP, std::string("CSR values from the sliced copy: ") + hipGetErrorString(e));
+                return nullptr;
+            }
+        } else if (bcsr4_sliced_to_csr(A->blocked, A->d_ptrow, A->d_coef, s) != MI_OK) return nullptr;
+        st.stale = false;
+    }
+    if (!g_internal_launches) st.live = true;
+    return A->d_coef;
+}
+
+extern "C" int mi_csr_values_state(mi_csr_t A, int* csr_stale, int* csr_live, int* blocks_stale, int* blocks_live)
+{
+    CHECK_ARG(A, "null handle");
+    if (A->inner) A = A->inner;
+    if (csr_stale) *csr_stale = A->coef_state.stale;
+    if (csr_live) *csr_live = A->coef_state.live;
+    if (blocks_stale) *blocks_stale = A->blocked ? (int)A->blocked->coef_state.stale : -1;
+    if (blocks_live) *blocks_live = A->blocked ? (int)A->blocked->coef_state.live : -1;
+    return MI_OK;
+}
+
 static int refresh_blocked_values(mi_csr_t A, hipStream_t s, bool sliced_done = false)
 {
+    A->coef_state.stale = false;
     if (A->ss.dev.val && !sliced_done) {
         SstreamTable& T = A->ss;
         sstream_fill_values(T.rounds, A->n, T.shift, A->d_ptrow, A->d_coef, nullptr, T.dev.slice_step, T.dev.slice_len, T.dev.val, T.max_slice_nnz, s, T.mw ? 1 : 0);
@@ -978,29 +1013,51 @@
     }
 }
 
-extern "C" int mi_csr_update_values_dev(mi_csr_t A, const double* d_coef, mi_stream_t s_)
+static int update_values_dev(mi_csr_t A, const double* d_coef, hipStream_t s, bool eager)
 {
     CHECK_ARG(A, "null handle");
     if (A->nnz == 0) return MI_OK;
     CHECK_ARG(d_coef, "null coef");
-    hipStream_t s = (hipStream_t)s_;
+    if (A->inner && !eager && csr_sliced_carries(A->inner)) {
+        mi_csr_t I = A->inner;
+        double* csr_out = I->coef_state.live ? I->d_coef : nullptr;
+        if (I->ss.dev.val) {
+            SstreamTable& T = I->ss;
+            sstream_fill_values(T.rounds, I->n, T.shift, I->d_ptrow, d_coef, csr_out, T.dev.slice_step, T.dev.slice_len, T.dev.val, T.max_slice_nnz, s, T.mw ? 1 : 0, A->d_src_start);
+            HIP_TRY(hipGetLastError());
+        } else if (int rc = bcsr4_refresh_from_csr(I->blocked, I->d_ptrow, d_coef, csr_out, s, I->blocked->coef_state.live, A->d_src_start)) return rc;
+        I->coef_state.stale = csr_out == nullptr;
+        return MI_OK;
+    }
     if (A->inner) {
         mi_csr_t I = A->inner;
         hipLaunchKernelGGL(permute_values_kernel, dim3((unsigned)std::max(1, std::min((A->n + 63) / 64, 4096))), dim3(256), 0, s, A->n, I->d_ptrow, A->d_src_start, d_coef, I->d_coef);
         HIP_TRY(hipGetLastError());
         return refresh_blocked_values(I, s);
     }
+    const bool lazy = !eager && csr_sliced_carries(A) && d_coef != A->d_coef;
+    double* csr_out = !lazy || A->coef_state.live ? A->d_coef : nullptr;
     if (A->ss.dev.val && d_coef != A->d_coef) {
         SstreamTable& T = A->ss;
-        sstream_fill_values(T.rounds, A->n, T.shift, A->d_ptrow, d_coef, A->d_coef, T.dev.slice_step, T.dev.slice_len, T.dev.val, T.max_slice_nnz, s, T.mw ? 1 : 0);
+        sstream_fill_values(T.rounds, A->n, T.shift, A->d_ptrow, d_coef, csr_out, T.dev.slice_step, T.dev.slice_len, T.dev.val, T.max_slice_nnz, s, T.mw ? 1 : 0);
         HIP_TRY(hipGetLastError());
+        if (!csr_out) {
+            A->coef_state.stale = true;
+            return MI_OK;
+        }
         return refresh_blocked_values(A, s, true);
     }
-    if (A->blocked && A->blocked->nbrows > 0 && d_coef != A->d_coef)
-        return bcsr4_refresh_from_csr(A->blocked, A->d_ptrow, d_coef, A->d_coef, s);
+    if (A->blocked && A->blocked->nbrows > 0 && d_coef != A->d_coef) {
+        const bool blocks_out = !lazy || A->blocked->coef_state.live;
+        int rc = bcsr4_refresh_from_csr(A->blocked, A->d_ptrow, d_coef, csr_out, s, blocks_out);
+        if (rc == MI_OK) A->coef_state.stale = csr_out == nullptr;
+        return rc;
+    }
     if (d_coef != A->d_coef) HIP_TRY(hipMemcpyAsync(A->d_coef, d_coef, sizeof(double) * (size_t)A->nnz, hipMemcpyDeviceToDevice, s));
     return refresh_blocked_values(A, s);
 }
+
+extern "C" int mi_csr_update_values_dev(mi_csr_t A, const double* d_coef, mi_stream_t s) { return update_values_dev(A, d_coef, (hipStream_t)s, false); }
 
 extern "C" int mi_csr_update_values(mi_csr_t A, const double* coef)
 {
@@ -1010,7 +1067,7 @@
     if (A->inner) {
         if (!A->d_vtmp) HIP_TRY(hipMalloc(&A->d_vtmp, sizeof(double) * (size_t)A->nnz));
         HIP_TRY(hipMemcpy(A->d_vtmp, coef, sizeof(double) * (size_t)A->nnz, hipMemcpyHostToDevice));
-        int rc = mi_csr_update_values_dev(A, A->d_vtmp, nullptr);
+        int rc = update_values_dev(A, A->d_vtmp, nullptr, true);
         if (rc) return rc;
         HIP_TRY(hipStreamSynchronize(nullptr));
         return MI_OK;
diff --git a/navierstokes_amd/csrc/capi_internal.hpp b/navierstokes_amd/csrc/capi_internal.hpp
--- a/navierstokes_amd/csrc/capi_internal.hpp
+++ b/navierstokes_amd/csrc/capi_internal.hpp
@@ -129,6 +129,19 @@
     }
     return st != hipStreamCaptureStatusNone;
 }
+
+struct ValuesState {
+    bool stale = false;
+    bool live = false;
+};
+
+extern thread_local int g_internal_launches;
+struct InternalLaunches {
+    InternalLaunches() { g_internal_launches++; }
+    ~InternalLaunches() { g_internal_launches--; }
+    InternalLaunches(const InternalLaunches&) = delete;
+    InternalLaunches& operator=(const InternalLaunches&) = delete;
+};
 
 struct BlockTable {
     int nnzb = 0;
@@ -200,6 +213,7 @@
     int* d_ptrow = nullptr;
     int* d_indcol = nullptr;
     double* d_coef = nullptr;
+    ValuesState coef_state;
     int* d_rowmap = nullptr;
     bool mapped = false;
     int y_offset = 0;
@@ -262,6 +276,7 @@
     int* d_ptrow = nullptr;
     int* d_indcol = nullptr;
     double* d_coef = nullptr;
+    ValuesState coef_state;
     int* d_browmap = nullptr;
     int* d_tl_ptr = nullptr;
     unsigned* d_tl_nodes = nullptr;
@@ -395,5 +410,15 @@
 static inline bool sstream_y_ok(const mi_csr_s* A, const double* yy, const int* map) { return map || A->ss.mw || (((uintptr_t)(yy - A->ss.shift)) & 15) == 0; }
 int bcsr4_values_changed(mi_bcsr4_s* A, hipStream_t s);
 void bcsr4_drop_sliced(mi_bcsr4_s* A);
-int bcsr4_refresh_from_csr(mi_bcsr4_s* A, const int* d_csr_ptrow, const double* d_src, double* d_csr_out, hipStream_t s);
+int bcsr4_refresh_from_csr(mi_bcsr4_s* A, const int* d_csr_ptrow, const double* d_src, double* d_csr_out, hipStream_t s, bool write_blocks = true,
+                           const int* d_src_start = nullptr);
 int launch_bcsr4(mi_bcsr4_t A, const double* d_x, double* d_y, mi_stream_t s, bool use_map);
+const double* block_values(mi_bcsr4_s* B, hipStream_t s);
+const double* csr_values(mi_csr_s* A, hipStream_t s);
+static inline bool bcsr4_sliced_carries(const mi_bcsr4_s* B) { return B && B->d_sell_val && B->nblocks > 0; }
+static inline bool csr_sliced_carries(const mi_csr_s* A)
+{
+    const bool blocked = A->blocked && A->blocked->nbrows > 0;
+    return A->ss.dev.val ? !blocked : bcsr4_sliced_carries(A->blocked);
+}
+int bcsr4_sliced_to_csr(mi_bcsr4_s* B, const int* d_csr_ptrow, double* d_csr_out, hipStream_t s);
diff --git a/navierstokes_amd/csrc/capi_lib.hip b/navierstokes_amd/csrc/capi_lib.hip
--- a/navierstokes_amd/csrc/capi_lib.hip
+++ b/navierstokes_amd/csrc/capi_lib.hip
@@ -1,6 +1,7 @@
 #include "capi_internal.hpp"
 
 thread_local std::string g_err;
+thread_local int g_internal_launches = 0;
 std::mutex g_mu;
 
 int need_device()
diff --git a/navierstokes_amd/csrc/capi_part.hip b/navierstokes_amd/csrc/capi_part.hip
--- a/navierstokes_amd/csrc/capi_part.hip
+++ b/navierstokes_amd/csrc/capi_part.hip
@@ -865,7 +865,9 @@
         BlockTable* T = nullptr;
         int rc = get_table(A, 1024, &T);
         if (rc) return rc;
-        CsrView V{A->n, A->ncols, A->d_ptrow, A->d_indcol, A->d_coef, nullptr, T->d_blk, nullptr, T->nblk};
+        const double* coef = csr_values(A, s);
+        if (!coef) return MI_ERR_HIP;
+        CsrView V{A->n, A->ncols, A->d_ptrow, A->d_indcol, coef, nullptr, T->d_blk, nullptr, T->nblk};
         if (trace) hipLaunchKernelGGL((spmv_csr_fused_ext<1024, false, true>), grid, dim3(kWG), 0, s, V, d_x_ext, d_y_local, C, P->d_ext_order);
         else if (A->stream_nt) hipLaunchKernelGGL((spmv_csr_fused_ext<1024, true>), grid, dim3(kWG), 0, s, V, d_x_ext, d_y_local, C, P->d_ext_order);
         else hipLaunchKernelGGL((spmv_csr_fused_ext<1024, false>), grid, dim3(kWG), 0, s, V, d_x_ext, d_y_local, C, P->d_ext_order);
@@ -881,7 +883,9 @@
         return MI_OK;
     }
     mi_bcsr4_t B = P->piece_all->blocked;
-    Bcsr4View V{B->nbrows, B->nbcols, B->d_ptrow, B->d_indcol, B->d_coef, nullptr};
+    const double* bcoef = block_values(B, s);
+    if (!bcoef) return MI_ERR_HIP;
+    Bcsr4View V{B->nbrows, B->nbcols, B->d_ptrow, B->d_indcol, bcoef, nullptr};
     if (trace) {
         hipLaunchKernelGGL((spmv_bcsr4_fused_ext<kBcsrDepth, 4, kWG, true>), grid, dim3(kWG), 0, s, V, d_x_ext, d_y_local, C, P->d_ext_units);
         HIP_TRY(hipGetLastError());
diff --git a/navierstokes_amd/csrc/devtools.hip b/navierstokes_amd/csrc/devtools.hip
--- a/navierstokes_amd/csrc/devtools.hip
+++ b/navierstokes_amd/csrc/devtools.hip
@@ -41,7 +41,7 @@
         hipLaunchKernelGGL(touch_pages_kernel, dim3(256), dim3(256), 0, nullptr, (const char*)p, bytes - 3, (size_t)stride_bytes, sink);
     };
     const size_t nnz = (size_t)A->nnz, n = (size_t)A->n;
-    touch(A->d_coef, 8 * nnz);
+    touch(csr_values(A, nullptr), 8 * nnz);
     touch(A->d_indcol, 4 * nnz);
     touch(A->d_ptrow, 4 * (n + 1));
     touch(A->d_rowmap, 4 * n);
@@ -55,7 +55,7 @@
         touch(A->tile.d_slots, 2 * nnz);
     }
     if (A->blocked) {
-        touch(A->blocked->d_coef, 128 * (size_t)A->blocked->nblocks);
+        touch(block_values(A->blocked, nullptr), 128 * (size_t)A->blocked->nblocks);
         touch(A->blocked->d_indcol, 4 * (size_t)A->blocked->nblocks);
         touch(A->blocked->d_ptrow, 4 * ((size_t)A->blocked->nbrows + 1));
     }
@@ -87,7 +87,7 @@
     V.ncols = A->ncols;
     V.ptrow = A->d_ptrow;
     V.indcol = A->d_indcol;
-    V.coef = A->d_coef;
+    if (!(V.coef = csr_values(A, nullptr))) return MI_ERR_HIP;
     V.rowmap = nullptr;
     V.nblk = M.nblk;
     long long* d = nullptr;
@@ -109,6 +109,7 @@
     if (A->inner) A = A->inner;
     void** slot = nullptr;
     size_t bytes = 0, pad_bytes = 0;
+    if (which == 0 && !csr_values(A, nullptr)) return MI_ERR_HIP;
     if (which == 0) { slot = (void**)&A->d_coef; bytes = sizeof(double) * (size_t)A->nnz; pad_bytes = sizeof(double) * (size_t)kRingPadNnz; }
     if (which == 1) { slot = (void**)&A->ring.d_slots; bytes = sizeof(unsigned short) * (size_t)A->ring.nblk * A->ring.cfg.nnzb; }
     if (which == 2) { slot = (void**)&A->d_ptrow; bytes = sizeof(int) * ((size_t)A->n + 1); pad_bytes = sizeof(int) * (size_t)kRingPadRows; }
diff --git a/navierstokes_amd/csrc/launch_csr.hip b/navierstokes_amd/csrc/launch_csr.hip
--- a/navierstokes_amd/csrc/launch_csr.hip
+++ b/navierstokes_amd/csrc/launch_csr.hip
@@ -62,12 +62,12 @@
     V.ncols = A->ncols;
     V.ptrow = A->d_ptrow;
     V.indcol = A->d_indcol;
-    V.coef = A->d_coef;
     V.rowmap = use_map ? A->d_rowmap : nullptr;
     V.blk = nullptr;
     V.blk_span = nullptr;
     V.nblk = 0;
     if (kid == MI_KERNEL_BCSR4 && (((uintptr_t)d_x) & 15) == 0) return launch_bcsr4(A->blocked, d_x, d_y, (mi_stream_t)s, use_map);
+    if (!(V.coef = csr_values(A, s))) return MI_ERR_HIP;
     if (kid == MI_KERNEL_BCSR4) {
         BlockTable* T = nullptr;
         int rc = get_table(A, 1024, &T);
diff --git a/navierstokes_amd/csrc/launch_spmk.hip b/navierstokes_amd/csrc/launch_spmk.hip
--- a/navierstokes_amd/csrc/launch_spmk.hip
+++ b/navierstokes_amd/csrc/launch_spmk.hip
@@ -34,14 +34,14 @@
     H->kstep_setup = 0;
 }
 
-static CsrView unmapped_view(const mi_csr_s* H)
+static CsrView unmapped_view(const mi_csr_s* H, const double* coef)
 {
     CsrView V{};
     V.n = H->n;
     V.ncols = H->ncols;
     V.ptrow = H->d_ptrow;
     V.indcol = H->d_indcol;
-    V.coef = H->d_coef;
+    V.coef = coef;
     V.rowmap = nullptr;
     V.blk = nullptr;
     V.blk_span = nullptr;
@@ -63,7 +63,7 @@
     if (maxdep > 64) return -1;
     int per_cu = 0, dev = 0, cus = 0;
     SpmkArgs dummy{};
-    if (launch_fused(H, unmapped_view(H), dummy, nullptr, true, &per_cu) != hipSuccess || hipGetDevice(&dev) != hipSuccess ||
+    if (launch_fused(H, unmapped_view(H, nullptr), dummy, nullptr, true, &per_cu) != hipSuccess || hipGetDevice(&dev) != hipSuccess ||
         hipDeviceGetAttribute(&cus, hipDeviceAttributeMultiprocessorCount, dev) != hipSuccess) {
         (void)hipGetLastError();
         return -1;
@@ -121,7 +121,9 @@
     static const unsigned spin_max = 1u << (getenv("MI355_SPMK_SPIN_LOG2") ? std::max(8, std::min(30, atoi(getenv("MI355_SPMK_SPIN_LOG2")))) : 21);
     K.spin_max = spin_max;
     K.acquire = env_is("MI355_SPMK_ACQUIRE", "1") ? 1 : 0;
-    hipError_t e = launch_fused(H, unmapped_view(H), K, s);
+    const double* coef = csr_values(H, s);
+    if (!coef) return MI_ERR_HIP;
+    hipError_t e = launch_fused(H, unmapped_view(H, coef), K, s);
     if (e != hipSuccess) return fail(MI_ERR_HIP, std::string("one-launch powers step: ") + hipGetErrorString(e));
     return MI_OK;
 }
diff --git a/navierstokes_amd/csrc/spmv_bcsr_sell.hpp b/navierstokes_amd/csrc/spmv_bcsr_sell.hpp
--- a/navierstokes_amd/csrc/spmv_bcsr_sell.hpp
+++ b/navierstokes_amd/csrc/spmv_bcsr_sell.hpp
@@ -104,10 +104,26 @@
     }
 }
 
+__global__ __launch_bounds__(64) void sell_to_bcsr4_kernel(int nslices, int nbrows, const int* __restrict__ ptrow, const int* __restrict__ sptr,
+                                                           const double* __restrict__ val, double* __restrict__ coef)
+{
+    const int lane = threadIdx.x, r = lane >> 2, q = lane & 3;
+    for (int s = blockIdx.x; s < nslices; s += gridDim.x) {
+        const int bi = kSellRows * s + r;
+        const int b0 = bi < nbrows ? ptrow[bi] : 0, n = bi < nbrows ? ptrow[bi + 1] - b0 : 0;
+        const int t0 = sptr[s];
+        for (int j = 0; j < n; j++) {
+            const sell_v2d* src = reinterpret_cast<const sell_v2d*>(val + (size_t)(t0 + j) * kSellStepDoubles);
+            sell_v2d* dst = reinterpret_cast<sell_v2d*>(coef + 16 * (size_t)(b0 + j) + 4 * q);
+            dst[0] = src[lane];
+            dst[1] = src[64 + lane];
+        }
+    }
+}
+
 template <int CAP>
-__global__ __launch_bounds__(256) void bcsr4_refresh_kernel(int nslices, int nbrows, const int* __restrict__ csr_ptrow, const double* __restrict__ src,
-                                                            double* __restrict__ csr_out, const int* __restrict__ bptr, double* __restrict__ bval,
-                                                            const int* __restrict__ sptr, double* __restrict__ sell_val)
+__global__ __launch_bounds__(256) void bcsr4_sell_to_csr_kernel(int nslices, int nbrows, const int* __restrict__ csr_ptrow, const int* __restrict__ bptr,
+                                                                const int* __restrict__ sptr, const double* __restrict__ sell_val, double* __restrict__ csr_out)
 {
     __shared__ double buf[CAP > 0 ? CAP : 1];
     __shared__ int rp[4 * kSellRows + 1];
@@ -119,11 +135,63 @@
         __syncthreads();
         const int base = rp[0], seg = rp[4 * kSellRows] - base;
         const bool staged = CAP > 0 && seg <= CAP;
+        const int t0 = sptr[s], L = sptr[s + 1] - t0;
+        for (int k = tid; k < L * 128; k += 256) {
+            const int j = k >> 7, h = (k >> 6) & 1, lane = k & 63, r = lane >> 2, q = lane & 3;
+            if (j >= bp[r + 1] - bp[r]) continue;
+            const sell_v2d v = reinterpret_cast<const sell_v2d*>(sell_val + (size_t)(t0 + j) * kSellStepDoubles)[h * 64 + lane];
+            const int at = rp[4 * r + q] + 4 * j + 2 * h;
+            if (staged) {
+                buf[at - base] = v.x;
+                buf[at - base + 1] = v.y;
+            } else {
+                csr_out[at] = v.x;
+                csr_out[at + 1] = v.y;
+            }
+        }
+        if (staged) {
+            __syncthreads();
+            for (int k = tid; k < seg; k += 256) csr_out[base + k] = buf[k];
+        }
+        __syncthreads();
+    }
+}
+
+template <int CAP>
+__global__ __launch_bounds__(256) void bcsr4_refresh_kernel(int nslices, int nbrows, const int* __restrict__ csr_ptrow, const double* __restrict__ src,
+                                                            double* __restrict__ csr_out, const int* __restrict__ bptr, double* __restrict__ bval,
+                                                            const int* __restrict__ sptr, double* __restrict__ sell_val, const int* __restrict__ src_start)
+{
+    __shared__ double buf[CAP > 0 ? CAP : 1];
+    __shared__ int rp[4 * kSellRows + 1];
+    __shared__ int bp[kSellRows + 1];
+    __shared__ int sa[4 * kSellRows];
+    const int tid = threadIdx.x;
+    for (int s = blockIdx.x; s < nslices; s += gridDim.x) {
+        if (tid <= 4 * kSellRows) rp[tid] = csr_ptrow[min(4 * kSellRows * s + tid, 4 * nbrows)];
+        if (tid <= kSellRows) bp[tid] = bptr[min(kSellRows * s + tid, nbrows)];
+        if (src_start && tid < 4 * kSellRows) {
+            const int r = 4 * kSellRows * s + tid;
+            sa[tid] = r < 4 * nbrows ? src_start[r] - csr_ptrow[r] : 0;
+        }
+        __syncthreads();
+        const int base = rp[0], seg = rp[4 * kSellRows] - base;
+        const bool staged = CAP > 0 && seg <= CAP;
+        auto from = [&](int p) -> double {
+            if (!src_start) return src[p];
+            int lo = 0, hi = 4 * kSellRows;
+            while (hi - lo > 1) {
+                const int mid = (lo + hi) >> 1;
+                if (rp[mid] <= p) lo = mid;
+                else hi = mid;
+            }
+            return src[sa[lo] + p];
+        };
         if (staged) {
             for (int k0 = tid; k0 < seg; k0 += 4 * 256) {
                 double v[4];
 #pragma unroll
-                for (int u = 0; u < 4; u++) v[u] = src[base + min(k0 + 256 * u, seg - 1)];
+                for (int u = 0; u < 4; u++) v[u] = from(base + min(k0 + 256 * u, seg - 1));
 #pragma unroll
                 for (int u = 0; u < 4; u++)
                     if (k0 + 256 * u < seg) {
@@ -133,13 +201,14 @@
             }
             __syncthreads();
         } else if (csr_out) {
-            for (int k = tid; k < seg; k += 256) csr_out[base + k] = src[base + k];
-        }
-        auto at = [&](int row, int pos) -> double { return staged ? buf[rp[row] - base + pos] : src[rp[row] + pos]; };
-        for (int r = 0; r < kSellRows; r++) {
-            const int nb = bp[r + 1] - bp[r];
-            for (int k = tid; k < 16 * nb; k += 256) bval[16 * (size_t)bp[r] + k] = at(4 * r + ((k >> 2) & 3), 4 * (k >> 4) + (k & 3));
-        }
+            for (int k = tid; k < seg; k += 256) csr_out[base + k] = from(base + k);
+        }
+        auto at = [&](int row, int pos) -> double { return staged ? buf[rp[row] - base + pos] : src[(src_start ? sa[row] : 0) + rp[row] + pos]; };
+        if (bval)
+            for (int r = 0; r < kSellRows; r++) {
+                const int nb = bp[r + 1] - bp[r];
+                for (int k = tid; k < 16 * nb; k += 256) bval[16 * (size_t)bp[r] + k] = at(4 * r + ((k >> 2) & 3), 4 * (k >> 4) + (k & 3));
+            }
         if (sell_val) {
             const int t0 = sptr[s], L = sptr[s + 1] - t0;
             for (int k = tid; k < L * 128; k += 256) {
diff --git a/navierstokes_amd/csrc/spmv_sstream.hpp b/navierstokes_amd/csrc/spmv_sstream.hpp
--- a/navierstokes_amd/csrc/spmv_sstream.hpp
+++ b/navierstokes_amd/csrc/spmv_sstream.hpp
@@ -305,7 +305,73 @@
 template <int CAP>
 __global__ __launch_bounds__(256) void sstream_fill_kernel(int nslices, int n, int shift, const int* __restrict__ ptrow, const double* __restrict__ src,
                                                            double* __restrict__ csr_out, const int* __restrict__ slice_step, const int* __restrict__ slice_len,
-                                                           ss_v2d* __restrict__ val, int pair64)
+                                                           ss_v2d* __restrict__ val, int pair64, const int* __restrict__ src_start)
+{
+    __shared__ double buf[CAP > 0 ? CAP : 1];
+    __shared__ int rp[kSsSliceRows + 1];
+    __shared__ int sa[kSsSliceRows];
+    const int tid = threadIdx.x;
+    for (int sidx = blockIdx.x; sidx < nslices; sidx += gridDim.x) {
+        const int row0 = kSsSliceRows * sidx - shift;
+        if (tid <= kSsSliceRows) rp[tid] = ptrow[max(0, min(row0 + tid, n))];
+        if (src_start && tid < kSsSliceRows) {
+            const int r = row0 + tid;
+            sa[tid] = r >= 0 && r < n ? src_start[r] - ptrow[r] : 0;
+        }
+        __syncthreads();
+        const int base = rp[0], seg = rp[kSsSliceRows] - base;
+        const bool staged = CAP > 0 && seg <= CAP;
+        auto from = [&](int p) -> double {
+            if (!src_start) return src[p];
+            int lo = 0, hi = kSsSliceRows;
+            while (hi - lo > 1) {
+                const int mid = (lo + hi) >> 1;
+                if (rp[mid] <= p) lo = mid;
+                else hi = mid;
+            }
+            return src[sa[lo] + p];
+        };
+        if (staged) {
+            for (int k = tid; k < seg; k += 256) {
+                const double v = from(base + k);
+                buf[k] = v;
+                if (csr_out) csr_out[base + k] = v;
+            }
+            __syncthreads();
+        } else if (csr_out) {
+            for (int k = tid; k < seg; k += 256) csr_out[base + k] = from(base + k);
+        }
+        const int t0 = slice_step[sidx], L = slice_len[sidx];
+        for (int q = tid; q < L * 64; q += 256) {
+            const int j = q >> 6, lane = q & 63;
+            const int ra = pair64 ? lane : 2 * lane, rb = pair64 ? lane + 64 : 2 * lane + 1;
+            const int a0 = rp[ra], a1 = rp[ra + 1], b0 = rp[rb], b1 = rp[rb + 1];
+            ss_v2d v = {0.0, 0.0};
+            if (j < a1 - a0) v.x = staged ? buf[a0 - base + j] : src[(src_start ? sa[ra] : 0) + a0 + j];
+            if (j < b1 - b0) v.y = staged ? buf[b0 - base + j] : src[(src_start ? sa[rb] : 0) + b0 + j];
+            val[(size_t)(t0 + j) * 64 + lane] = v;
+        }
+        __syncthreads();
+    }
+}
+
+inline void sstream_fill_values(int rounds, int n, int shift, const int* d_ptrow, const double* d_src, double* d_csr_out, const int* d_slice_step,
+                                const int* d_slice_len, ss_v2d* d_val, int max_slice_nnz, hipStream_t s, int pair64 = 0, const int* d_src_start = nullptr)
+{
+    const int nslices = 4 * rounds;
+    if (nslices <= 0) return;
+    if (max_slice_nnz <= 2048)
+        hipLaunchKernelGGL((sstream_fill_kernel<2048>), dim3((unsigned)std::min(nslices, 2048)), dim3(256), 0, s, nslices, n, shift, d_ptrow, d_src, d_csr_out, d_slice_step, d_slice_len, d_val, pair64, d_src_start);
+    else if (max_slice_nnz <= 8192)
+        hipLaunchKernelGGL((sstream_fill_kernel<8192>), dim3((unsigned)std::min(nslices, 1024)), dim3(256), 0, s, nslices, n, shift, d_ptrow, d_src, d_csr_out, d_slice_step, d_slice_len, d_val, pair64, d_src_start);
+    else
+        hipLaunchKernelGGL((sstream_fill_kernel<0>), dim3((unsigned)std::min(nslices, 2048)), dim3(256), 0, s, nslices, n, shift, d_ptrow, d_src, d_csr_out, d_slice_step, d_slice_len, d_val, pair64, d_src_start);
+}
+
+template <int CAP>
+__global__ __launch_bounds__(256) void sstream_unfill_kernel(int nslices, int n, int shift, const int* __restrict__ ptrow, const ss_v2d* __restrict__ val,
+                                                             const int* __restrict__ slice_step, const int* __restrict__ slice_len, double* __restrict__ csr_out,
+                                                             int pair64)
 {
     __shared__ double buf[CAP > 0 ? CAP : 1];
     __shared__ int rp[kSsSliceRows + 1];
@@ -316,41 +382,42 @@
         __syncthreads();
         const int base = rp[0], seg = rp[kSsSliceRows] - base;
         const bool staged = CAP > 0 && seg <= CAP;
-        if (staged) {
-            for (int k = tid; k < seg; k += 256) {
-                const double v = src[base + k];
-                buf[k] = v;
-                if (csr_out) csr_out[base + k] = v;
-            }
-            __syncthreads();
-        } else if (csr_out) {
-            for (int k = tid; k < seg; k += 256) csr_out[base + k] = src[base + k];
-        }
         const int t0 = slice_step[sidx], L = slice_len[sidx];
         for (int q = tid; q < L * 64; q += 256) {
             const int j = q >> 6, lane = q & 63;
             const int ra = pair64 ? lane : 2 * lane, rb = pair64 ? lane + 64 : 2 * lane + 1;
             const int a0 = rp[ra], a1 = rp[ra + 1], b0 = rp[rb], b1 = rp[rb + 1];
-            ss_v2d v = {0.0, 0.0};
-            if (j < a1 - a0) v.x = staged ? buf[a0 - base + j] : src[a0 + j];
-            if (j < b1 - b0) v.y = staged ? buf[b0 - base + j] : src[b0 + j];
-            val[(size_t)(t0 + j) * 64 + lane] = v;
+            const bool ha = j < a1 - a0, hb = j < b1 - b0;
+            if (!ha && !hb) continue;
+            const ss_v2d v = val[(size_t)(t0 + j) * 64 + lane];
+            if (ha) {
+                if (staged) buf[a0 - base + j] = v.x;
+                else csr_out[a0 + j] = v.x;
+            }
+            if (hb) {
+                if (staged) buf[b0 - base + j] = v.y;
+                else csr_out[b0 + j] = v.y;
+            }
+        }
+        if (staged) {
+            __syncthreads();
+            for (int k = tid; k < seg; k += 256) csr_out[base + k] = buf[k];
         }
         __syncthreads();
     }
 }
 
-inline void sstream_fill_values(int rounds, int n, int shift, const int* d_ptrow, const double* d_src, double* d_csr_out, const int* d_slice_step,
-                                const int* d_slice_len, ss_v2d* d_val, int max_slice_nnz, hipStream_t s, int pair64 = 0)
+inline void sstream_unfill_values(int rounds, int n, int shift, const int* d_ptrow, const ss_v2d* d_val, const int* d_slice_step, const int* d_slice_len,
+                                  double* d_csr_out, int max_slice_nnz, hipStream_t s, int pair64 = 0)
 {
     const int nslices = 4 * rounds;
     if (nslices <= 0) return;
     if (max_slice_nnz <= 2048)
-        hipLaunchKernelGGL((sstream_fill_kernel<2048>), dim3((unsigned)std::min(nslices, 2048)), dim3(256), 0, s, nslices, n, shift, d_ptrow, d_src, d_csr_out, d_slice_step, d_slice_len, d_val, pair64);
+        hipLaunchKernelGGL((sstream_unfill_kernel<2048>), dim3((unsigned)std::min(nslices, 2048)), dim3(256), 0, s, nslices, n, shift, d_ptrow, d_val, d_slice_step, d_slice_len, d_csr_out, pair64);
     else if (max_slice_nnz <= 8192)
-        hipLaunchKernelGGL((sstream_fill_kernel<8192>), dim3((unsigned)std::min(nslices, 1024)), dim3(256), 0, s, nslices, n, shift, d_ptrow, d_src, d_csr_out, d_slice_step, d_slice_len, d_val, pair64);
+        hipLaunchKernelGGL((sstream_unfill_kernel<8192>), dim3((unsigned)std::min(nslices, 1024)), dim3(256), 0, s, nslices, n, shift, d_ptrow, d_val, d_slice_step, d_slice_len, d_csr_out, pair64);
     else
-        hipLaunchKernelGGL((sstream_fill_kernel<0>), dim3((unsigned)std::min(nslices, 2048)), dim3(256), 0, s, nslices, n, shift, d_ptrow, d_src, d_csr_out, d_slice_step, d_slice_len, d_val, pair64);
+        hipLaunchKernelGGL((sstream_unfill_kernel<0>), dim3((unsigned)std::min(nslices, 2048)), dim3(256), 0, s, nslices, n, shift, d_ptrow, d_val, d_slice_step, d_slice_len, d_csr_out, pair64);
 }
 
 struct SsDevice {
diff --git a/navierstokes_amd/mpk.py b/navierstokes_amd/mpk.py
--- a/navierstokes_amd/mpk.py
+++ b/navierstokes_amd/mpk.py
@@ -101,6 +101,8 @@
         "mi_csr_tile_info": [_vp, P(i), P(i), P(d), P(d), P(i)],
         "mi_bcsr4_tile_info": [_vp, P(i), P(i), P(d), P(d)],
         "mi_bcsr4_sell_info": [_vp, P(i), P(i), P(ll), P(d), P(d)],
+        "mi_csr_values_state": [_vp, P(i), P(i), P(i), P(i)],
+        "mi_bcsr4_values_state": [_vp, P(i), P(i)],
         "mi_bcsr4_sell_plan_probe": [i, _vp, _vp, i, P(i), P(ll), P(i), _vp, _vp, _vp],
         "mi_csr_mring_info": [_vp, P(i), P(i), P(i), P(d), P(d), P(i)],
         "mi_csr_sstream_info": [_vp, P(i), P(i), P(ll), P(d), P(d), P(i)],
@@ -435,6 +437,11 @@
         check(lib().mi_vec_from_internal_dev(self.handle, _dev_ptr(x_int, self.n, "x_int"), _dev_ptr(out, self.n, "x"), _stream_ptr()))
         return out
 
+    def values_state(self):
+        v = [_c.c_int() for _ in range(4)]
+        check(lib().mi_csr_values_state(self.handle, *[_c.byref(t) for t in v]))
+        return dict(csr=(bool(v[0].value), bool(v[1].value)), blocks=None if v[2].value < 0 else (bool(v[2].value), bool(v[3].value)))
+
     def update_values(self, coef):
         if _is_torch(coef):
             check(lib().mi_csr_update_values_dev(self.handle, _dev_ptr(coef, self.nnz, "coef"), _stream_ptr()))
@@ -481,6 +488,11 @@
                                                self.coef.ctypes.data, self.layout, _c.byref(h)))
             self._h = h
         return self._h
+
+    def values_state(self):
+        a, b = _c.c_int(), _c.c_int()
+        check(lib().mi_bcsr4_values_state(self.handle, _c.byref(a), _c.byref(b)))
+        return bool(a.value), bool(b.value)
 
     def update_values(self, coef):
         if _is_torch(coef):
```

After: 1228. No clear change (-0.7%).
